# waveygang/wfmash

Hardware: AMD Instinct MI355X
Metric: aligned bases/sec (whole node) + CIGAR-identical rate vs CPU ref (higher is better)
Workload: dtype int32; 1 GPU; C3: 64 synthetic 5%-divergence 50kb segment pairs per GPU, WFA-only (BiWFA gap-affine-2p 5,8,2,24,1; mappings pre-supplied); pairs_per_gpu=64, pairs_total=64, parallelism=records sharded over 1 GPU(s)

## Files before the change

### include/wfmash_hip.h

```cpp
#ifndef WFMASH_HIP_H_
#define WFMASH_HIP_H_

#include <stddef.h>
#include <stdint.h>

#ifdef __cplusplus
extern "C" {
#endif

#define WFM_OK              0
#define WFM_E_NODEVICE     (-1)
#define WFM_E_HIP          (-2)
#define WFM_E_ARG          (-3)
#define WFM_E_NOMEM        (-4)
#define WFM_E_UNSUPPORTED  (-5)
#define WFM_E_ARENA        (-6)

#define WFM_ST_OK            0
#define WFM_ST_UNREACHABLE (-300)
#define WFM_ST_OOM         (-200)
#define WFM_ST_MAX_SCORE   (-100)

#define WFMASH_HIP_VERSION "wfmash-hip-0.3"

// ... 135 lines not shown

#define WFM_CS_SHORT 0
#define WFM_CS_LONG  1
#define WFM_CS_NOT_DONE 1u
#define WFM_CS_SPANS    2u
typedef struct { uint32_t flags, n_runs; uint64_t off, len; } wfm_cs_t;
#define WFM_CS_SLICE 16384
int  wfm_cs_strings(wfm_handle_t* h, const wfm_seqset_t* s, const wfm_result_t* res, const uint32_t* runs, size_t n_runs_total,
                    int form, char** out, size_t* out_bytes, wfm_cs_t* per);
void wfm_free_cs(char* p);

typedef struct { uint32_t problem, kind; uint32_t p, t; uint32_t ref_len, alt_len; uint64_t off; } wfm_variant_t;
typedef struct { uint32_t flags, n_runs; uint64_t first, count; uint32_t end_gaps, pad_; } wfm_varcall_t;
#define WFM_VAR_SNV 0u
#define WFM_VAR_INS 1u
#define WFM_VAR_DEL 2u
#define WFM_VAR_MASKED 256u
#define WFM_VAR_NOT_DONE 1u
#define WFM_VAR_SPANS    2u
#define WFM_VAR_SLICE 16384
int  wfm_call_variants(wfm_handle_t* h, const wfm_seqset_t* s, const wfm_result_t* res, const uint32_t* runs, size_t n_runs_total,
                       wfm_variant_t** vars, size_t* n_vars, char** alleles, size_t* allele_bytes, wfm_varcall_t* per);
void wfm_free_variants(wfm_variant_t* vars, char* alleles);

typedef struct wfm_coverage wfm_coverage_t;
typedef struct { uint64_t base, runs_off; uint32_t n_runs, pad_; } wfm_cov_prob_t;
typedef struct { uint64_t pos; int32_t delta; uint32_t pad_; } wfm_cov_entry_t;
typedef struct { uint64_t start; uint32_t depth, pad_; } wfm_cov_interval_t;
#define WFM_COV_SPANS 2u
#define WFM_COV_TILE 4096
#define WFM_COV_SCAN_BLOCK 1024
int  wfm_coverage_create(wfm_handle_t* h, uint64_t n_bases, wfm_coverage_t** cov);
void wfm_coverage_free(wfm_coverage_t* cov);
int  wfm_coverage_add(wfm_handle_t* h, wfm_coverage_t* cov, const wfm_cov_prob_t* probs, size_t n, const uint32_t* runs, size_t n_runs_total,
                      uint32_t* flags_out);
int  wfm_coverage_export(wfm_handle_t* h, wfm_coverage_t* cov, wfm_cov_entry_t** entries, size_t* n);
int  wfm_coverage_import(wfm_handle_t* h, wfm_coverage_t* cov, const wfm_cov_entry_t* entries, size_t n);
int  wfm_coverage_intervals(wfm_handle_t* h, wfm_coverage_t* cov, wfm_cov_interval_t** iv, size_t* n, uint64_t totals[3]);
void wfm_coverage_free_list(void* p);

#define WFM_OPT_NOT_CHECKED 1u
#define WFM_OPT_SKIPPED     2u
#define WFM_OPT_CHEAPER     4u
#define WFM_OPT_UNREACHED   8u
typedef struct {
  uint32_t flags; int32_t dp_score;
  int32_t  band_lo, band_hi;
  uint64_t cells;
} wfm_optcheck_t;
#define WFM_OPT_BAND_C1   256
#define WFM_OPT_BAND_C4   1024
#define WFM_OPT_REG_MAX   4096
#define WFM_OPT_ROWS_MB   256
int wfm_check_optimal(wfm_handle_t* h, const wfm_penalties_t* pen, const wfm_seqset_t* s,
                      const wfm_result_t* res, uint64_t max_cells , wfm_optcheck_t* out);

void wfm_set_concurrent_calls(wfm_handle_t* h, int other_calls);

#define WFM_PF_ROOT_AGAIN   1u
#define WFM_PF_JOB_AGAIN    2u
#define WFM_PF_BASE_RETRY   4u
#define WFM_PF_BASE_RETRY2  8u
#define WFM_PF_BYTE_KERNEL 16u
#define WFM_PF_P2_ROUNDS   32u
#define WFM_PF_RING_KERNEL 64u
#define WFM_PF_BASE_TILES 128u
#define WFM_PF_RING_GROWN 256u
size_t wfm_get_problem_flags(const wfm_handle_t* h, uint32_t* out, size_t n);

enum {
  WFM_TC_JOBS = 0,
  WFM_TC_EXACT_ENDS = 1,
  WFM_TC_FINE_RERUNS = 2,
  WFM_TC_GAP_RERUNS = 3,
  WFM_TC_RING3 = 4,
  WFM_TC_BLOCKS_COARSE = 5,
  WFM_TC_BLOCKS_FINE = 6,
  WFM_TC_LEFT_BAND = 7,
  WFM_TC_REUSE_RESUMED = 8,
  WFM_TC_REUSE_FALLBACKS = 9,
  WFM_TC_REUSE_KEEPS = 10,
  WFM_TC_REUSE_TOUCHED = 11,
  WFM_TC_REUSE_FELL_OTHER = 12,
  WFM_TILE_COUNTERS = 13
};
size_t wfm_get_tile_counters(const wfm_handle_t* h, uint64_t* out, size_t n);

size_t wfm_trim_device_cache(void);

int  wfm_get_stats(const wfm_handle_t* h, wfm_stats_t* out);
size_t wfm_get_busy_intervals(const wfm_handle_t* h, double* start_end_ms, size_t cap);


int  wfm_hash_kmers(wfm_handle_t* h, const char* seq, int64_t len, int k,
                    uint64_t* hash, int8_t* strand);

typedef struct {
  uint64_t hash;
  int64_t  wpos;
  int64_t  wpos_end;
  int32_t  seqId;
  int16_t  strand;
  int16_t  pad_;
} wfm_minmer_t;

int  wfm_sketch_fragments(wfm_handle_t* h, const char* seq, int64_t seq_len,
                          const int64_t* frag_off, const int32_t* frag_len, size_t n,
                          int k, int s, int32_t seq_id,
                          wfm_minmer_t* out, int32_t* out_count);

typedef struct {
  int64_t  pos;
  uint64_t hash;
  int32_t  seqId;
  int8_t   side;
  int8_t   pad_[3];
} wfm_interval_point_t;

typedef struct wfm_index wfm_index_t;
typedef struct {
  int64_t  n_windows;
  int64_t  n_kept;
  int64_t  n_unique;
  int64_t  n_points;
  uint64_t threshold;
  int64_t  filtered;
  int32_t  adjusted;
  int32_t  pad_;
} wfm_index_info_t;
int  wfm_index_build(wfm_handle_t* h, const wfm_minmer_t* minmers, int64_t n, double max_kmer_freq, wfm_index_t** out);
void wfm_index_free(wfm_handle_t* h, wfm_index_t* ix);
int  wfm_index_info(const wfm_index_t* ix, wfm_index_info_t* out);
int  wfm_index_download(wfm_handle_t* h, const wfm_index_t* ix, uint64_t* uhash, int64_t* poff,
                        wfm_interval_point_t* points, wfm_minmer_t* minmers);

int  wfm_index_replicate(wfm_handle_t* src, const wfm_index_t* ix, wfm_handle_t* dst, wfm_index_t** out);

int  wfm_index_upload(wfm_handle_t* h, const uint64_t* uhash, const int64_t* poff, int64_t n_unique,
                      const wfm_interval_point_t* points, const wfm_minmer_t* minmers, int64_t n_kept,
                      wfm_index_t** out);

int64_t wfm_add_minmers(wfm_handle_t* h, const char* seq, int64_t len, int k, int w, int s, int32_t seq_id,
                        wfm_minmer_t* out, int64_t cap);

int64_t wfm_add_minmers_multi(wfm_handle_t* h, const char* const* seqs, const int64_t* lens, const int32_t* seq_ids,
                              int64_t nseq, int k, int w, int s, int threads, wfm_minmer_t* out, int64_t cap, int64_t* counts);

int wfm_index_build_sequences(wfm_handle_t* h, const char* const* seqs, const int64_t* lens, const int32_t* seq_ids,
                              int64_t nseq, int k, int w, int s, int threads, double max_kmer_freq,
                              wfm_index_t** out, int64_t* n_windows);

typedef struct wfm_minmer_part wfm_minmer_part_t;
int  wfm_sketch_part(wfm_handle_t* h, const char* const* seqs, const int64_t* lens, const int32_t* seq_ids, int64_t nseq,
                     int k, int w, int s, int threads, wfm_minmer_part_t** out);
int64_t wfm_minmer_part_info(const wfm_minmer_part_t* part, int64_t* n_records, int64_t* counts, int64_t cap);
int64_t wfm_minmer_part_download(wfm_handle_t* h, const wfm_minmer_part_t* part, wfm_minmer_t* out, int64_t cap);
void wfm_minmer_part_free(wfm_minmer_part_t* part);

typedef struct { int32_t part; int32_t seq; } wfm_part_seq_t;
#define WFM_GATHER_TILE 2048
int  wfm_index_build_parts(wfm_handle_t* h, const wfm_minmer_part_t* const* parts, int nparts, const wfm_part_seq_t* order,
                           int64_t norder, double max_kmer_freq, wfm_index_t** out, int64_t* n_windows);

int64_t wfm_prefilter_kmers(wfm_handle_t* h, const char* seq, int64_t len, int k, int w, int s, double c_factor,
                            uint32_t* pos, uint64_t* hash, int8_t* strand, int64_t cap);

int64_t wfm_finish_records(wfm_handle_t* h, const wfm_minmer_t* raw, int64_t n, int w, wfm_minmer_t* out, int64_t cap,
// ... 90 lines not shown
```

### include/wfmash_host.h

```cpp
#ifndef WFMASH_HOST_H_
#define WFMASH_HOST_H_

#include <stdint.h>
#include "wfmash_hip.h"

#ifdef __cplusplus
extern "C" {
#endif

typedef struct {
  int32_t  mismatch, gap_open1, gap_ext1, gap_open2, gap_ext2;
  float    min_identity;
  uint64_t min_alignment_length;
  float    min_block_identity;
  uint64_t target_padding;
  uint64_t query_padding;
  uint64_t wflign_max_len_minor;
  int32_t  disable_chain_patching;
  int32_t  sam_format;
  int32_t  emit_md_tag;
  int32_t  no_seq_in_sam;
  int32_t  threads;
  int32_t  resident_sequences;
} wfmh_align_params_t;

typedef struct {
  uint64_t records;
  uint64_t aligned_bp;
  uint64_t written;
  uint64_t skipped;
  uint64_t cells;
  double   ms_gpu;
  double   ms_total;
  double   ms_rows;
  double   ms_fetch;
  double   ms_wflign;
  double   ms_text;
  uint64_t batches;
  uint64_t cells_tile;
  uint64_t tile_launches;
  double   ms_tile;
  double   ms_tags;
  uint64_t records_resident;
  uint64_t lazy_fetches;
} wfmh_align_summary_t;

void wfmh_align_default_params(wfmh_align_params_t* p);

int wfmh_align_paf(wfm_handle_t* h, const char* target_fasta, const char* query_fasta,
                   const char* mapping_paf, const char* out_paf,
                   const wfmh_align_params_t* params, wfmh_align_summary_t* summary);

int wfmh_align_paf_multi(wfm_handle_t* const* handles, int n, const char* target_fasta, const char* query_fasta,
                         const char* mapping_paf, const char* out_paf,
                         const wfmh_align_params_t* params, wfmh_align_summary_t* summary);

void wfmh_set_verify(int on);
int  wfmh_verify_counts(uint64_t out[4]);
int  wfmh_verify_paf(wfm_handle_t* h, const char* target_fasta, const char* query_fasta, const char* aligned_paf, uint64_t out[4]);
char* wfmh_test_verify_parse(const char* line);

void wfmh_set_verify_optimal(int on, uint64_t max_cells);
int  wfmh_verify_optimal_counts(uint64_t out[4]);

void wfmh_set_left_align(int on);
int  wfmh_left_align_counts(uint64_t out[4]);

void wfmh_set_cs(int form);
int  wfmh_cs_counts(uint64_t out[4]);

void wfmh_set_variants(const char* path_or_null);
int  wfmh_variants_counts(uint64_t out[4]);

void wfmh_set_coverage(const char* path_or_null);
int  wfmh_coverage_counts(uint64_t out[4]);
int  wfmh_coverage_paf(wfm_handle_t* h, const char* target_fasta, const char* aligned_paf, const char* out_path, uint64_t out[4]);
char* wfmh_test_coverage_bedgraph(const char* const* names, const uint64_t* lengths, int n_seq, const uint64_t* starts, const uint32_t* depths,
                                  int64_t n_iv);

char* wfmh_test_cigar(const char* fn, const char* a, const char* b, const char* query, const char* target,
                      long long i0, long long i1);
void  wfmh_free(char* p);
void  wfmh_test_subwindow(int64_t win_start, int64_t win_end, int rev, int64_t a, int64_t b, int64_t* out_start, int64_t* out_end);
int wfmh_test_rows(const int32_t* q, int64_t n, int64_t* out);
int wfmh_test_tile_plan(const int32_t* jobs, int64_t n, const int32_t* rules, int32_t* per_block, int32_t* tasks, int64_t tasks_cap, int64_t* scalars);
int wfmh_test_p2_plan(const int32_t* cand, int64_t n, int64_t i0, int rows, int rows_bm, unsigned long long budget, int threads, int core, int64_t* geo,
                      int32_t* tasks, int64_t tasks_cap, int64_t* scalars);
int wfmh_test_base_plan(int op, const int32_t* in, int64_t n, int32_t* out);
int wfmh_test_reuse_plan(int op, const int64_t* in, int64_t n, int64_t* out);
int wfmh_test_tile_plan_dirs(const int32_t* jobs, int64_t n, const int32_t* rules, const uint8_t* dirs, int32_t* per_block, int32_t* tasks, int64_t tasks_cap,
                             int64_t* scalars);
int wfmh_test_tile_interior(const int32_t* q, int64_t n, int32_t* out);
int wfmh_test_tile_lean_waves(const int32_t* in, int64_t* out);
int wfmh_test_opt_band(const int64_t* in, int64_t* out);
int64_t wfmh_test_winnow(const char* seq, int64_t len, int k, int w, int s, int32_t seq_id,
                         const uint64_t* hash, const int8_t* strand, wfm_minmer_t* out, int64_t cap);

int64_t wfmh_test_winnow_chunked(const char* seq, int64_t len, int k, int w, int s, int32_t seq_id,
                                 const uint64_t* hash, const int8_t* strand, int64_t chunk_len,
                                 wfm_minmer_t* out, int64_t cap, int* replays);

int64_t wfmh_test_winnow_thinned(const char* seq, int64_t len, int k, int w, int s, int32_t seq_id,
                                 const uint64_t* hash, const int8_t* strand, double c_factor, int64_t chunk_len,
                                 wfm_minmer_t* out, int64_t cap, uint32_t* kept_pos, int64_t cap_kept,
                                 int64_t* n_kept, int* replays);

void wfmh_test_sort_records(wfm_minmer_t* recs, int64_t n, int threads);
int wfmh_test_packed_lce(const uint8_t* buf_p, int64_t n_p, int64_t start_p, const uint8_t* buf_t, int64_t n_t, int64_t start_t, int v, int h, int maxn);
int wfmh_test_is_acgt(const uint8_t* seq, int64_t n);

int64_t wfmh_test_winnow_model(const char* seq, int64_t len, int k, int w, int s, int32_t seq_id, const uint64_t* hash,
                               const int8_t* strand, double c_factor, int64_t chunk_len, wfm_minmer_t* out, int64_t cap,
                               uint32_t* why);

void wfmh_test_sortlike_model(wfm_minmer_t* recs, int64_t n);

int64_t wfmh_test_finish_records(const wfm_minmer_t* raw, int64_t n, int w, wfm_minmer_t* out, int64_t cap);


typedef struct {
  int32_t  kmer_size;
  int64_t  window_length;
  int64_t  block_length;
  int64_t  chain_gap;
  uint64_t max_mapping_length;
  float    percentage_identity;
  int32_t  sketch_size;
  int32_t  filter_mode;
  uint32_t num_mappings_for_segment;
  uint32_t num_mappings_for_scaffold;
  int32_t  drop_rand;
  int32_t  split;
  int32_t  merge_mappings;
  int32_t  skip_self;
  int32_t  skip_prefix;
  int32_t  lower_triangular;
  char     prefix_delim;
  int32_t  filter_length_mismatches;
  uint64_t sparsity_hash_threshold;
  double   overlap_threshold;
  double   scaffold_overlap_threshold;
  int64_t  scaffold_max_deviation;
  int64_t  scaffold_gap;
  int64_t  scaffold_min_length;
  int32_t  legacy_output;
  int32_t  minimum_hits;
  double   max_kmer_freq;
  int64_t  index_by_size;
  float    kmer_complexity_threshold;
  int32_t  stage1_topani_filter;
  int32_t  stage2_full_scan;
  float    ani_diff, ani_diff_conf;
  double   hg_numerator;
  int32_t  threads;
  int32_t  auto_pct_identity;
  int32_t  ani_percentile;
  float    ani_adjustment;
  const char* target_prefix;
  const char* target_list;
  const char* query_prefix;
  const char* query_list;
  const char* index_file;
  int32_t  write_index;
  int32_t  pad_;
  const char* scaffold_out;
  int32_t  streaming_minhash;
} wfmh_map_params_t;

void wfmh_map_default_params(wfmh_map_params_t* p);

typedef struct {
  uint64_t targets, queries, subsets;
// ... 63 lines not shown
```

### wfmash_amd/capi.py

```python
import ctypes as C
import os

import numpy as np

_HERE = os.path.dirname(os.path.abspath(__file__))
LIB_PATH = os.environ.get("WFM_LIB_PATH") or os.path.join(_HERE, "libwfmash_hip.so")

WFM_MODE_END2END_BIWFA = 0
WFM_MODE_ENDSFREE = 1
WFM_MODE_END2END_UNI = 2
WFM_MODE_MASK = 0xff
WFM_MODE_SCORE_ONLY = 0x100
WFM_MODE_SCORE_LIMIT = 0x200
WFM_ST_MAX_SCORE = -100

DEFAULT_PEN = (5, 8, 2, 24, 1)
WFM_PF_ROOT_AGAIN, WFM_PF_JOB_AGAIN, WFM_PF_BASE_RETRY, WFM_PF_BASE_RETRY2, WFM_PF_BYTE_KERNEL, WFM_PF_P2_ROUNDS, WFM_PF_RING_KERNEL, WFM_PF_BASE_TILES = 1, 2, 4, 8, 16, 32, 64, 128
WFM_PF_RING_GROWN = 256
TILE_COUNTERS = ("jobs", "exact_ends", "fine_reruns", "gap_reruns", "ring3", "blocks_coarse", "blocks_fine", "left_band",
                 "reuse_resumed", "reuse_fallbacks", "reuse_keeps", "reuse_touched", "reuse_fell_other")

EXPORTS = [
    "wfm_create", "wfm_destroy", "wfm_last_error", "wfm_device_name",
    "wfm_align_arena_bytes", "wfm_align_batch", "wfm_upload_sequences",
    "wfm_free_sequences", "wfm_align_resident", "wfm_get_stats",
    "wfm_hash_kmers", "wfm_sketch_fragments", "wfm_add_minmers",
    "wfm_index_build", "wfm_index_free", "wfm_index_info", "wfm_index_download",
    "wfm_map_l1", "wfm_map_l2", "wfm_map_fragments", "wfm_minhash_sketch", "wfm_add_minmers_multi",
    "wfm_prefilter_kmers", "wfm_index_build_sequences", "wfm_index_upload",
    "wfm_index_replicate", "wfm_device_count", "wfm_finish_records",
    "wfm_align_batch_rle", "wfm_align_resident_rle", "wfm_free_runs", "wfm_score_bounds", "wfm_get_busy_intervals", "wfm_trim_device_cache", "wfm_map_fragments_ordered", "wfm_map_sequence_cache", "wfm_selftest_dpp", "wfm_selftest_arena_growth", "wfm_set_concurrent_calls", "wfm_get_problem_flags",
    "wfm_get_tile_counters",
    "wfm_streaming_minmers", "wfm_index_build_streaming",
    "wfm_sketch_part", "wfm_minmer_part_info", "wfm_minmer_part_download", "wfm_minmer_part_free", "wfm_index_build_parts",
    "wfm_seqstore_create", "wfm_seqstore_free", "wfm_seqstore_add", "wfm_seqstore_info",
    "wfm_upload_sequence_refs", "wfm_align_refs_rle", "wfm_download_sequences",
    "wfm_check_runs", "wfm_check_optimal", "wfm_left_align_runs", "wfm_cs_strings", "wfm_free_cs",
    "wfm_call_variants", "wfm_free_variants",
    "wfm_coverage_create", "wfm_coverage_free", "wfm_coverage_add", "wfm_coverage_export", "wfm_coverage_import", "wfm_coverage_intervals",
    "wfm_coverage_free_list",
    "wfm_sketch_intersections",
]
ISECT_LDS_MAX = 4096
WFM_CK_NOT_CHECKED, WFM_CK_BAD_RUN, WFM_CK_SPANS, WFM_CK_M_DIFFERS, WFM_CK_X_EQUAL, WFM_CK_SCORE, WFM_CK_COUNTS = 1, 2, 4, 8, 16, 32, 64
CK_NAMES = ("NOT_CHECKED", "BAD_RUN", "SPANS", "M_DIFFERS", "X_EQUAL", "SCORE", "COUNTS")
CHECK_SLICE = 16384
WFM_LA_NOT_DONE, WFM_LA_SPANS = 1, 2
WFM_CS_SHORT, WFM_CS_LONG = 0, 1
WFM_CS_NOT_DONE, WFM_CS_SPANS = 1, 2
WFM_CS_SLICE = 16384
WFM_VAR_SNV, WFM_VAR_INS, WFM_VAR_DEL = 0, 1, 2
WFM_VAR_MASKED = 256
WFM_VAR_NOT_DONE, WFM_VAR_SPANS = 1, 2
WFM_VAR_SLICE = 16384
WFM_COV_SPANS = 2
WFM_COV_TILE = 4096
WFM_COV_SCAN_BLOCK = 1024
WFM_OPT_NOT_CHECKED, WFM_OPT_SKIPPED, WFM_OPT_CHEAPER, WFM_OPT_UNREACHED = 1, 2, 4, 8
OPT_NAMES = ("NOT_CHECKED", "SKIPPED", "CHEAPER", "UNREACHED")
OPT_BAND_C1, OPT_BAND_C4, OPT_REG_MAX = 256, 1024, 4096
OPT_ROWS_MB = 256
SEQ_GATHER_CHUNK = 16384


class Penalties(C.Structure):
    _fields_ = [("x", C.c_int32), ("o1", C.c_int32), ("e1", C.c_int32),
                ("o2", C.c_int32), ("e2", C.c_int32)]


class Problem(C.Structure):
    _fields_ = [("pattern", C.c_char_p), ("plen", C.c_int32),
                ("text", C.c_char_p), ("tlen", C.c_int32),
                ("mode", C.c_int32),
                ("pattern_begin_free", C.c_int32), ("pattern_end_free", C.c_int32),
                ("text_begin_free", C.c_int32), ("text_end_free", C.c_int32),
                ("score_hint", C.c_int32), ("pad_", C.c_int32)]


class ProblemRef(C.Structure):
    _fields_ = [("pattern", C.c_char_p), ("text", C.c_char_p),
                ("pattern_off", C.c_int64), ("text_off", C.c_int64),
                ("pattern_seq", C.c_int32), ("text_seq", C.c_int32),
                ("plen", C.c_int32), ("tlen", C.c_int32),
                ("mode", C.c_int32),
                ("pattern_revcomp", C.c_int32), ("text_revcomp", C.c_int32),
                ("pattern_begin_free", C.c_int32), ("pattern_end_free", C.c_int32),
                ("text_begin_free", C.c_int32), ("text_end_free", C.c_int32),
                ("score_hint", C.c_int32)]


class Result(C.Structure):
    _fields_ = [("status", C.c_int32), ("score", C.c_int32),
                ("ops_off", C.c_uint64), ("ops_len", C.c_uint32),
                ("n_runs", C.c_uint32), ("cells", C.c_uint64)]


class Check(C.Structure):
    _fields_ = [("flags", C.c_uint32), ("score", C.c_int32), ("bad_p", C.c_int32), ("bad_t", C.c_int32),
                ("bad_run", C.c_uint32), ("n_runs", C.c_uint32),
                ("matches", C.c_uint32), ("mismatches", C.c_uint32), ("ins_runs", C.c_uint32), ("ins_bases", C.c_uint32),
                ("del_runs", C.c_uint32), ("del_bases", C.c_uint32)]


# ... 984 lines not shown
                     ident.ctypes.data, cut.ctypes.data)
        f = self._L.wfm_map_l2
        f.restype = C.c_int64
        f.argtypes = [C.c_void_p, C.c_void_p, C.c_void_p, C.c_void_p, C.c_void_p, C.c_void_p, C.c_int64, C.c_int, C.c_void_p,
                      C.c_int64, C.POINTER(L2Params), C.c_void_p, C.c_void_p, C.c_int64]
        cap = 1 << 16
        while True:
            out = np.zeros(cap, dtype=MAPPING_DTYPE)
            frag = np.zeros(cap, dtype=np.int32)
            n = f(self._p, index._p, q.ctypes.data, qc.ctypes.data, ql.ctypes.data, kc.ctypes.data, nfrag, s, cd.ctypes.data, len(cd),
                  C.byref(P), out.ctypes.data, frag.ctypes.data, cap)
            if n < 0:
                raise WfmError(f"wfm_map_l2 failed ({n}): {self.last_error()}")
            if n <= cap:
                return out[:n], frag[:n]
            cap = int(n)

    def add_minmers_multi(self, seqs, k: int, w: int, s: int, seq_ids=None, threads: int = 1, cap=None):
        n = len(seqs)
        ids = np.ascontiguousarray(seq_ids if seq_ids is not None else range(n), dtype=np.int32)
        bufs = [np.frombuffer(x, dtype=np.uint8) for x in seqs]
        ptrs = (C.c_void_p * n)(*[b.ctypes.data for b in bufs])
        lens = np.array([len(x) for x in seqs], dtype=np.int64)
        cap = int(cap) if cap else 4 * int(lens.sum()) + 64
        out = np.zeros(cap, dtype=MINMER_DTYPE)
        counts = np.zeros(n, dtype=np.int64)
        f = self._L.wfm_add_minmers_multi
        f.restype = C.c_int64
        f.argtypes = [C.c_void_p, C.c_void_p, C.c_void_p, C.c_void_p, C.c_int64, C.c_int, C.c_int, C.c_int, C.c_int, C.c_void_p, C.c_int64,
                      C.c_void_p]
        tot = f(self._p, ptrs, lens.ctypes.data, ids.ctypes.data, n, k, w, s, threads, out.ctypes.data, cap, counts.ctypes.data)
        if tot < 0:
            raise WfmError(f"wfm_add_minmers_multi failed ({tot}): {self.last_error()}")
        offs = np.concatenate([[0], np.cumsum(counts)])
        return [out[offs[i]:offs[i + 1]] for i in range(n)]

    def finish_records(self, raw, w: int):
        raw = np.ascontiguousarray(raw, dtype=MINMER_DTYPE)
        f = self._L.wfm_finish_records
        f.restype = C.c_int64
        f.argtypes = [C.c_void_p, C.c_void_p, C.c_int64, C.c_int, C.c_void_p, C.c_int64, C.POINTER(C.c_int32), C.POINTER(C.c_int32)]
        cap = 4 * len(raw) + 64
        lv, hp = C.c_int32(0), C.c_int32(0)
        while True:
            out = np.zeros(cap, dtype=MINMER_DTYPE)
            n = f(self._p, raw.ctypes.data, len(raw), w, out.ctypes.data, cap, C.byref(lv), C.byref(hp))
            if n < 0:
                raise WfmError(f"wfm_finish_records failed ({n}): {self.last_error()}")
            if n <= cap:
                return out[:n], lv.value, hp.value
            cap = int(n)

    def prefilter_kmers(self, seq: bytes, k: int, w: int, s: int, c_factor: float = 4.0):
        cap = len(seq) + 1
        pos = np.zeros(cap, dtype=np.uint32)
        hsh = np.zeros(cap, dtype=np.uint64)
        st = np.zeros(cap, dtype=np.int8)
        buf = np.frombuffer(seq, dtype=np.uint8)
        f = self._L.wfm_prefilter_kmers
        f.restype = C.c_int64
        f.argtypes = [C.c_void_p, C.c_void_p, C.c_int64, C.c_int, C.c_int, C.c_int, C.c_double, C.c_void_p, C.c_void_p, C.c_void_p, C.c_int64]
        n = f(self._p, buf.ctypes.data, len(seq), k, w, s, c_factor, pos.ctypes.data, hsh.ctypes.data, st.ctypes.data, cap)
        if n < 0:
            raise WfmError(f"wfm_prefilter_kmers failed ({n}): {self.last_error()}")
        return pos[:n], hsh[:n], st[:n]

    def add_minmers(self, seq: bytes, k: int, w: int, s: int, seq_id: int = 0):
        cap = 4 * len(seq) + 64
        out = np.zeros(cap, dtype=MINMER_DTYPE)
        buf = np.frombuffer(seq, dtype=np.uint8)
        self._L.wfm_add_minmers.restype = C.c_int64
        self._L.wfm_add_minmers.argtypes = [C.c_void_p, C.c_void_p, C.c_int64, C.c_int, C.c_int, C.c_int, C.c_int32, C.c_void_p, C.c_int64]
        n = self._L.wfm_add_minmers(self._p, buf.ctypes.data, len(seq), k, w, s, seq_id, out.ctypes.data, cap)
        if n < 0:
            raise WfmError(f"wfm_add_minmers failed ({n}): {self.last_error()}")
        return out[:n]


HOST_EXPORTS = ["wfmh_test_packed_lce", "wfmh_test_is_acgt", "wfmh_align_default_params", "wfmh_align_paf", "wfmh_test_cigar", "wfmh_free", "wfmh_test_winnow",
                "wfmh_map_default_params", "wfmh_test_filter", "wfmh_map", "wfmh_test_winnow_chunked", "wfmh_test_fasta", "wfmh_test_winnow_thinned", "wfmh_test_sort_records", "wfmh_test_index_file",
                "wfmh_map_multi", "wfmh_align_paf_multi", "wfmh_test_winnow_model", "wfmh_test_sortlike_model", "wfmh_test_finish_records",
                "wfmh_release_sequences", "wfmh_test_fasta_shared", "wfmh_seed_paf", "wfmh_test_deal", "wfmh_test_subwindow",
                "wfmh_test_rows", "wfmh_test_tile_plan", "wfmh_test_p2_plan", "wfmh_test_base_plan", "wfmh_test_map_plan", "wfmh_test_filter_ordered",
                "wfmh_test_reuse_plan", "wfmh_test_tile_plan_dirs", "wfmh_test_tile_interior", "wfmh_test_tile_lean_waves", "wfmh_set_verify", "wfmh_verify_counts", "wfmh_verify_paf", "wfmh_test_verify_parse",
                "wfmh_set_verify_optimal", "wfmh_verify_optimal_counts", "wfmh_test_opt_band", "wfmh_set_left_align", "wfmh_left_align_counts", "wfmh_set_cs", "wfmh_cs_counts", "wfmh_set_variants", "wfmh_variants_counts",
                "wfmh_set_coverage", "wfmh_coverage_counts", "wfmh_coverage_paf", "wfmh_test_coverage_bedgraph",
                "wfmh_ani_matrix", "wfmh_ani_matrix_rows", "wfmh_free_ani_rows", "wfmh_set_ani_matrix", "wfmh_test_ani_tsv"]


class MapSummary(C.Structure):
    _fields_ = [("targets", C.c_uint64), ("queries", C.c_uint64), ("subsets", C.c_uint64), ("target_bp", C.c_uint64),
                ("query_bp", C.c_uint64), ("index_windows", C.c_uint64), ("fragments", C.c_uint64), ("l2_mappings", C.c_uint64),
                ("written", C.c_uint64), ("percentage_identity", C.c_float), ("sketch_size", C.c_int32), ("ms_index", C.c_double), ("ms_map", C.c_double), ("ms_filter", C.c_double),
                ("ms_total", C.c_double), ("ms_replicate", C.c_double), ("ms_identity", C.c_double), ("ms_wall", C.c_double),
                ("index_parts", C.c_int32), ("pad_", C.c_int32), ("ms_index_sketch", C.c_double), ("ms_index_merge", C.c_double)]


def _handle_array(handles):
    arr = (C.c_void_p * len(handles))(*[h._p for h in handles])
    return arr


def map_paf_multi(handles, target_fasta: str, out_paf: str, query_fasta: str = None, params=None) -> "MapSummary":
    L = load()
    L.wfmh_map_multi.restype = C.c_int
    L.wfmh_map_multi.argtypes = [C.c_void_p, C.c_int, C.c_char_p, C.c_char_p, C.c_char_p, C.c_void_p, C.POINTER(MapSummary)]
    s = MapSummary()
    rc = L.wfmh_map_multi(_handle_array(handles), len(handles), target_fasta.encode(), query_fasta.encode() if query_fasta else None,
                          out_paf.encode(), C.byref(params) if params is not None else None, C.byref(s))
    if rc != 0:
        raise WfmError(f"wfmh_map_multi failed ({rc}): {handles[0].last_error()}")
    return s


def seed_paf(target_fasta: str, seeds_paf: str, out_paf: str, query_fasta: str = None, params=None) -> "MapSummary":
    L = load()
    L.wfmh_seed_paf.restype = C.c_int
    L.wfmh_seed_paf.argtypes = [C.c_char_p, C.c_char_p, C.c_char_p, C.c_char_p, C.c_void_p, C.POINTER(MapSummary)]
    s = MapSummary()
    rc = L.wfmh_seed_paf(target_fasta.encode(), query_fasta.encode() if query_fasta else None, seeds_paf.encode(), out_paf.encode(),
                         C.byref(params) if params is not None else None, C.byref(s))
    if rc != 0:
        raise WfmError(f"wfmh_seed_paf failed ({rc})")
    return s


def map_paf(handle, target_fasta: str, out_paf: str, query_fasta: str = None, params=None) -> "MapSummary":
    L = load()
    L.wfmh_map.restype = C.c_int
    L.wfmh_map.argtypes = [C.c_void_p, C.c_char_p, C.c_char_p, C.c_char_p, C.c_void_p, C.POINTER(MapSummary)]
    s = MapSummary()
    rc = L.wfmh_map(handle._p, target_fasta.encode(), query_fasta.encode() if query_fasta else None, out_paf.encode(),
                    C.byref(params) if params is not None else None, C.byref(s))
    if rc != 0:
        raise WfmError(f"wfmh_map failed ({rc}): {handle.last_error()}")
    return s


class AniRowC(C.Structure):
    _fields_ = [("query_group", C.c_void_p), ("target_group", C.c_void_p), ("query_hashes", C.c_uint64), ("target_hashes", C.c_uint64),
                ("shared", C.c_uint64), ("jaccard", C.c_double), ("ani", C.c_double)]


def ani_matrix(handles_or_handle, target_fasta: str, query_fasta: str = None, params=None):
    L = load()
    handles = list(handles_or_handle) if isinstance(handles_or_handle, (list, tuple)) else [handles_or_handle]
    f = L.wfmh_ani_matrix_rows
    f.restype = C.c_int
    f.argtypes = [C.c_void_p, C.c_int, C.c_char_p, C.c_char_p, C.c_void_p, C.POINTER(C.POINTER(AniRowC)), C.POINTER(C.c_int64)]
    L.wfmh_free_ani_rows.restype = None
    L.wfmh_free_ani_rows.argtypes = [C.POINTER(AniRowC), C.c_int64]
    rows, n = C.POINTER(AniRowC)(), C.c_int64(0)
    rc = f(_handle_array(handles), len(handles), os.fsencode(target_fasta), os.fsencode(query_fasta) if query_fasta else None,
           C.byref(params) if params is not None else None, C.byref(rows), C.byref(n))
    if rc != 0:
        raise WfmError(f"wfmh_ani_matrix_rows failed ({rc}): {handles[0].last_error()}")
    try:
        return [(C.string_at(r.query_group).decode(), C.string_at(r.target_group).decode(), int(r.query_hashes), int(r.target_hashes),
                 int(r.shared), float(r.jaccard), float(r.ani)) for r in (rows[i] for i in range(n.value))]
    finally:
        L.wfmh_free_ani_rows(rows, n)


def ani_matrix_tsv(handles_or_handle, target_fasta: str, out_tsv: str, query_fasta: str = None, params=None) -> None:
    L = load()
    handles = list(handles_or_handle) if isinstance(handles_or_handle, (list, tuple)) else [handles_or_handle]
    f = L.wfmh_ani_matrix
# ... 638 lines not shown
```

### wfmash_amd/csrc/wfa_device.h

```cpp
#ifndef WFM_WFA_DEVICE_H_
#define WFM_WFA_DEVICE_H_

#include <hip/hip_runtime.h>
#include <stdint.h>

#include "wfa_rows.h"

namespace wfm {

constexpr int WF_NULL = -(1 << 30);
constexpr int RING = 32;
constexpr int RMASK = RING - 1;
constexpr int RING_BIG = 128;

enum { C_M = 0, C_I1 = 1, C_I2 = 2, C_D1 = 3, C_D2 = 4 };
enum { OP_M = 0, OP_X = 1, OP_I = 2, OP_D = 3 };
enum { BT_I1_EXT = 8, BT_I2_EXT = 16, BT_D1_EXT = 32, BT_D2_EXT = 64 };

constexpr int WFM_DEV_UNREACHABLE = -300;
constexpr int WFM_DEV_OVERFLOW = -2;
constexpr int WFM_DEV_BAND = -4;
constexpr int WFM_DEV_P2_NOTHING = -6;
constexpr int WFM_DEV_LIMIT = -7;
constexpr int WFM_DEV_P2_MORE = -5;

struct DevPen { int x, o1, e1, o2, e2; };

struct BpJob {
  int64_t p_fwd, t_fwd, p_rev, t_rev;
  int64_t ring_off;
  int32_t pl, tl;
  int32_t comp_begin, comp_end;
  int32_t width;
  int32_t koff;
  int32_t resume_s;
  int32_t fmax0, rmax0;
  int32_t band;
  int32_t resume_sr;
  int32_t last_fwd;
  int32_t sub;
  int32_t best0;
  int32_t packed;
  int32_t limit;
};
static_assert(sizeof(BpJob) == 104, "BpJob::limit fills the struct's tail padding: the job arrays keep their stride");

struct TileJob {
  int64_t p_fwd, t_fwd, p_rev, t_rev;
  int64_t ring_in, ring_out;
  int32_t pl, tl;
  int32_t comp_begin, comp_end;
  int32_t width, koff;
  int32_t s0;
  int32_t active;
  int32_t fmax, rmax;
  int32_t nblocks;
  int32_t mode;
  int32_t tf, tr;
  int32_t last_fwd;
  int32_t packed;
  int64_t p2_off;
  int32_t w2, koff2;
  int32_t sub;
  int32_t fine_s;
  int64_t ring_prev;
  int32_t prev_ok;
  int32_t reran;
};

struct KeepTask {
  int32_t* dst;
  int32_t job, dir;
  int32_t expect_s;
  int32_t kmin, n;
  int32_t pad_;
};
struct RestoreTask {
  const int32_t* src;
  int32_t job, dir;
  int32_t s_k, kmin, n;
  int32_t slack;
};
void launch_keep(const int32_t* ring, const TileJob* jobs, const KeepTask* tasks, int ntasks, int max_n, hipStream_t st);
void launch_restore(int32_t* ring, const TileJob* jobs, const RestoreTask* tasks, int32_t* out, int ntasks, int max_n, hipStream_t st);

constexpr int P2K = 32;
constexpr int P2ROWS = SNAP_ROWS + P2K;
constexpr int P2TESTS = 2 * P2K;
constexpr int P2ENT = RING * 5;
struct P2Job {
  int64_t ring_in;
  int64_t p2_off;
  int32_t width, koff;
  int32_t w2, koff2;
  int32_t pl, tl;
  int32_t sf, sr, last_fwd;
  int32_t sub, best0;
  int32_t nblk;
  int64_t bm_off;
};

struct BpResult {
  int32_t status;
  int32_t score, score_fwd, score_rev, k_fwd, off_fwd, comp;
  int32_t steps;
  uint64_t cells;
  int32_t steps_p1;
  uint32_t ticks_p1, ticks_p2;
  int32_t pad_;
  uint32_t ticks_list, ticks_pick;
  uint32_t work_items, pad2_;
};

struct BaseJob {
  int64_t p_off, t_off;
  int64_t pre_off;
  int64_t bt_off;
  int64_t ring_off;
  int64_t rle_end;
  int32_t pl, tl;
  int32_t comp_begin, comp_end;
  int32_t endsfree, pbf, pef, tbf, tef;
  int32_t smax, kmin, width;
  int32_t type;
  int32_t pad_;
  int32_t score_only;
};
static_assert(sizeof(BaseJob) == 112, "BaseJob::score_only fills the struct's tail padding: the job arrays keep their stride");

struct BaseResult {
  int32_t status;
  int32_t score;
  int32_t nruns;
  int32_t pad_;
  uint64_t cells;
};

struct Base2TJob {
  BaseJob b;
  int64_t snap_in, snap_out;
  int32_t ntiles, core;
  int32_t task0;
  int32_t s0;
  int32_t done;
  int32_t end_s, end_k, end_off;
};
struct Base2TTask { int32_t job, tile; };
constexpr int B2T_ROWS = 32;
constexpr int B2T_THREADS = 512;
void launch_base2t_block(const uint32_t* pk, int32_t* a32, uint8_t* a8, const Base2TJob* jobs, const Base2TTask* tasks, unsigned long long* tile_key,
                         int32_t* tile_off, int ntasks, int T, hipStream_t st);
// ... 113 lines not shown
```

### wfmash_amd/csrc/wfa_generic_inc.h

```cpp

struct BpCtx {
  const uint8_t* P[2];
  const uint8_t* T[2];
  int32_t* ring;
  int64_t width;
  int pl, tl, koff;
  int kb_lo, kb_hi;
  DevPen pen;
};

__device__ __forceinline__ int32_t* bp_row(const BpCtx& c, int dir, int comp, int s) {
  return c.ring + ((int64_t)((dir * 5 + comp) * RING + (s & RMASK))) * c.width;
}

__device__ __forceinline__ Src bp_src(const BpCtx& c, int dir, int comp, int s, const int (*s_lo)[RING], const int (*s_hi)[RING]) {
  Src r;
  if (s < 0) {
    r.p = c.ring; r.lo = 1; r.hi = 0;
  } else {
    r.p = bp_row(c, dir, comp, s);
    r.lo = s_lo[dir][s & RMASK];
    r.hi = s_hi[dir][s & RMASK];
  }
  return r;
// ... 271 lines not shown
  }
  if (first) bp_row(c, d, C_M, 0)[0] = m0;
  return (c.pl == c.tl && ce == C_M && m0 >= c.tl) ? 1 : 0;
}

__global__ __launch_bounds__(1024) void wfa_bp_kernel(const uint8_t* __restrict__ seq, int32_t* __restrict__ ring_arena,
                                                      const BpJob* __restrict__ jobs, BpResult* __restrict__ results,
                                                      DevPen pen, int scope) {
  const BpJob J = jobs[blockIdx.x];
  __shared__ int s_lo[2][RING];
  __shared__ int s_hi[2][RING];
  __shared__ int s_mak[3][2];
  __shared__ int s_mink[RING * 5];
  __shared__ unsigned char s_bits[RING];
  __shared__ int s_bp[8];
  __shared__ int s_rmax[2][RING][5];

  if (J.resume_s == -3) {
    if (threadIdx.x == 0) {
      BpResult r; r.status = WFM_DEV_BAND; r.score = 0; r.score_fwd = 0; r.score_rev = 0; r.k_fwd = 0; r.off_fwd = 0; r.comp = 0; r.steps = 0; r.cells = 0;
      r.steps_p1 = 0; r.ticks_p1 = 0; r.ticks_p2 = 0; r.pad_ = 0;
      results[blockIdx.x] = r;
    }
    return;
  }
  const int band = J.band;
  BpCtx c;
  c.P[0] = seq + J.p_fwd; c.T[0] = seq + J.t_fwd;
  c.P[1] = seq + J.p_rev; c.T[1] = seq + J.t_rev;
  c.width = J.width;
  c.koff = J.koff;
  c.ring = ring_arena + J.ring_off + c.koff;
  c.pl = J.pl; c.tl = J.tl;
  c.kb_lo = (J.tl - J.pl) - J.sub; c.kb_hi = (J.tl - J.pl) + J.sub;
  c.pen = pen;
  const int tid = threadIdx.x;
  const int A = J.pl + J.tl - 1;
  uint64_t cells = 0;

  if (tid < 2 * RING) { s_lo[tid / RING][tid % RING] = 1; s_hi[tid / RING][tid % RING] = 0; }
  if (tid < 6) ((int*)s_mak)[tid] = 0;
  for (int i = tid; i < 2 * RING * 5; i += blockDim.x) ((int*)s_rmax)[i] = 0;
  __syncthreads();
  int end_reached = 0;
  const bool exact = J.resume_s >= 0 && J.resume_sr >= 0;
  const int rs_f = J.resume_s, rs_r = exact ? J.resume_sr : J.resume_s;
  if (J.resume_s >= 0) {
    if (tid < 2 * RING) {
      const int d = tid / RING, sc = (d == 0 ? rs_f : rs_r) - (tid % RING);
      if (sc >= 0) { const Rng RG = make_rng(J.pl, J.tl, J.sub); s_lo[d][sc & RMASK] = rng_lo(RG, sc); s_hi[d][sc & RMASK] = rng_hi(RG, sc); }
    }
    if (tid == 0) { s_mak[0][0] = J.fmax0; s_mak[0][1] = J.rmax0; s_bp[6] = 0; s_bp[7] = 0; }
  } else if (tid < 128) {
    const int d = tid >> 6;
    int mak = 0;
    const int ended = bp_init_row0(c, d, d == 0 ? J.comp_begin : J.comp_end, d == 0 ? J.comp_end : J.comp_begin, mak);
    if ((tid & 63) == 0) {
      s_bp[6 + d] = ended;
      s_lo[d][0] = 0; s_hi[d][0] = 0;
      s_mak[0][d] = mak;
    }
  }
  __syncthreads();
  int fmax = s_mak[0][0], rmax = s_mak[0][1];
  end_reached = s_bp[6] | s_bp[7];
  if (end_reached) {
    if (tid == 0) {
      BpResult r; r.status = 1; r.score = 0; r.score_fwd = 0; r.score_rev = 0; r.k_fwd = 0; r.off_fwd = 0; r.comp = 0; r.steps = 0; r.cells = 2;
      r.steps_p1 = 0; r.ticks_p1 = 0; r.ticks_p2 = 0; r.pad_ = 0;
      results[blockIdx.x] = r;
    }
    return;
  }
  cells = J.resume_s >= 0 ? 0 : 2;
  const int64_t max_steps = (int64_t)(pen.o1 + pen.o2) * 4 + (int64_t)(J.pl + J.tl + 2) * max(pen.x, max(pen.e1, pen.e2)) * 2 + 256;
  int sf = max(rs_f, 0), sr = max(rs_r, 0);
  int last_fwd = exact ? J.last_fwd : 0;
  int status = 0;
  int buf = 0;
  const long long t_begin = wall_clock64();
  long long sec[8] = {0, 0, 0, 0, 0, 0, 0, 0};
  (void)sec;

  for (;;) {
    if (fmax + rmax >= A) break;
    if (J.limit > 0 && sf >= J.limit) { status = WFM_DEV_LIMIT; break; }
    if (band > 0 && max(sf, sr) + 2 > band) { status = WFM_DEV_BAND; break; }
    buf = (buf + 1) % 3;
    if (tid == 0) { s_mak[(buf + 1) % 3][0] = 0; s_mak[(buf + 1) % 3][1] = 0; }
    if (tid < 10) s_rmax[tid / 5][((tid < 5 ? sf : sr) + 2) & RMASK][tid % 5] = 0;
    int makf = 0, makr = 0;
    int cmf[5] = {0, 0, 0, 0, 0}, cmr[5] = {0, 0, 0, 0, 0};
    SEC_T(ta);
    const int nf = bp_compute_row<true>(c, 0, sf + 1, s_lo, s_hi, makf, sec, cmf);
    const int nr = bp_compute_row<true>(c, 1, sr + 1, s_lo, s_hi, makr, sec, cmr);
    SEC_T(tb);
    makf = wave_max(makf);
    makr = wave_max(makr);
    if ((tid & 63) == 0) {
      if (makf > 0) atomicMax(&s_mak[buf][0], makf);
      if (makr > 0) atomicMax(&s_mak[buf][1], makr);
    }
#pragma unroll
    for (int cc = 0; cc < 5; ++cc) {
      const int vf = wave_max_dpp63(cmf[cc]), vr = wave_max_dpp63(cmr[cc]);
      if ((tid & 63) == 63) {
        if (vf > 0) atomicMax(&s_rmax[0][(sf + 1) & RMASK][cc], vf);
        if (vr > 0) atomicMax(&s_rmax[1][(sr + 1) & RMASK][cc], vr);
      }
    }
    SEC_T(tc);
    __syncthreads();
    SEC_T(td);
    SEC_ADD(3, ta, tb); SEC_ADD(4, tb, tc); SEC_ADD(5, tc, td);
    ++sf; cells += (uint64_t)nf;
    fmax = max(fmax, s_mak[buf][0]);
    last_fwd = 1;
    if (fmax + rmax >= A) break;
    ++sr; cells += (uint64_t)nr;
    rmax = max(rmax, s_mak[buf][1]);
    last_fwd = 0;
    if ((int64_t)sf + sr > max_steps) { status = WFM_DEV_UNREACHABLE; break; }
  }

  const int best0 = min(J.sub < SUB_NONE ? J.sub + 1 : INT32_MAX, J.best0 > 0 ? J.best0 : INT32_MAX);
  int best = best0;
  if (tid == 0) s_bp[7] = 0;
  const long long t_mid = wall_clock64();
#ifdef WFM_PROFILE_SECTIONS
  if (tid == 0 && blockIdx.x == 0) { for (int q = 0; q < 6; ++q) g_sec[q] = sec[q]; g_sec[6] = sf + sr; }
#endif
  const int steps_p1 = sf + sr;
  if (status == 0) {
    const int gopen = max(pen.o1, pen.o2);
    const int own_f = max(rs_f, 0) + 1, own_r = max(rs_r, 0) + 1;
    for (int i = 0; i < scope; ++i) {
      if (sf - i >= 0 && sf - i < own_f) bp_row_maxima(c, 0, sf - i, s_lo, s_hi, s_rmax);
      if (sr - i >= 0 && sr - i < own_r) bp_row_maxima(c, 1, sr - i, s_lo, s_hi, s_rmax);
    }
    __syncthreads();
    for (;;) {
      int d0;
      if (last_fwd) {
        const int min_sr = (sr > scope - 1) ? sr - (scope - 1) : 0;
        if (sf + min_sr - gopen >= best) break;
        d0 = 0;
      } else {
        const int min_sf = (sf > scope - 1) ? sf - (scope - 1) : 0;
        if (min_sf + sr - gopen >= best) break;
        d0 = 1;
      }
      const int s0 = d0 == 0 ? sf : sr;
      const int s1 = d0 == 0 ? sr : sf;
      const bool m0_valid = s_lo[d0][s0 & RMASK] <= s_hi[d0][s0 & RMASK];
      if (m0_valid) {
        for (int i = tid; i < RING * 5; i += blockDim.x) s_mink[i] = INT32_MAX;
        if (tid < scope) s_bits[tid] = (unsigned char)bp_pair_bits(c, d0, s0, s1, tid, best, s_lo, s_hi, s_rmax);
        __syncthreads();
        bp_overlap_scan(c, d0, s0, s1, best, s_lo, s_hi, s_mink, scope, s_rmax, s_bits);
        __syncthreads();
        if (tid == 0) {
          int b = best;
          const int order[5] = {C_D2, C_I2, C_D1, C_I1, C_M};
          for (int i = 0; i < scope; ++i) {
            const int si = s1 - i;
            if (si < 0) break;
            for (int oi = 0; oi < 5; ++oi) {
// ... 408 lines not shown
```

### wfmash_amd/csrc/wfa_host.hip

```cpp
#include <hip/hip_runtime.h>

#include <algorithm>
#include <chrono>
#include <climits>
#include <cstdio>
#include <cstring>
#include <atomic>
#include <mutex>
#include <string>
#include <thread>
#include <vector>

#include "../../include/wfmash_hip.h"
#include "wfa_device.h"
#include "dev_cache.h"
#include "wfa_plan.h"
#include "wfa_optband.h"

#ifdef WFM_PROFILE_SECTIONS
namespace wfm { void read_sections(long long* out); }
#endif
namespace wfm { void p2_counters(unsigned long long* out); }
namespace {

// ... 517 lines not shown
}


struct TileCfg {
  bool exact = true;
  int T_refine = 0;
  int chunk = 2;
  int T = 100, Wt = 1024, threads = 512;
  int min_len = 128, min_score = 64;
  bool enabled = true;
  bool reg = false;
  int C = 2;
  bool fine = true;
  int debug = 0;
  bool p2_dump_on = false;
  int p2_dump = 0;
};

TileCfg tile_cfg(const wfm_penalties_t& pen, int scope) {
  TileCfg c;
  if (const char* e = getenv("WFM_TILE")) c.enabled = atoi(e) != 0;
  if (const char* e = getenv("WFM_TILE_T")) c.T = atoi(e);
  if (const char* e = getenv("WFM_TILE_T_REFINE")) c.T_refine = atoi(e);
  if (const char* e = getenv("WFM_TILE_EXACT")) c.exact = atoi(e) != 0;
  if (const char* e = getenv("WFM_TILE_W")) c.Wt = atoi(e);
  if (const char* e = getenv("WFM_TILE_THREADS")) c.threads = atoi(e);
  if (const char* e = getenv("WFM_TILE_MIN_LEN")) c.min_len = atoi(e);
  if (const char* e = getenv("WFM_TILE_MIN_SCORE")) c.min_score = atoi(e);
  c.fine = env_num("WFM_TILE_FINE", 1) != 0;
  c.debug = env_debug();
  if (const char* e = getenv("WFM_P2_DUMP")) { c.p2_dump_on = true; c.p2_dump = atoi(e); }
  const int RR = ring_rows_for(scope);
  c.T = std::max(c.T, RR);
  if (c.T_refine > 0) c.T_refine = std::max(c.T_refine, RR);
  const bool dflt = pen.x == 5 && pen.o1 + pen.e1 == 10 && pen.o2 + pen.e2 == 25 && pen.e1 == 2 && pen.e2 == 1;
  c.reg = dflt && !(getenv("WFM_TILE_REG") && atoi(getenv("WFM_TILE_REG")) == 0);
  if (c.reg) {
    if (!getenv("WFM_TILE_THREADS")) c.threads = 512;
    c.T = std::min(c.T, (int)((40 * 1024) / (4 * TILE_SLOTS_WIDE)) - 1);
    while (c.threads * c.C <= 2 * c.T && c.threads < 1024) c.threads += 64;
    if (const char* e = getenv("WFM_TILE_CHUNK")) c.chunk = std::max(1, atoi(e));
    c.Wt = c.threads * c.C;
    return c;
  }
  const size_t rows = (size_t)scope + 2 * (pen.e1 + 1) + 2 * (pen.e2 + 1);
  while ((rows * c.Wt + c.T + 1) * 4 > 160 * 1024 && c.Wt > 4 * c.T) c.Wt -= 64;
  if (c.Wt < 4 * c.T || (rows * c.Wt + c.T + 1) * 4 > 160 * 1024) c.enabled = false;
  return c;
}


inline TileJob tile_job_from(const BpJob& j) {
  TileJob t{};
  t.p_fwd = j.p_fwd; t.t_fwd = j.t_fwd; t.p_rev = j.p_rev; t.t_rev = j.t_rev;
  t.ring_in = j.ring_off;
  t.pl = j.pl; t.tl = j.tl; t.comp_begin = j.comp_begin; t.comp_end = j.comp_end;
  t.width = j.width; t.koff = j.koff; t.active = 1; t.packed = j.packed; t.sub = j.sub;
  return t;
}

struct ReuseUse { int32_t keep = 0, dir = 0, s_k = 0; };
struct ReuseCtl {
  KeepStore* store = nullptr;
  int cadence = 0;
  int slack = 0;
  int min_blocks = 1;
  std::vector<ReuseUse> use;
  std::vector<int32_t> upto;
  std::vector<int32_t> meet;
  std::vector<char> bad;
  std::vector<std::vector<int32_t>> kept[2];
  uint64_t keep_bytes = 0, restore_bytes = 0;
};

struct TilePhase {
  wfm_handle* h; wfm_seqset* S; const DevPen& dp; int scope; const TileCfg& cfg; int T; bool refine;
  std::vector<BpJob>& jobs; const std::vector<int>& tiled; std::vector<int64_t>& ring2; double& tile_ms; uint64_t& tile_cells;
  size_t n;
  std::vector<TileJob> tj, got;
  std::vector<int> fmax, rmax, s_begin;
  std::vector<char> active;
  size_t n_active = 0;
  bool any_cut = false;
  int chunk = 1;
  TilePlanRules rules;
  std::vector<TilePlanJob> pjobs;
  TileChunkPlan plan;
  uint32_t blocks = 0;
  double lane_cells = 0;
  ReuseCtl* ru = nullptr;
  std::vector<uint8_t> dirs, own;
  std::vector<int32_t> resumed_at;
  std::vector<KeepTask> ktasks;
  std::vector<int32_t> kids;
  std::vector<RestoreTask> rtasks;
  std::vector<int32_t> rres;
};

void reuse_fall_back(TilePhase& p, size_t i, bool touched = false) {
  if (p.active[i]) { p.active[i] = 0; --p.n_active; }
  p.tj[i].active = 0; p.tj[i].mode = 3;
  p.dirs[i] = 3; p.resumed_at[i] = -1;
  p.ru->bad[i] = 1;
  p.ru->store->drop(p.ru->use[i].keep);
  p.h->tile_ctr[WFM_TC_REUSE_FALLBACKS] += 1;
  p.h->tile_ctr[touched ? WFM_TC_REUSE_TOUCHED : WFM_TC_REUSE_FELL_OTHER] += 1;
}

int init_tile_jobs(TilePhase& p, const std::vector<int32_t>* fine_from, const std::vector<int64_t>* ring3) {
  wfm_handle* h = p.h;
  const TileCfg& cfg = p.cfg;
  const size_t n = p.n;
  const int T = p.T;
  p.tj.resize(n); p.fmax.assign(n, 0); p.rmax.assign(n, 0); p.active.assign(n, 1); p.s_begin.assign(n, 0);
  p.dirs.assign(n, 3); p.own.assign(n, 3); p.resumed_at.assign(n, 0);
  if (p.ru) { p.ru->bad.assign(n, 0); p.ru->kept[0].assign(n, {}); p.ru->kept[1].assign(n, {}); }
  for (size_t i = 0; i < n; ++i) {
    const BpJob& j = p.jobs[(size_t)p.tiled[i]];
    TileJob& t = p.tj[i];
    t = tile_job_from(j);
    t.ring_out = p.ring2[i];
    t.fine_s = (fine_from && i < fine_from->size()) ? (*fine_from)[i] : INT_MAX;
    t.ring_prev = (ring3 && i < ring3->size() && (*ring3)[i] >= 0 && (j.packed & 1) && cfg.reg && cfg.exact && !p.refine) ? (*ring3)[i] : -1;
    h->tile_ctr[WFM_TC_RING3] += t.ring_prev >= 0;
  }
  if (!p.refine || T == cfg.T) h->tile_ctr[WFM_TC_JOBS] += n;
  for (size_t i = 0; i < n; ++i) p.any_cut |= p.tj[i].sub != SUB_NONE;
  if (h->tilejobs.ensure(n) || h->tilemak.ensure(n * 2 * (size_t)std::max(T, 2))) { h->err = "out of device memory (tiles)"; return WFM_E_NOMEM; }
  if (!p.refine) {
    HIPCHK(h, hipMemcpyAsync(h->tilejobs.p, p.tj.data(), n * sizeof(TileJob), hipMemcpyHostToDevice, h->stream));
    launch_tile_init(p.S->d_seq, h->ring.p, h->tilejobs.p, h->tilemak.p, (int)n, ring_rows_for(p.scope), h->stream);
    HIPCHK(h, hipGetLastError());
    std::vector<int32_t> mak(n * 4);
    HIPCHK(h, hipMemcpyAsync(mak.data(), h->tilemak.p, n * 4 * sizeof(int32_t), hipMemcpyDeviceToHost, h->stream));
    HIPCHK(h, hipStreamSynchronize(h->stream));
    for (size_t i = 0; i < n; ++i) {
      p.fmax[i] = mak[(i * 2 + 0) * 2]; p.rmax[i] = mak[(i * 2 + 1) * 2];
      const bool ended = mak[(i * 2 + 0) * 2 + 1] || mak[(i * 2 + 1) * 2 + 1];
      const int A = p.tj[i].pl + p.tj[i].tl - 1;
      if (ended || p.fmax[i] + p.rmax[i] >= A) p.active[i] = 0;
      p.n_active += p.active[i];
      p.tj[i].active = p.active[i]; p.tj[i].fmax = p.fmax[i]; p.tj[i].rmax = p.rmax[i]; p.tj[i].nblocks = 0;
    }
    for (size_t i = 0; p.ru && i < n; ++i) {
      ReuseUse& u = p.ru->use[i];
      if (u.keep <= 0) continue;
      const int A = p.tj[i].pl + p.tj[i].tl - 1;
      const int kept_max = p.ru->store->v[(size_t)u.keep - 1].mx;
      if (!p.active[i] || kept_max + (u.dir == 0 ? p.rmax[i] : p.fmax[i]) >= A) {
        p.ru->store->drop(u.keep); u.keep = 0;
        h->tile_ctr[WFM_TC_REUSE_FALLBACKS] += 1;
        h->tile_ctr[WFM_TC_REUSE_FELL_OTHER] += 1;
        continue;
      }
      (u.dir == 0 ? p.fmax[i] : p.rmax[i]) = kept_max;
      p.tj[i].fmax = p.fmax[i]; p.tj[i].rmax = p.rmax[i];
      p.dirs[i] = (uint8_t)(1 << (1 - u.dir)); p.own[i] = p.dirs[i];
    }
  } else {
    for (size_t i = 0; i < n; ++i) {
      const BpJob& j = p.jobs[(size_t)p.tiled[i]];
      const int A = p.tj[i].pl + p.tj[i].tl - 1;
      p.fmax[i] = j.fmax0; p.rmax[i] = j.rmax0;
      p.s_begin[i] = j.resume_s;
      p.active[i] = (char)(p.fmax[i] + p.rmax[i] < A);
      p.n_active += p.active[i];
      p.tj[i].s0 = j.resume_s; p.tj[i].active = p.active[i]; p.tj[i].fmax = p.fmax[i]; p.tj[i].rmax = p.rmax[i]; p.tj[i].nblocks = 0;
    }
  }
  return WFM_OK;
}

int drop_leavers(TilePhase& p) {
  wfm_handle* h = p.h;
  bool left = false;
  for (size_t i = 0; i < p.n; ++i) {
    const TileJob& t = p.tj[i];
    const BpJob& bj = p.jobs[(size_t)p.tiled[i]];
    if (!p.active[i] || !(tile_job_leaves(t.pl, t.tl, t.sub, t.s0, bj.band, p.chunk, p.T) || tile_job_beyond_limit(t.pl, t.tl, t.sub, bj.limit, t.s0, p.T))) continue;
    p.active[i] = 0; p.tj[i].active = 0; p.tj[i].mode = 3; left = true; --p.n_active;
  }
  if (left) HIPCHK(h, hipMemcpyAsync(h->tilejobs.p, p.tj.data(), p.n * sizeof(TileJob), hipMemcpyHostToDevice, h->stream));
  return WFM_OK;
}

int plan_tile_tasks(TilePhase& p) {
  wfm_handle* h = p.h;
  for (size_t i = 0; i < p.n; ++i) {
    const TileJob& t = p.tj[i];
    p.pjobs[i] = TilePlanJob{t.pl, t.tl, t.sub, t.s0, t.mode, t.fine_s, t.packed, p.active[i]};
  }
  plan_tile_chunk(p.pjobs.data(), p.n, p.rules, p.plan, p.dirs.data());
  const std::vector<TileTask>& tasks = p.plan.tasks;
  if (tasks.empty()) { h->err = "tile phase: active jobs without a tile"; return WFM_E_HIP; }
  if (h->tiletasks.ensure(tasks.size())) { h->err = "out of device memory (tile tasks)"; return WFM_E_NOMEM; }
  HIPCHK(h, hipMemcpyAsync(h->tiletasks.p, tasks.data(), tasks.size() * sizeof(TileTask), hipMemcpyHostToDevice, h->stream));
  return WFM_OK;
}

int launch_keeps(TilePhase& p) {
  wfm_handle* h = p.h;
  p.ktasks.clear(); p.kids.clear();
  if (!p.ru || p.ru->cadence <= 0) return WFM_OK;
  ReuseCtl& ru = *p.ru;
  int max_n = 0;
  for (size_t i = 0; i < p.n && ru.cadence > 0; ++i) {
    const TileJob& t = p.tj[i];
    const int64_t es = (int64_t)t.s0 + (int64_t)p.chunk * p.T;
    if (!p.active[i] || t.mode != 0 || es > ru.upto[i] || es < (int64_t)ru.min_blocks * p.T || es % ((int64_t)ru.cadence * p.T) != 0) continue;
    if (!reuse_keep_wanted((int)es, ru.meet[i] > 0 ? ru.meet[i] : reuse_meet_estimate(t.s0, (int64_t)p.fmax[i] + p.rmax[i], t.pl + t.tl - 1), ru.cadence, p.T)) continue;
    for (int d = 0; d < 2; ++d) {
      if (!((p.own[i] >> d) & 1)) continue;
      KeptRows kr;
      kr.s0 = (int32_t)es; kr.kmin = reuse_keep_kmin(t.pl, (int)es); kr.n = reuse_keep_cols(t.pl, t.tl, (int)es);
      kr.pl = t.pl; kr.tl = t.tl; kr.sub = t.sub;
      kr.d = ru.store->take(reuse_keep_elems(t.pl, t.tl, (int)es), &kr.slab);
      if (!kr.d) {
        ru.cadence = ru.cadence * 2 <= (1 << 20) ? ru.cadence * 2 : 0;
        break;
      }
      ru.store->v.push_back(kr);
      p.kids.push_back((int32_t)ru.store->v.size());
      p.ktasks.push_back(KeepTask{kr.d, (int32_t)i, d, kr.s0, kr.kmin, kr.n, 0});
      max_n = std::max(max_n, kr.n);
      ru.keep_bytes += 2ull * 4ull * (uint64_t)KEEP_ROWS * (uint64_t)kr.n;
    }
  }
  if (p.ktasks.empty()) return WFM_OK;
  if (h->keeptasks.ensure(p.ktasks.size())) { h->err = "out of device memory (keeps)"; return WFM_E_NOMEM; }
  HIPCHK(h, hipMemcpyAsync(h->keeptasks.p, p.ktasks.data(), p.ktasks.size() * sizeof(KeepTask), hipMemcpyHostToDevice, h->stream));
  launch_keep(h->ring.p, h->tilejobs.p, h->keeptasks.p, (int)p.ktasks.size(), max_n, h->stream);
  HIPCHK(h, hipGetLastError());
  return WFM_OK;
}

void settle_keeps(TilePhase& p) {
  for (size_t q = 0; q < p.ktasks.size(); ++q) {
    const KeepTask& kt = p.ktasks[q];
    const TileJob& t = p.tj[(size_t)kt.job];
    if (t.active && t.mode == 0 && t.s0 == kt.expect_s) {
      p.ru->store->v[(size_t)p.kids[q] - 1].mx = kt.dir == 0 ? t.fmax : t.rmax;
      p.ru->kept[kt.dir][(size_t)kt.job].push_back(p.kids[q]);
      p.h->tile_ctr[WFM_TC_REUSE_KEEPS] += 1;
    } else p.ru->store->drop(p.kids[q]);
  }
  p.ktasks.clear(); p.kids.clear();
}

int restore_kept(TilePhase& p) {
  wfm_handle* h = p.h;
  if (!p.ru) return WFM_OK;
  ReuseCtl& ru = *p.ru;
  bool changed = false;
  p.rtasks.clear();
  int max_n = 0;
  for (size_t i = 0; i < p.n; ++i) {
    const TileJob& t = p.tj[i];
    if (p.resumed_at[i] > 0) {
      if (t.s0 > p.resumed_at[i]) p.resumed_at[i] = -1;
      else if (!t.active || t.mode != 0) { reuse_fall_back(p, i); changed = true; }
      continue;
    }
    if (p.dirs[i] == 3 || ru.bad[i]) continue;
    const ReuseUse& u = ru.use[i];
    if (!t.active || t.mode != 0 || t.s0 > u.s_k || (u.s_k - t.s0) % (p.chunk * p.T) != 0) { reuse_fall_back(p, i); changed = true; continue; }
    if (t.s0 < u.s_k) continue;
    const KeptRows& kr = ru.store->v[(size_t)u.keep - 1];
    p.rtasks.push_back(RestoreTask{kr.d, (int32_t)i, u.dir, u.s_k, kr.kmin, kr.n, ru.slack});
    max_n = std::max(max_n, kr.n);
    ru.restore_bytes += 2ull * 4ull * (uint64_t)KEEP_ROWS * (uint64_t)kr.n;
  }
  if (!p.rtasks.empty()) {
    p.rres.assign(p.rtasks.size() * 2, 0);
    if (h->restoretasks.ensure(p.rtasks.size()) || h->restoreres.ensure(p.rres.size())) { h->err = "out of device memory (keeps)"; return WFM_E_NOMEM; }
    HIPCHK(h, hipMemcpyAsync(h->restoretasks.p, p.rtasks.data(), p.rtasks.size() * sizeof(RestoreTask), hipMemcpyHostToDevice, h->stream));
    HIPCHK(h, hipMemsetAsync(h->restoreres.p, 0, p.rres.size() * sizeof(int32_t), h->stream));
    launch_restore(h->ring.p, h->tilejobs.p, h->restoretasks.p, h->restoreres.p, (int)p.rtasks.size(), max_n, h->stream);
    HIPCHK(h, hipGetLastError());
    HIPCHK(h, hipMemcpyAsync(p.rres.data(), h->restoreres.p, p.rres.size() * sizeof(int32_t), hipMemcpyDeviceToHost, h->stream));
    HIPCHK(h, hipStreamSynchronize(h->stream));
    for (size_t q = 0; q < p.rtasks.size(); ++q) {
      const size_t i = (size_t)p.rtasks[q].job;
      changed = true;
      if (p.rres[2 * q]) { reuse_fall_back(p, i, true); continue; }
      const ReuseUse& u = ru.use[i];
      (u.dir == 0 ? p.fmax[i] : p.rmax[i]) = p.rres[2 * q + 1];
      p.tj[i].fmax = p.fmax[i]; p.tj[i].rmax = p.rmax[i];
      p.tj[i].prev_ok = 0;
      p.dirs[i] = 3; p.resumed_at[i] = u.s_k;
      ru.store->drop(u.keep);
      h->tile_ctr[WFM_TC_REUSE_RESUMED] += 1;
    }
  }
  if (changed) HIPCHK(h, hipMemcpyAsync(h->tilejobs.p, p.tj.data(), p.n * sizeof(TileJob), hipMemcpyHostToDevice, h->stream));
  return WFM_OK;
}

int launch_chunk(TilePhase& p) {
  wfm_handle* h = p.h;
  wfm_seqset* S = p.S;
  const TileCfg& cfg = p.cfg;
  const int T = p.T;
  const std::vector<TileTask>& tasks = p.plan.tasks;
  const size_t n_pk = p.plan.n_pk;
  const std::vector<int>&threads_b = p.plan.threads_b, &variants_b = p.plan.variants_b;
  const size_t lds = ((size_t)(p.scope + 2 * (p.dp.e1 + 1) + 2 * (p.dp.e2 + 1)) * cfg.Wt + T + 1) * 4;
  for (int b = 0; b < p.chunk; ++b) {
    HIPCHK(h, hipEventRecord(h->tile_ev[2 * b], h->stream));
    if (cfg.reg) {
      if (n_pk) {
        launch_tile2(S->d_pk, h->ring.p, h->tilejobs.p, h->tiletasks.p, h->tilemak.p, (int)n_pk, threads_b[(size_t)b], T, variants_b[(size_t)b], h->stream);
        h->tile_ctr[WFM_TC_BLOCKS_COARSE] += (variants_b[(size_t)b] & 1) != 0;
        h->tile_ctr[WFM_TC_BLOCKS_FINE] += (variants_b[(size_t)b] & 2) != 0;
      }
      if (tasks.size() > n_pk)
        launch_tile_reg(S->d_seq, h->ring.p, h->tilejobs.p, h->tiletasks.p + n_pk, h->tilemak.p, (int)(tasks.size() - n_pk), threads_b[(size_t)b], T, cfg.C, p.any_cut, h->stream);
    } else launch_tile(S->d_seq, h->ring.p, h->tilejobs.p, h->tiletasks.p, h->tilemak.p, (int)tasks.size(), cfg.threads, T, cfg.Wt, lds, p.dp, p.scope, ring_rows_for(p.scope), h->stream);
    HIPCHK(h, hipEventRecord(h->tile_ev[2 * b + 1], h->stream));
    launch_tile_advance(h->tilejobs.p, h->tilemak.p, (int)p.n, T, p.dp, (cfg.reg && cfg.exact) ? 1 : 0, p.rules.coarse_on ? 1 : 0, variants_b[(size_t)b], h->stream);
  }
  HIPCHK(h, hipGetLastError());
  const int rc = launch_keeps(p);
  if (rc != WFM_OK) return rc;
  HIPCHK(h, hipMemcpyAsync(p.got.data(), h->tilejobs.p, p.n * sizeof(TileJob), hipMemcpyDeviceToHost, h->stream));
  return WFM_OK;
}

int time_chunk(TilePhase& p) {
  wfm_handle* h = p.h;
  const size_t ntasks = p.plan.tasks.size();
  for (int b = 0; b < p.chunk; ++b) {
    float ms = 0;
    HIPCHK(h, hipEventElapsedTime(&ms, h->tile_ev[2 * b], h->tile_ev[2 * b + 1]));
    p.tile_ms += ms;
    if (h->call_base) {
      float t0 = 0;
      HIPCHK(h, hipEventElapsedTime(&t0, h->call_base, h->tile_ev[2 * b]));
      h->tile_iv.emplace_back(t0, t0 + ms);
    }
  }
  p.blocks += (uint32_t)p.chunk;
  for (int b = 0; b < p.chunk; ++b) p.lane_cells += (double)ntasks * p.plan.threads_b[(size_t)b] * p.cfg.C * p.T;
  h->stats.tile_launches += (uint32_t)p.chunk;
  h->stats.tile_tasks += (uint32_t)(ntasks * (size_t)p.chunk);
  return WFM_OK;
}

void account_chunk(TilePhase& p) {
  wfm_handle* h = p.h;
  const int T = p.T;
  p.n_active = 0;
  for (size_t i = 0; i < p.n; ++i) {
    const TileJob& was = p.tj[i];
    const TileJob& got = p.got[i];
    for (int bl = was.nblocks; bl < got.nblocks; ++bl) {
      const bool last_exact = got.mode == 2 && bl == got.nblocks - 1;
      const int base = p.s_begin[i] + (last_exact ? bl - 1 : bl) * T;
      for (int d = 0; d < 2; ++d) {
        if (!((p.dirs[i] >> d) & 1)) continue;
        const int steps = last_exact ? (d == 0 ? got.tf : got.tr) : T;
        p.tile_cells += (uint64_t)cells_sum(was.pl, was.tl, was.sub, base + 1, base + steps);
      }
    }
    if (got.fine_s == -1 && was.fine_s != -1) {
      for (int d = 0; d < 2; ++d) if ((p.dirs[i] >> d) & 1) p.tile_cells += (uint64_t)cells_sum(was.pl, was.tl, was.sub, got.s0 + 1, got.s0 + T);
      h->tile_ctr[WFM_TC_FINE_RERUNS] += 1;
    }
    if (got.reran > was.reran) {
      for (int d = 0; d < 2; ++d) if ((p.dirs[i] >> d) & 1) p.tile_cells += (uint64_t)cells_sum(was.pl, was.tl, was.sub, got.s0 - T + 1, got.s0);
      h->tile_ctr[WFM_TC_GAP_RERUNS] += (uint64_t)(got.reran - was.reran);
    }
    p.tj[i] = got;
    p.active[i] = (char)(got.active != 0);
    p.fmax[i] = got.fmax; p.rmax[i] = got.rmax;
    p.n_active += p.active[i];
  }
}

void hand_back(TilePhase& p, uint32_t level, double cells_before) {
  wfm_handle* h = p.h;
  uint64_t unique_level = 0;
  for (size_t i = 0; i < p.n; ++i) {
    const TileJob& t = p.tj[i];
    const int sf_end = t.mode == 2 ? t.s0 + t.tf : t.s0, sr_end = t.mode == 2 ? t.s0 + t.tr : t.s0;
    if (p.ru && p.ru->bad[i]) continue;
    unique_level += (uint64_t)cells_sum(t.pl, t.tl, t.sub, p.s_begin[i] + 1, sf_end) + (uint64_t)cells_sum(t.pl, t.tl, t.sub, p.s_begin[i] + 1, sr_end);
  }
  h->stats.cells_tile_unique += unique_level;
  for (size_t i = 0; i < p.n; ++i) {
    const TileJob& t = p.tj[i];
    BpJob& j = p.jobs[(size_t)p.tiled[i]];
    j.ring_off = t.ring_in;
    p.ring2[i] = t.ring_out;
    j.resume_s = t.s0;
    j.resume_sr = -1; j.last_fwd = 0;
    h->tile_ctr[WFM_TC_EXACT_ENDS] += t.mode == 2;
    h->tile_ctr[WFM_TC_LEFT_BAND] += t.mode == 3 && !(p.ru && p.ru->bad[i]);
    if (t.mode == 3) {
      j.resume_s = -3; j.resume_sr = t.s0; j.fmax0 = p.fmax[i]; j.rmax0 = p.rmax[i];
      continue;
    }
    if (t.mode == 2) {
      j.resume_s = t.s0 + t.tf;
      j.resume_sr = t.s0 + t.tr;
      j.last_fwd = t.last_fwd;
    }
    j.fmax0 = p.fmax[i]; j.rmax0 = p.rmax[i];
  }
  if (p.cfg.debug) fprintf(stderr, "[wfm] level %u: tiled %zu jobs, %u blocks of %d scores (Wt %d), %.3f ms; %.3e cells computed on %.3e lane-steps (%.0f %% of the lanes hold a cell), %.3e of them in the result (the block in which a job's wavefronts meet runs twice)\n", level, p.n, p.blocks, p.T, p.cfg.Wt, p.tile_ms,
                           (double)p.tile_cells - cells_before, p.lane_cells, p.lane_cells > 0 ? 100.0 * ((double)p.tile_cells - cells_before) / p.lane_cells : 0.0, (double)unique_level);
}

int run_tiled_phase(wfm_handle* h, wfm_seqset* S, const DevPen& dp, int scope, const TileCfg& cfg, int T, bool refine,
                    std::vector<BpJob>& jobs, const std::vector<int>& tiled, std::vector<int64_t>& ring2,
                    double& tile_ms, uint64_t& tile_cells, uint32_t level, const std::vector<int32_t>* fine_from = nullptr,
                    const std::vector<int64_t>* ring3 = nullptr, ReuseCtl* reuse = nullptr) {
  const size_t n = tiled.size();
  if (n == 0) return WFM_OK;
  const double cells_before = (double)tile_cells;
  TilePhase p{h, S, dp, scope, cfg, T, refine, jobs, tiled, ring2, tile_ms, tile_cells, n};
  p.ru = refine ? nullptr : reuse;
  int rc = init_tile_jobs(p, fine_from, ring3);
  if (rc != WFM_OK) return rc;
  if (p.n_active) {
    HIPCHK(h, hipMemcpyAsync(h->tilejobs.p, p.tj.data(), n * sizeof(TileJob), hipMemcpyHostToDevice, h->stream));
    HIPCHK(h, hipMemsetAsync(h->tilemak.p, 0, n * 2 * (size_t)T * sizeof(int32_t), h->stream));
    p.chunk = std::max(1, std::min(cfg.chunk, (int)h->tile_ev.size() / 2));
    p.got.resize(n); p.pjobs.resize(n);
    p.rules = TilePlanRules{cfg.threads, cfg.C, T, p.chunk, cfg.Wt - 2 * T, cfg.reg, cfg.fine, cfg.reg && cfg.exact && tile2_coarse_maxima()};
    auto clk = [] { return std::chrono::steady_clock::now(); };
    auto msd = [](std::chrono::steady_clock::time_point a, std::chrono::steady_clock::time_point b) { return std::chrono::duration<double, std::milli>(b - a).count(); };
    double ms_prep = 0, ms_launch = 0, ms_wait = 0, ms_post = 0;
    while (p.n_active) {
      const auto tq0 = clk();
      if ((rc = drop_leavers(p)) != WFM_OK) return rc;
      if (!p.n_active) break;
      if ((rc = plan_tile_tasks(p)) != WFM_OK) return rc;
      const auto tq1 = clk();
      if ((rc = launch_chunk(p)) != WFM_OK) return rc;
      const auto tq2 = clk();
      HIPCHK(h, hipStreamSynchronize(h->stream));
      const auto tq3 = clk();
      if ((rc = time_chunk(p)) != WFM_OK) return rc;
      account_chunk(p);
      settle_keeps(p);
      if ((rc = restore_kept(p)) != WFM_OK) return rc;
      ms_prep += msd(tq0, tq1); ms_launch += msd(tq1, tq2); ms_wait += msd(tq2, tq3); ms_post += msd(tq3, clk());
    }
    if (cfg.debug > 1)
      fprintf(stderr, "[wfm] level %u tile phase, host side: task lists %.2f ms, launches %.2f ms, waiting for the device %.2f ms, bookkeeping %.2f ms\n", level, ms_prep, ms_launch, ms_wait, ms_post);
  }
  hand_back(p, level, cells_before);
  return WFM_OK;
}


struct P2Chunk {
  wfm_handle* h; wfm_seqset* S; const DevPen& dp; int scope; const TileCfg& cfg; std::vector<BpJob>& jobs;
  const std::vector<int>& cand; const std::vector<int64_t>& ring_other; std::vector<BpResult>& res; double& ms_out;
  std::vector<BpResult>& carry; std::vector<char>& has_carry; bool may_continue; std::vector<int>& again;
  std::vector<P2PlanJob> pcand;
  P2ChunkPlan plan;
  size_t i0 = 0, n = 0;
  std::vector<TileJob> tj;
  std::vector<P2Job> pj;
  std::vector<BpResult> got;
  float ms = 0;
};

void fill_p2_chunk(P2Chunk& c, size_t i0) {
  const size_t budget = std::max<size_t>(c.h->mem_budget / 4, (size_t)64 << 20);
  plan_p2_chunk(c.pcand.data(), c.pcand.size(), i0, P2K, P2ROWS, budget, c.cfg.threads, c.cfg.Wt - 2 * P2K, c.plan);
  c.i0 = i0; c.n = c.plan.geo.size();
  c.tj.clear(); c.pj.clear();
  for (size_t q = 0; q < c.n; ++q) {
    const BpJob& j = c.jobs[(size_t)c.cand[i0 + q]];
    const P2Geometry& g = c.plan.geo[q];
    TileJob t = tile_job_from(j);
    t.ring_out = c.ring_other[i0 + q];
    t.mode = 4; t.tf = j.resume_s; t.tr = j.resume_sr; t.last_fwd = j.last_fwd;
    t.p2_off = (int64_t)g.p2_off; t.w2 = (int32_t)g.w2; t.koff2 = g.koff2;
    P2Job pq{};
    pq.ring_in = j.ring_off; pq.p2_off = (int64_t)g.p2_off; pq.width = j.width; pq.koff = j.koff; pq.w2 = (int32_t)g.w2; pq.koff2 = g.koff2;
    pq.pl = j.pl; pq.tl = j.tl; pq.sf = j.resume_s; pq.sr = j.resume_sr; pq.last_fwd = j.last_fwd; pq.sub = j.sub; pq.best0 = j.best0;
    pq.nblk = (int32_t)g.nblk; pq.bm_off = (int64_t)g.bm_off;
    c.tj.push_back(t); c.pj.push_back(pq);
  }
}

int launch_p2_chunk(P2Chunk& c) {
  wfm_handle* h = c.h;
  wfm_seqset* S = c.S;
  const size_t n = c.n, elems = c.plan.elems, bm_elems = c.plan.bm_elems, n_pk = c.plan.tiles.n_pk;
  const std::vector<TileTask>& tasks = c.plan.tiles.tasks;
  const int threads_c = c.plan.threads_c;
  if (h->p2rows.ensure(elems + 16) || h->p2max.ensure(n * 2 * P2ROWS * 5) || h->p2bmax.ensure(bm_elems + 16) || h->p2pbmax.ensure(bm_elems + 16) ||
      h->p2jobs.ensure(n) || h->tilejobs.ensure(n) || h->tiletasks.ensure(tasks.size()) || h->bpres.ensure(std::max(n, c.jobs.size()))) {
    h->err = "out of device memory (phase-2 rows)"; return WFM_E_NOMEM;
  }
  HIPCHK(h, hipMemcpyAsync(h->tilejobs.p, c.tj.data(), n * sizeof(TileJob), hipMemcpyHostToDevice, h->stream));
  HIPCHK(h, hipMemcpyAsync(h->p2jobs.p, c.pj.data(), n * sizeof(P2Job), hipMemcpyHostToDevice, h->stream));
  HIPCHK(h, hipMemcpyAsync(h->tiletasks.p, tasks.data(), tasks.size() * sizeof(TileTask), hipMemcpyHostToDevice, h->stream));
  HIPCHK(h, hipEventRecord(h->ev0, h->stream));
  bool any_cut = false;
  for (const TileJob& t : c.tj) any_cut |= t.sub != SUB_NONE;
  if (n_pk) launch_tile2_p2(S->d_pk, h->ring.p, h->tilejobs.p, h->tiletasks.p, (int)n_pk, threads_c, h->p2rows.p, h->stream);
  if (tasks.size() > n_pk) launch_tile_p2(S->d_seq, h->ring.p, h->tilejobs.p, h->tiletasks.p + n_pk, (int)(tasks.size() - n_pk), threads_c, h->p2rows.p, any_cut, h->stream);
  launch_p2_blockmax(h->ring.p, h->p2rows.p, h->p2jobs.p, h->p2bmax.p, h->p2max.p, (int)n, h->stream);
  static const int p2_threads = getenv("WFM_P2_THREADS") ? atoi(getenv("WFM_P2_THREADS")) : 0;
  launch_p2_overlap(h->ring.p, h->p2rows.p, h->p2jobs.p, h->p2max.p, h->p2bmax.p, h->p2pbmax.p, h->bpres.p, (int)n,
                    p2_threads > 0 ? p2_threads : 1024, (int)(c.plan.maxw2 >> 6) + 1, c.dp, c.scope, h->stream);
  HIPCHK(h, hipGetLastError());
// ... 24 lines not shown
    for (int r = 0; r < P2ROWS; r += 3) {
      const int32_t* m = rm.data() + ((size_t)d * P2ROWS + r) * 5;
      fprintf(stderr, "[wfm]   dir %d row %d (s = %d): max M %d I1 %d I2 %d D1 %d D2 %d\n", d, r, (d == 0 ? pjq.sf : pjq.sr) - RNG_BACK + r, m[0], m[1], m[2], m[3], m[4]);
    }
  return WFM_OK;
}

void print_p2_chunk(const P2Chunk& c) {
  const std::vector<BpResult>& got = c.got;
  const std::vector<P2Job>& pj = c.pj;
  const size_t n = c.n;
  int more = 0;
  double tk = 0, tc = 0, rd = 0; uint32_t tkmax = 0; int rdmax = 0;
  for (const BpResult& r : got) { more += r.status == WFM_DEV_P2_MORE; tk += r.ticks_p2; tc += r.ticks_p1; rd += r.pad_; tkmax = std::max(tkmax, r.ticks_p2); rdmax = std::max(rdmax, r.pad_); }
  fprintf(stderr, "[wfm] phase 2 from rows computed ahead: %zu jobs, widest %zu columns, %zu tiles of %d threads, %.3f ms, %d left to the step kernel; walk per job: %.1f rounds (max %d), %.0f us (max %.0f), of which cells stage %.0f us\n",
          n, c.plan.maxw2, c.plan.tiles.tasks.size(), c.plan.threads_c, c.ms, more, rd / n, rdmax, tk / n / 100.0, tkmax / 100.0, tc / n / 100.0);
  size_t qs = 0;
  for (size_t q = 0; q < n; ++q) if (got[q].ticks_p2 > got[qs].ticks_p2) qs = q;
  fprintf(stderr, "[wfm]   slowest walk: pl %d tl %d sub %d w2 %d nblk %d: %d rounds, %.0f us = listing %.0f + cells %.0f (incl. listing) + pick %.0f, %u blocks listed, status %d\n", pj[qs].pl, pj[qs].tl,
          pj[qs].sub == SUB_NONE ? -1 : pj[qs].sub, pj[qs].w2, pj[qs].nblk, got[qs].pad_, got[qs].ticks_p2 / 100.0, got[qs].ticks_list / 100.0, got[qs].ticks_p1 / 100.0, got[qs].ticks_pick / 100.0,
          got[qs].work_items, got[qs].status);
}

int continue_p2_chunk(P2Chunk& c) {
  wfm_handle* h = c.h;
  std::vector<BpResult>& got = c.got;
  std::vector<P2Job> mj;
  for (size_t q = 0; q < c.n; ++q) {
    const size_t jq = (size_t)c.cand[c.i0 + q];
    BpJob& j = c.jobs[jq];
    if (got[q].status == WFM_DEV_P2_NOTHING) { got[q] = c.carry[jq]; continue; }
    if (got[q].status != WFM_DEV_P2_MORE) continue;
    if (got[q].comp >= 0) {
      c.carry[jq] = got[q]; c.carry[jq].status = 0; c.has_carry[jq] = 1;
      j.best0 = got[q].score;
    }
    if (!c.may_continue || (j.band > 0 && std::max(j.resume_s, j.resume_sr) + 2 * P2K + 2 > j.band)) continue;
    mj.push_back(c.pj[q]);
    j.resume_s += P2K; j.resume_sr += P2K;
    c.again.push_back((int)(c.i0 + q));
  }
  if (!mj.empty()) {
    HIPCHK(h, hipMemcpyAsync(h->p2jobs.p, mj.data(), mj.size() * sizeof(P2Job), hipMemcpyHostToDevice, h->stream));
    launch_p2_to_ring(h->ring.p, h->p2rows.p, h->p2jobs.p, (int)mj.size(), h->stream);
    HIPCHK(h, hipGetLastError());
    HIPCHK(h, hipStreamSynchronize(h->stream));
  }
  for (size_t q = 0; q < c.n; ++q) c.res[(size_t)c.cand[c.i0 + q]] = got[q];
  return WFM_OK;
}

int run_p2_phase(wfm_handle* h, wfm_seqset* S, const DevPen& dp, int scope, const TileCfg& cfg, std::vector<BpJob>& jobs,
                 const std::vector<int>& cand, const std::vector<int64_t>& ring_other, std::vector<BpResult>& res, double& ms_out,
                 std::vector<BpResult>& carry, std::vector<char>& has_carry, bool may_continue, std::vector<int>& again) {
  if (cand.empty()) return WFM_OK;
  P2Chunk c{h, S, dp, scope, cfg, jobs, cand, ring_other, res, ms_out, carry, has_carry, may_continue, again};
  for (int q : cand) {
    const BpJob& j = jobs[(size_t)q];
    c.pcand.push_back(P2PlanJob{j.pl, j.tl, j.sub, j.resume_s, j.resume_sr, j.packed});
  }
  for (size_t i0 = 0; i0 < cand.size(); i0 += c.n) {
    fill_p2_chunk(c, i0);
    int rc = launch_p2_chunk(c);
    if (rc != WFM_OK) return rc;
    if (cfg.p2_dump_on && (rc = dump_p2_job(c)) != WFM_OK) return rc;
    h->stats.p2_launches++;
    h->stats.p2_jobs += (uint32_t)c.n;
    if (cfg.debug) print_p2_chunk(c);
    if ((rc = continue_p2_chunk(c)) != WFM_OK) return rc;
  }
  return WFM_OK;
}


struct Knobs {
  static int num(const char* name, int dflt) { const char* e = getenv(name); return e ? atoi(e) : dflt; }
  bool use_hints = num("WFM_SCORE_HINT", 1) != 0;
  bool use_bound = use_hints && num("WFM_BOUND", 1) != 0;
  int slack_env = num("WFM_SUB_SLACK", -1);
  bool ring3_on = num("WFM_TILE_RING3", 1) != 0, p2_on = num("WFM_P2", 1) != 0;
  int p2_rounds = std::max(1, num("WFM_P2_ROUNDS", 64));
  int fine_margin = num("WFM_TILE_FINE_MARGIN", 48);
  int coarse_min_blocks = num("WFM_TILE_COARSE_MIN_BLOCKS", 32), coarse_max_jobs = num("WFM_TILE_COARSE_MAX_JOBS", 128);
  bool tile_v2 = num("WFM_TILE_V2", 1) != 0;
  bool band_on = num("WFM_BAND", 1) != 0;
  int band_root = std::max(64, num("WFM_BAND_ROOT", 4096));
  int resume_margin = num("WFM_RESUME_MARGIN", SNAP_ROWS);
  bool reuse = num("WFM_REUSE", 1) != 0 && slack_env < (1 << 28);
  int reuse_min_blocks = std::max(1, num("WFM_REUSE_MIN_BLOCKS", 8));
  int reuse_every = std::max(1, num("WFM_REUSE_EVERY", 2)), reuse_slack = std::max(0, num("WFM_REUSE_TOUCH_SLACK", 0));
  int reuse_levels = num("WFM_REUSE_LEVELS", 8);
  int debug = env_debug();
};

struct Chunk {
  std::vector<BpJob> jobs;
  std::vector<int32_t> node_of;
  size_t ring_elems = 0, end = 0;
  int maxw = 0;
  std::vector<int> tiled, tiled_r;
  std::vector<int64_t> ring2, ring3, ring2_r;
  std::vector<int32_t> fine_from, fine_r, snap_r;
  std::vector<size_t> ring_third;
  std::vector<char> grown_job, resume_bad, has_carry;
  std::vector<ReuseUse> reuse;
  std::vector<int32_t> keep_upto;
  std::vector<char> reuse_bad;
  std::vector<std::vector<int32_t>> kept[2];
  std::vector<BpResult> res, carry;
  std::vector<int> rest, more_set;
  void clear() {
    jobs.clear(); node_of.clear(); ring_elems = 0; maxw = 0;
    tiled.clear(); ring2.clear(); ring3.clear(); ring_third.clear(); fine_from.clear();
    tiled_r.clear(); ring2_r.clear(); fine_r.clear(); snap_r.clear(); grown_job.clear();
    reuse.clear(); keep_upto.clear();
  }
};

struct AlignCall {
  wfm_handle* h;
  const wfm_penalties_t* pen;
  wfm_seqset* S;
  size_t first, last;
  wfm_result_t* out;
  char* ops_arena;
  size_t arena_bytes, arena_base;
  std::vector<uint32_t>* runs_out;
  uint32_t* pflags;
  int scope;
  DevPen dp;
  const Knobs knobs;
  TileCfg tcfg;
  BaseCfg bcfg;
  int RR;
  RingRules rules;
  std::vector<int32_t> prob_status;
  std::vector<uint64_t> prob_cells;
  std::vector<int32_t> prob_score;
  std::vector<Node> bp_nodes, base_nodes, next_bp;
  uint32_t level = 0;
  Chunk ck;
  LevelTimer tm;
  double wall_tile = 0, wall_base = 0;
  uint64_t band_retries = 0, band_jobs = 0, roots_banded = 0, roots_out = 0, hint_retries = 0, limit_out = 0;
  uint64_t grown_jobs = 0, grown_widened = 0, grown_restarts = 0;
  int64_t grown_maxband = 0;
  size_t ring_peak = 0;
  GrownSnaps snaps;
  KeepStore keeps;
  uint64_t reuse_children = 0, reuse_found = 0, reuse_taken = 0;
  uint64_t keep_bytes = 0, restore_bytes = 0;
  uint64_t reuse_full_rings = 0;
};

void make_roots(AlignCall& c) {
  for (size_t i = c.first; i < c.last; ++i) {
    const ProbMeta& pm = c.S->meta[i];
    Node nd{};
    nd.prob = (int32_t)i; nd.pb = 0; nd.pl = pm.plen; nd.tb = 0; nd.tl = pm.tlen;
    nd.cb = C_M; nd.ce = C_M; nd.score_rem = INT_MAX; nd.endsfree = 0;
    nd.sub = SUB_NONE; nd.hinted = 0;
    if (c.pflags && (pm.mode == WFM_MODE_END2END_BIWFA || pm.mode == WFM_MODE_ENDSFREE) && !((size_t)i < c.S->acgt.size() && c.S->acgt[i])) c.pflags[i] |= WFM_PF_BYTE_KERNEL;
    if (c.knobs.use_hints && pm.hint > 0 && pm.mode == WFM_MODE_END2END_BIWFA) { nd.sub = pm.hint; nd.hinted = 1; }
    if (pm.limit > 0) { nd.limit = pm.limit; nd.sub = pm.limit; nd.hinted = 1; }
    int64_t bound = (int64_t)gapcost(*c.pen, pm.plen) + gapcost(*c.pen, pm.tlen) + 8;
    if (pm.limit > 0 && (pm.plen == 0 || pm.tlen == 0) && bound - 8 > pm.limit) { c.prob_status[i] = WFM_ST_MAX_SCORE; continue; }
    if (pm.limit > 0) bound = std::min<int64_t>(bound, pm.limit);
    if (pm.mode == WFM_MODE_ENDSFREE) {
      nd.endsfree = 1;
      nd.smax = (int32_t)std::min<int64_t>(bound, 256);
      c.base_nodes.push_back(nd);
    } else if (pm.mode == WFM_MODE_END2END_UNI || std::max(pm.plen, pm.tlen) <= BIALIGN_FALLBACK_MIN_LENGTH ||
               pm.plen == 0 || pm.tlen == 0) {
      nd.smax = (int32_t)std::min<int64_t>(bound, 256);
      c.base_nodes.push_back(nd);
    } else {
      c.bp_nodes.push_back(nd);
    }
  }
}

int bound_roots(AlignCall& c) {
  wfm_handle* h = c.h;
  std::vector<BoundJob> bj;
  std::vector<size_t> owner;
  if (c.knobs.use_bound)
    for (size_t q = 0; q < c.bp_nodes.size(); ++q) {
      const Node& nd = c.bp_nodes[q];
      const ProbMeta& pm = c.S->meta[nd.prob];
      if (pm.mode != WFM_MODE_END2END_BIWFA || std::min(nd.pl, nd.tl) < 1024 || std::abs(nd.tl - nd.pl) < 64) continue;
      bj.push_back(BoundJob{pm.p_fwd, pm.t_fwd, nd.pl, nd.tl});
      owner.push_back(q);
    }
  if (bj.empty()) return WFM_OK;
  uint64_t bounded_roots = 0, bound_gain = 0;
  const auto tb0 = std::chrono::steady_clock::now();
  if (h->bndjobs.ensure(bj.size()) || h->bndres.ensure(bj.size())) { h->err = "out of device memory (score bounds)"; return WFM_E_NOMEM; }
  HIPCHK(h, hipMemcpyAsync(h->bndjobs.p, bj.data(), bj.size() * sizeof(BoundJob), hipMemcpyHostToDevice, h->stream));
// ... 19 lines not shown
  return WFM_OK;
}

void level_budget(AlignCall& c) {
  size_t total = 0;
  for (const Node& nd : c.bp_nodes) total += ring_elems(ring_full_width(nd.pl, nd.tl), c.RR, 2);
  c.rules.use_band = c.knobs.band_on && total * 4 > std::min<size_t>(c.h->mem_budget, (size_t)2 << 30);
  c.rules.over_budget = total * 4 > c.h->mem_budget;
}

void plan_chunk(AlignCall& c, size_t i0) {
  wfm_handle* h = c.h;
  Chunk& k = c.ck;
  const TileCfg& tcfg = c.tcfg;
  static const size_t ring_chunk_bytes = (size_t)(getenv("WFM_RING_CHUNK_GB") ? std::max(1, atoi(getenv("WFM_RING_CHUNK_GB"))) : 4) << 30;
  k.clear();
  size_t i = i0;
  int64_t fine_min_blocks_r = INT64_MAX;
  int64_t fine_min_blocks = INT64_MAX;
  for (; i < c.bp_nodes.size(); ++i) {
    const Node& nd = c.bp_nodes[i];
    const ProbMeta& pm = c.S->meta[nd.prob];
    RingPlan rp = plan_ring(nd, c.rules);
    const int32_t job_sub = (nd.sub != SUB_NONE && (nd.limit > 0 || (int64_t)std::abs(nd.tl - nd.pl) * 8 >= (int64_t)nd.sub)) ? nd.sub : SUB_NONE;
    const bool reuse_on = c.knobs.reuse && tcfg.reg && tcfg.exact && c.RR == RING;
    if (nd.keep > 0 && reuse_on && rp.fits && rp.band > 0 && !rp.grown) {
      RingRules full = c.rules;
      full.use_band = false;
      const RingPlan fp = plan_ring(nd, full);
      const KeptRows& kr = c.keeps.v[(size_t)nd.keep - 1];
      if (kr.d && kr.s0 % (tcfg.chunk * tcfg.T) == 0 && reuse_eligible(nd, fp, kr.pl, kr.tl, kr.sub, job_sub, kr.s0, tcfg.T)) { rp = fp; ++c.reuse_full_rings; }
    }
    if (!rp.fits) { c.prob_status[nd.prob] = WFM_ST_OOM; c.snaps.drop(nd.snap); c.keeps.drop(nd.keep); continue; }
    const size_t width = rp.width, need = rp.need; const int band = rp.band; const bool tile_it = rp.tile_it, grown = rp.grown;
    if (!k.jobs.empty() && (k.ring_elems + need) * 4 > std::min<size_t>(h->mem_budget, k.jobs.size() >= 128 ? ring_chunk_bytes : std::max(ring_chunk_bytes, (size_t)8 << 30))) break;
    BpJob j{};
    j.p_fwd = pm.p_fwd + nd.pb;
    j.t_fwd = pm.t_fwd + nd.tb;
    j.p_rev = pm.p_rev + (pm.plen - nd.pb - nd.pl);
    j.t_rev = pm.t_rev + (pm.tlen - nd.tb - nd.tl);
    j.ring_off = (int64_t)k.ring_elems;
    j.pl = nd.pl; j.tl = nd.tl;
    j.comp_begin = nd.cb; j.comp_end = nd.ce;
    j.width = (int32_t)width;
    j.koff = rp.koff;
    j.resume_s = -1; j.resume_sr = -1; j.last_fwd = 0; j.fmax0 = 0; j.rmax0 = 0;
    j.band = band;
    j.sub = job_sub;
    j.limit = nd.limit;
    j.best0 = 0;
    j.packed = (c.knobs.tile_v2 && tcfg.reg && tcfg.C == 2 && (size_t)nd.prob < c.S->acgt.size() && c.S->acgt[(size_t)nd.prob]) ? 1 : 0;
    if (j.packed && nd.sub != SUB_NONE && (int64_t)nd.sub * 16 < (int64_t)nd.pl + nd.tl) j.packed |= 2;
    c.band_jobs += band > 0 && !grown;
    k.grown_job.push_back((char)grown);
    const bool resumes = grown && tile_it && nd.snap > 0;
    if (nd.snap > 0 && !resumes) c.snaps.drop(nd.snap);
    if (grown) {
      ++c.grown_jobs;
      c.grown_maxband = std::max<int64_t>(c.grown_maxband, band);
      if (resumes) ++c.grown_widened; else if (nd.noband || nd.band > 0) ++c.grown_restarts;
      if (c.pflags) c.pflags[nd.prob] |= WFM_PF_RING_GROWN;
      if (c.knobs.debug)
        fprintf(stderr, "[wfm] grown ring: problem %d, %s of %d x %d: band %d, %zu columns on the %s%s\n", nd.prob, nd.score_rem == INT_MAX ? "root" : "child", nd.pl, nd.tl, band, width,
                tile_it ? "tile kernels" : "step kernel alone", resumes ? ", widened from its snapshot" : ((nd.noband || nd.band > 0) ? ", from score 0 again" : ""));
    }
    if (resumes) {
      const GrownSnap& sn = c.snaps.v[(size_t)nd.snap - 1];
      k.tiled_r.push_back((int)k.jobs.size()); k.ring2_r.push_back((int64_t)(k.ring_elems + need / 2)); k.snap_r.push_back(nd.snap);
      const int64_t est = nd.score_rem != INT_MAX ? (int64_t)nd.score_rem : (int64_t)nd.pl + nd.tl;
      fine_min_blocks_r = std::min<int64_t>(fine_min_blocks_r, std::max<int64_t>(0, est / 2 - sn.s0) / tcfg.T);
      k.fine_r.push_back(nd.score_rem != INT_MAX ? std::max(0, nd.score_rem / 2 - c.knobs.fine_margin) : INT_MAX);
    } else if (tile_it) {
      k.tiled.push_back((int)k.jobs.size()); k.ring2.push_back((int64_t)(k.ring_elems + need / 2)); k.ring_third.push_back(need / 2);
      const int64_t est = nd.score_rem != INT_MAX ? (int64_t)nd.score_rem : (nd.sub != SUB_NONE ? (int64_t)nd.sub : (int64_t)nd.pl + nd.tl);
      fine_min_blocks = std::min<int64_t>(fine_min_blocks, est / 2 / tcfg.T);
      k.fine_from.push_back(nd.score_rem != INT_MAX ? std::max(0, nd.score_rem / 2 - c.knobs.fine_margin) : INT_MAX);
      ReuseUse use;
      if (nd.keep > 0 && reuse_on) {
        const KeptRows& kr = c.keeps.v[(size_t)nd.keep - 1];
        if (kr.d && kr.s0 % (tcfg.chunk * tcfg.T) == 0 && reuse_eligible(nd, rp, kr.pl, kr.tl, kr.sub, j.sub, kr.s0, tcfg.T)) { use.keep = nd.keep; use.dir = nd.keep_dir; use.s_k = kr.s0; ++c.reuse_taken; }
      }
      if (nd.keep > 0 && use.keep == 0) c.keeps.drop(nd.keep);
      k.reuse.push_back(use);
      int32_t upto = 0;
      if (reuse_on && band == 0 && !grown && (int)c.level <= c.knobs.reuse_levels && !(nd.score_rem == INT_MAX && pm.score_only())) {
        const int known = nd.score_rem != INT_MAX ? nd.score_rem : (nd.sub != SUB_NONE ? nd.sub : INT_MAX);
        upto = known != INT_MAX ? std::max(0, reuse_resume_limit(known / 2 + 2 * SNAP_ROWS, tcfg.T, c.knobs.fine_margin)) : INT_MAX;
      }
      k.keep_upto.push_back(upto);
    } else c.keeps.drop(nd.keep);
    if (resumes) c.keeps.drop(nd.keep);
    k.node_of.push_back((int32_t)i);
    k.ring_elems += need;
    const int64_t est_w = nd.score_rem == INT_MAX ? (int64_t)width : std::min<int64_t>((int64_t)width, (int64_t)nd.score_rem + 128);
    k.maxw = std::max(k.maxw, (int)est_w);
    k.jobs.push_back(j);
  }
  k.end = i;
  if (k.tiled.size() > (size_t)c.knobs.coarse_max_jobs || fine_min_blocks < (int64_t)c.knobs.coarse_min_blocks) std::fill(k.fine_from.begin(), k.fine_from.end(), 0);
  if (k.tiled_r.size() > (size_t)c.knobs.coarse_max_jobs || fine_min_blocks_r < (int64_t)c.knobs.coarse_min_blocks) std::fill(k.fine_r.begin(), k.fine_r.end(), 0);
  size_t third = 0;
  for (size_t x : k.ring_third) third += x;
  const bool give = c.knobs.ring3_on && tcfg.reg && tcfg.exact && third > 0 && (k.ring_elems + third) * 4 <= std::min<size_t>(h->mem_budget, (size_t)12 << 30);
  k.ring3.assign(k.tiled.size(), -1);
  if (give)
    for (size_t q = 0; q < k.tiled.size(); ++q) { k.ring3[q] = (int64_t)k.ring_elems; k.ring_elems += k.ring_third[q]; }
}

int widen_resumed(AlignCall& c) {
  wfm_handle* h = c.h;
  Chunk& k = c.ck;
  if (h->ring.ensure(k.ring_elems + 16) || h->bpjobs.ensure(k.jobs.size()) || h->bpres.ensure(k.jobs.size())) {
    h->err = "out of device memory (ring arena)"; return WFM_E_NOMEM;
  }
  c.ring_peak = std::max(c.ring_peak, k.ring_elems);
  k.resume_bad.assign(k.jobs.size(), 0);
  if (k.tiled_r.empty()) return WFM_OK;
  std::vector<RingWidenJob> wj;
  int maxw_dst = 0;
  for (size_t q = 0; q < k.tiled_r.size(); ++q) {
    BpJob& j = k.jobs[(size_t)k.tiled_r[q]];
    const GrownSnap& sn = c.snaps.v[(size_t)k.snap_r[q] - 1];
    wj.push_back(RingWidenJob{sn.d, h->ring.p + j.ring_off, sn.w, sn.koff, j.width, j.koff, -(sn.s0 + 8), sn.s0 + 8});
    maxw_dst = std::max(maxw_dst, j.width);
    j.resume_s = sn.s0; j.resume_sr = -1; j.fmax0 = sn.fmax; j.rmax0 = sn.rmax;
  }
  if (h->widenjobs.ensure(wj.size())) { h->err = "out of device memory (ring arena)"; return WFM_E_NOMEM; }
  HIPCHK(h, hipMemcpyAsync(h->widenjobs.p, wj.data(), wj.size() * sizeof(RingWidenJob), hipMemcpyHostToDevice, h->stream));
  launch_ring_widen(h->widenjobs.p, (int)wj.size(), maxw_dst, c.RR, h->stream);
  HIPCHK(h, hipGetLastError());
  HIPCHK(h, hipStreamSynchronize(h->stream));
  for (int32_t id : k.snap_r) c.snaps.drop(id);
  return WFM_OK;
}

int run_chunk_tiles(AlignCall& c) {
  wfm_handle* h = c.h;
  Chunk& k = c.ck;
  const TileCfg& tcfg = c.tcfg;
  double tms = 0; uint64_t tcells = 0;
  const auto tw0 = std::chrono::steady_clock::now();
  ReuseCtl ru;
  ru.store = &c.keeps; ru.slack = c.knobs.reuse_slack; ru.min_blocks = c.knobs.reuse_min_blocks;
  ru.use = k.reuse; ru.upto = k.keep_upto;
  for (size_t q = 0; q < k.tiled.size(); ++q) {
    const Node& nd = c.bp_nodes[(size_t)k.node_of[(size_t)k.tiled[q]]];
    ru.meet.push_back(nd.score_rem != INT_MAX ? nd.score_rem / 2 : 0);
  }
  {
    std::vector<ReuseKeeper> kp;
    for (size_t q = 0; q < k.tiled.size(); ++q) {
      const BpJob& j = k.jobs[(size_t)k.tiled[q]];
      if (k.keep_upto[q] > 0) kp.push_back(ReuseKeeper{j.pl, j.tl, k.keep_upto[q] == INT_MAX ? (j.pl + j.tl) / 16 : k.keep_upto[q]});
    }
    c.keeps.cap_bytes = h->mem_budget / 8;
    const int chunk_blocks = std::max(1, std::min(tcfg.chunk, (int)h->tile_ev.size() / 2));
    ru.cadence = kp.empty() ? 0 : reuse_fit_cadence(kp.data(), kp.size(), reuse_cadence(c.knobs.reuse_every, chunk_blocks), tcfg.T, c.keeps.cap_bytes);
  }
  const bool any_reuse = ru.cadence > 0 || std::any_of(ru.use.begin(), ru.use.end(), [](const ReuseUse& u) { return u.keep > 0; });
  int rc = run_tiled_phase(h, c.S, c.dp, c.scope, tcfg, tcfg.T, false, k.jobs, k.tiled, k.ring2, tms, tcells, c.level, &k.fine_from, &k.ring3, any_reuse ? &ru : nullptr);
  k.reuse_bad.assign(k.jobs.size(), 0);
  k.kept[0].assign(k.jobs.size(), {}); k.kept[1].assign(k.jobs.size(), {});
  if (any_reuse && !ru.bad.empty())
    for (size_t q = 0; q < k.tiled.size(); ++q) {
      k.reuse_bad[(size_t)k.tiled[q]] = ru.bad[q];
      for (int d = 0; d < 2; ++d) k.kept[d][(size_t)k.tiled[q]].swap(ru.kept[d][q]);
    }
  c.keep_bytes += ru.keep_bytes; c.restore_bytes += ru.restore_bytes;
  if (rc == WFM_OK && tcfg.T_refine > 0 && tcfg.T_refine < tcfg.T && !(tcfg.reg && tcfg.exact))
    rc = run_tiled_phase(h, c.S, c.dp, c.scope, tcfg, tcfg.T_refine, true, k.jobs, k.tiled, k.ring2, tms, tcells, c.level);
  if (rc == WFM_OK && !k.tiled_r.empty()) {
    std::vector<int> from_s(k.tiled_r.size());
    for (size_t q = 0; q < k.tiled_r.size(); ++q) from_s[q] = k.jobs[(size_t)k.tiled_r[q]].resume_s;
    rc = run_tiled_phase(h, c.S, c.dp, c.scope, tcfg, tcfg.T, true, k.jobs, k.tiled_r, k.ring2_r, tms, tcells, c.level, &k.fine_r);
    for (size_t q = 0; rc == WFM_OK && q < k.tiled_r.size(); ++q) {
      BpJob& j = k.jobs[(size_t)k.tiled_r[q]];
      const bool exact_end = j.resume_s >= 0 && j.resume_sr >= 0;
      if (tcfg.reg && tcfg.exact && ((exact_end && std::min(j.resume_s, j.resume_sr) - from_s[q] < c.knobs.resume_margin) || (j.resume_s >= 0 && j.resume_sr < 0 && j.resume_s == from_s[q]))) {
        j.resume_s = -3; j.resume_sr = -1;
        k.resume_bad[(size_t)k.tiled_r[q]] = 1;
      }
      k.tiled.push_back(k.tiled_r[q]); k.ring2.push_back(k.ring2_r[q]);
    }
  }
  c.wall_tile += std::chrono::duration<double, std::milli>(std::chrono::steady_clock::now() - tw0).count();
  if (rc != WFM_OK) return rc;
  c.tm.bp_ms += tms; c.tm.tile_ms += tms;
  h->stats.cells_bp += tcells; h->stats.cells_tile += tcells;
  return WFM_OK;
}

int run_chunk_p2(AlignCall& c) {
  wfm_handle* h = c.h;
  Chunk& k = c.ck;
  k.res.assign(k.jobs.size(), BpResult{});
  k.rest.clear(); k.more_set.clear();
  std::vector<int> cand;
  std::vector<int64_t> other;
  std::vector<char> is_cand(k.jobs.size(), 0);
  if (c.knobs.p2_on && c.tcfg.reg && c.tcfg.exact)
    for (size_t q = 0; q < k.tiled.size(); ++q) {
      const BpJob& j = k.jobs[(size_t)k.tiled[q]];
      if (j.resume_s >= 0 && j.resume_sr >= 0) { cand.push_back(k.tiled[q]); other.push_back(k.ring2[q]); is_cand[(size_t)k.tiled[q]] = 1; }
    }
  double pms = 0;
  k.carry.assign(k.jobs.size(), BpResult{});
  k.has_carry.assign(k.jobs.size(), 0);
  std::vector<int> cand_r = cand, again;
  std::vector<int64_t> other_r = other;
  for (int round = 1; !cand_r.empty(); ++round) {
    again.clear();
    const int rc = run_p2_phase(h, c.S, c.dp, c.scope, c.tcfg, k.jobs, cand_r, other_r, k.res, pms, k.carry, k.has_carry, round < c.knobs.p2_rounds, again);
    if (rc != WFM_OK) return rc;
    std::vector<int> c2; std::vector<int64_t> o2;
    for (int a : again) {
      c2.push_back(cand_r[(size_t)a]); o2.push_back(other_r[(size_t)a]);
      if (c.pflags) c.pflags[c.bp_nodes[(size_t)k.node_of[(size_t)cand_r[(size_t)a]]].prob] |= WFM_PF_P2_ROUNDS;
    }
    h->stats.p2_again += (uint32_t)again.size();
    cand_r.swap(c2); other_r.swap(o2);
  }
  c.tm.bp_ms += pms;
  for (size_t q = 0; q < k.jobs.size(); ++q)
    if (!is_cand[q] || k.res[q].status == WFM_DEV_P2_MORE) { k.rest.push_back((int)q); h->stats.p2_more += is_cand[q]; if (is_cand[q]) k.more_set.push_back((int)q); }
  if (c.pflags)
    for (size_t q = 0; q < k.jobs.size(); ++q)
      if (is_cand[q] && k.res[q].status == WFM_DEV_P2_MORE) c.pflags[c.bp_nodes[(size_t)k.node_of[q]].prob] |= WFM_PF_P2_ROUNDS;
  return WFM_OK;
}

int run_chunk_step(AlignCall& c) {
  wfm_handle* h = c.h;
  Chunk& k = c.ck;
  const std::vector<int>& rest = k.rest;
  if (rest.empty()) return WFM_OK;
  auto is_more = [&](int q) { return std::find(k.more_set.begin(), k.more_set.end(), q) != k.more_set.end(); };
  int threads = 1024;
  if (k.maxw <= 1024) threads = 256;
  else if (k.maxw <= 8192) threads = 512;
  std::vector<BpJob> rj(rest.size());
  for (size_t q = 0; q < rest.size(); ++q) rj[q] = k.jobs[(size_t)rest[q]];
  HIPCHK(h, hipMemcpyAsync(h->bpjobs.p, rj.data(), rj.size() * sizeof(BpJob), hipMemcpyHostToDevice, h->stream));
  HIPCHK(h, hipEventRecord(h->ev0, h->stream));
  launch_bp(c.S->d_seq, h->ring.p, h->bpjobs.p, h->bpres.p, (int)rj.size(), threads, c.dp, c.scope, c.RR, h->stream);
  HIPCHK(h, hipGetLastError());
  HIPCHK(h, hipEventRecord(h->ev1, h->stream));
  std::vector<BpResult> rr(rj.size());
  HIPCHK(h, hipMemcpyAsync(rr.data(), h->bpres.p, rr.size() * sizeof(BpResult), hipMemcpyDeviceToHost, h->stream));
  HIPCHK(h, hipStreamSynchronize(h->stream));
  float ms = 0;
  HIPCHK(h, hipEventElapsedTime(&ms, h->ev0, h->ev1));
  c.tm.bp_ms += ms;
  if (h->call_base) {
    float t0 = 0;
    HIPCHK(h, hipEventElapsedTime(&t0, h->call_base, h->ev0));
    h->bp_iv.emplace_back(t0, t0 + ms);
  }
  h->stats.bp_launches++;
  for (size_t q = 0; q < rest.size(); ++q) {
    if (rr[q].status == WFM_DEV_P2_NOTHING) {
      const uint64_t cl = rr[q].cells; const int32_t st = rr[q].steps;
      rr[q] = k.carry[(size_t)rest[q]]; rr[q].cells = cl; rr[q].steps = st;
    }
    k.res[(size_t)rest[q]] = rr[q];
  }
  if (c.knobs.debug) {
    uint64_t cl = 0; double t1 = 0, t2 = 0; int64_t st1 = 0, st = 0; uint32_t m1 = 0, m2 = 0;
    for (const BpResult& r : rr) { cl += r.cells; t1 += r.ticks_p1; t2 += r.ticks_p2; st1 += r.steps_p1; st += r.steps; m1 = std::max(m1, r.ticks_p1); m2 = std::max(m2, r.ticks_p2); }
    fprintf(stderr, "[wfm] level %u: %zu bp jobs (step kernel), %d thr, %.3f ms, cells %.3e, avg steps p1 %.0f p2 %.0f, avg ms p1 %.3f p2 %.3f, max ms p1 %.3f p2 %.3f\n", c.level, rr.size(), threads, ms,
            (double)cl, (double)st1 / rr.size(), (double)(st - st1) / rr.size(), t1 / rr.size() / 1e5, t2 / rr.size() / 1e5, m1 / 1e5, m2 / 1e5);
    if (c.knobs.debug > 1) {
      std::vector<size_t> ord(rr.size());
      for (size_t q = 0; q < ord.size(); ++q) ord[q] = q;
      std::sort(ord.begin(), ord.end(), [&](size_t a, size_t b) { return rr[a].ticks_p1 + rr[a].ticks_p2 > rr[b].ticks_p1 + rr[b].ticks_p2; });
      for (size_t q = 0; q < std::min<size_t>(3, ord.size()); ++q) {
        const BpResult& r = rr[ord[q]];
        const BpJob& j = rj[ord[q]];
        fprintf(stderr, "[wfm]   slow step-kernel job: pl %d tl %d width %d band %d sub %d resume %d/%d (%s), status %d score %d = %d + %d, steps p1 %d p2 %d, ms p1 %.3f p2 %.3f\n", j.pl, j.tl, j.width,
                j.band, j.sub == SUB_NONE ? -1 : j.sub, j.resume_s, j.resume_sr, is_more(rest[ord[q]]) ? "phase-2 walk ran out of rows" : (j.resume_sr >= 0 ? "exact" : "not exact"), r.status,
                r.score, r.score_fwd, r.score_rev, r.steps_p1, r.steps - r.steps_p1, r.ticks_p1 / 1e5, r.ticks_p2 / 1e5);
      }
    }
  }
  return WFM_OK;
}

int keep_snapshot(AlignCall& c, size_t q, Node& again) {
  wfm_handle* h = c.h;
  const BpJob& j = c.ck.jobs[q];
  if (c.ck.resume_bad[q] || c.ck.res[q].status != WFM_DEV_BAND || j.resume_s != -3 || j.resume_sr < 0 || j.sub != SUB_NONE || j.band <= 0) return WFM_OK;
  GrownSnap sn;
  sn.s0 = j.resume_sr; sn.fmax = j.fmax0; sn.rmax = j.rmax0;
  const int reach = sn.s0 + 8;
  sn.koff = reach + 4;
  sn.koff += ((j.koff - sn.koff) % 4 + 4) % 4;
  sn.w = (sn.koff + reach + 5 + 3) & ~3;
  if (wfm_dmalloc((void**)&sn.d, ring_elems((size_t)sn.w, c.RR) * sizeof(int32_t)) != hipSuccess) { (void)hipGetLastError(); sn.d = nullptr; }
  if (!sn.d) return WFM_OK;
  const RingWidenJob wj{h->ring.p + j.ring_off, sn.d, j.width, j.koff, sn.w, sn.koff, -reach, reach};
  c.snaps.v.push_back(sn);
  again.snap = (int32_t)c.snaps.v.size();
  if (h->widenjobs.ensure(1)) { h->err = "out of device memory (ring arena)"; return WFM_E_NOMEM; }
  HIPCHK(h, hipMemcpyAsync(h->widenjobs.p, &wj, sizeof(wj), hipMemcpyHostToDevice, h->stream));
  launch_ring_widen(h->widenjobs.p, 1, sn.w, c.RR, h->stream);
  HIPCHK(h, hipGetLastError());
  HIPCHK(h, hipStreamSynchronize(h->stream));
  return WFM_OK;
}

void push_children(AlignCall& c, const Node& nd, const BpResult& r, int bp_v, int bp_h, size_t q) {
  const wfm_penalties_t* pen = c.pen;
  Node a{}, b{};
  a.prob = nd.prob; a.pb = nd.pb; a.pl = bp_v; a.tb = nd.tb; a.tl = bp_h;
  const int slack = c.knobs.slack_env >= 0 ? c.knobs.slack_env : 2 * std::max(pen->o1, pen->o2) + 8;
  a.sub = (int)std::min<int64_t>((int64_t)r.score_fwd + slack, SUB_NONE);
  b.sub = (int)std::min<int64_t>((int64_t)r.score_rev + slack, SUB_NONE);
  a.hinted = 0; b.hinted = 0;
  a.cb = nd.cb; a.ce = r.comp; a.score_rem = r.score_fwd;
  b.prob = nd.prob; b.pb = nd.pb + bp_v; b.pl = nd.pl - bp_v; b.tb = nd.tb + bp_h; b.tl = nd.tl - bp_h;
  b.cb = r.comp; b.ce = nd.ce; b.score_rem = r.score_rev;
  for (Node* ch : {&a, &b}) {
    if (ch->pl == 0 || ch->tl == 0) { ch->smax = 0; c.base_nodes.push_back(*ch); }
    else if (ch->score_rem <= BIALIGN_FALLBACK_MIN_SCORE) {
      const int open_end = ch->ce == C_M ? 0 : ((ch->ce == C_I1 || ch->ce == C_D1) ? pen->o1 : pen->o2);
      ch->smax = std::max(ch->score_rem, 0) + open_end;
      c.base_nodes.push_back(*ch);
    }
    else {
      const int d = ch == &a ? 0 : 1;
      std::vector<int32_t>& kept = c.ck.kept[d][q];
      if (!kept.empty()) {
        ++c.reuse_children;
        std::vector<int32_t> kept_s(kept.size());
        for (size_t x = 0; x < kept.size(); ++x) kept_s[x] = c.keeps.v[(size_t)kept[x] - 1].s0;
        const int pick = ch->sub != SUB_NONE ? reuse_pick_keep(kept_s.data(), kept_s.size(), ch->score_rem, c.tcfg.T, c.knobs.fine_margin, c.knobs.reuse_min_blocks) : -1;
        if (pick >= 0) { ch->keep = kept[(size_t)pick]; ch->keep_dir = d; kept[(size_t)pick] = 0; ++c.reuse_found; }
      }
      c.next_bp.push_back(*ch);
    }
  }
}

void dump_failed_problem(AlignCall& c, const Node& nd, const char* dd) {
  const ProbMeta& pm = c.S->meta[nd.prob];
  std::vector<char> pb((size_t)pm.plen), tb((size_t)pm.tlen);
  (void)hipMemcpy(pb.data(), c.S->d_seq + pm.p_fwd, pb.size(), hipMemcpyDeviceToHost);
  (void)hipMemcpy(tb.data(), c.S->d_seq + pm.t_fwd, tb.size(), hipMemcpyDeviceToHost);
  static std::atomic<int> nfail{0};
  const std::string fn = std::string(dd) + "/fail_" + std::to_string(nfail.fetch_add(1)) + ".txt";
  if (FILE* f = fopen(fn.c_str(), "w")) {
    fprintf(f, "%d %d %d\n", pm.plen, pm.tlen, pm.hint);
    fwrite(pb.data(), 1, pb.size(), f); fputc('\n', f);
    fwrite(tb.data(), 1, tb.size(), f); fputc('\n', f);
    fclose(f);
  }
}

int settle_chunk(AlignCall& c) {
  wfm_handle* h = c.h;
  Chunk& k = c.ck;
  h->stats.bp_jobs += (uint32_t)k.jobs.size();
  for (size_t q = 0; q < k.jobs.size(); ++q) {
    const Node nd = c.bp_nodes[(size_t)k.node_of[q]];
    const BpResult& r = k.res[q];
    c.prob_cells[nd.prob] += r.cells;
    h->stats.cells_bp += r.cells;
    if (nd.score_rem == INT_MAX && k.jobs[q].band > 0 && !k.grown_job[q]) { ++c.roots_banded; c.roots_out += r.status == WFM_DEV_BAND; }
    c.keeps.drop(nd.keep);
    if (k.reuse_bad[q]) {
      Node again = nd; again.keep = 0; again.keep_dir = 0;
      c.next_bp.push_back(again);
      continue;
    }
    if (nd.limit > 0 && !(r.status == 1 || (r.status == 0 && r.score <= nd.limit))) {
      const BpJob& j = k.jobs[q];
      const bool beyond = r.status == WFM_DEV_LIMIT || r.status == 0 || (r.status == WFM_DEV_BAND && j.band == 0) ||
                          (r.status == WFM_DEV_BAND && j.resume_s == -3 && j.resume_sr >= 0 && !k.resume_bad[q] &&
                           tile_job_beyond_limit(j.pl, j.tl, j.sub, j.limit, j.resume_sr, c.tcfg.T));
      if (beyond) { c.prob_status[nd.prob] = WFM_ST_MAX_SCORE; ++c.limit_out; continue; }
      if (r.status == WFM_DEV_BAND) {
        Node again = nd; again.noband = 1; again.band = j.band; again.snap = 0; again.keep = 0; again.keep_dir = 0;
        if (c.pflags) c.pflags[nd.prob] |= WFM_PF_ROOT_AGAIN;
        const bool full_fits = ring_elems(ring_full_width(nd.pl, nd.tl), c.RR) * 4 <= h->mem_budget;
        if (!full_fits && c.pflags) c.pflags[nd.prob] |= WFM_PF_RING_GROWN;
        c.next_bp.push_back(again);
        c.band_retries += full_fits;
        continue;
      }
    }
    const bool guessed = nd.hinted && k.jobs[q].sub != SUB_NONE;
    if (r.status == WFM_DEV_BAND || (guessed && (r.status < 0 || (r.status == 0 && r.score > nd.sub)))) {
      Node again = nd; again.noband = 1; again.sub = SUB_NONE; again.hinted = 0;
      again.band = k.jobs[q].band; again.snap = 0; again.keep = 0; again.keep_dir = 0;
      if (c.pflags) c.pflags[nd.prob] |= nd.score_rem == INT_MAX ? WFM_PF_ROOT_AGAIN : WFM_PF_JOB_AGAIN;
      const bool full_fits = ring_elems(ring_full_width(nd.pl, nd.tl), c.RR) * 4 <= h->mem_budget;
      if (!full_fits) {
        if (c.pflags) c.pflags[nd.prob] |= WFM_PF_RING_GROWN;
        if (k.resume_bad[q]) again.band = nd.band;
        const int rc = keep_snapshot(c, q, again);
        if (rc != WFM_OK) return rc;
      }
      static const bool same_level = getenv("WFM_RETRY_SAME_LEVEL") && atoi(getenv("WFM_RETRY_SAME_LEVEL")) != 0;
      if (guessed || !same_level) c.next_bp.push_back(again); else c.bp_nodes.push_back(again);
// ... 1719 lines not shown
```

### wfmash_amd/csrc/wfa_kernels.hip

```cpp
#include <hip/hip_runtime.h>
#include <stdint.h>
#include <algorithm>
#include <cstdlib>
#include <type_traits>

#include "wfa_device.h"
#include "wfa_base.h"

namespace wfm {

#ifdef WFM_PROFILE_SECTIONS
__device__ long long g_sec[8];
#define SEC_T(v) const long long v = clock64(); asm volatile("" ::: "memory")
#define SEC_ADD(i, a, b) sec[i] += (b) - (a)
#else
#define SEC_T(v)
#define SEC_ADD(i, a, b)
#endif

__device__ __forceinline__ uint64_t load8(const uint8_t* p) {
  uint64_t v;
  __builtin_memcpy(&v, p, 8);
  return v;
}
// ... 529 lines not shown
      I2h[c] = nI2[c]; D2h[c] = nD2[c];
    }
    mak = wave_max_dpp63(mak);
    if (lane == 63 && mak > 0) atomicMax(&s_makr[t], mak);
  }
  }
  if (P2) return;
  const int s_end = s0 + Tn;
  if (Tn < H) {
#pragma unroll
    for (int c = 0; c < C; ++c) {
      const int k = k0 + c;
      if (k < tk.core_lo || k > tk.core_hi) continue;
      for (int d = Tn; d < H; ++d) {
        const int sc = s_end - d;
        if (sc < 0 || k < rlo(sc) || k > rhi(sc)) continue;
        const int64_t ro = ((int64_t)(sc & RMASK)) * width + k;
        rout[(int64_t)C_I1 * RING * width + ro] = rin[(int64_t)C_I1 * RING * width + ro];
        rout[(int64_t)C_I2 * RING * width + ro] = rin[(int64_t)C_I2 * RING * width + ro];
        rout[(int64_t)C_D1 * RING * width + ro] = rin[(int64_t)C_D1 * RING * width + ro];
        rout[(int64_t)C_D2 * RING * width + ro] = rin[(int64_t)C_D2 * RING * width + ro];
      }
    }
  }
  auto write_rows = [&](auto TR) {
    constexpr int tr = decltype(TR)::value;
#pragma unroll
    for (int c = 0; c < C; ++c) {
      const int k = k0 + c;
      if (k < tk.core_lo || k > tk.core_hi) continue;
#pragma unroll
      for (int d = 0; d < H; ++d) {
        const int r = ((tr - d) % NCL + NCL) % NCL;
        const int back = ((tr - r) % NCL + NCL) % NCL;
        const int e = (d - back) / NCL;
        const int sc = s_end - d;
        if (sc >= 0 && k >= rlo(sc) && k <= rhi(sc)) rout[((int64_t)(C_M * RING + (sc & RMASK))) * width + k] = Mh[c][r][e];
      }
    }
  };
  switch (Tn % NCL) {
    case 0: write_rows(std::integral_constant<int, 0>{}); break;
    case 1: write_rows(std::integral_constant<int, 1>{}); break;
    case 2: write_rows(std::integral_constant<int, 2>{}); break;
    case 3: write_rows(std::integral_constant<int, 3>{}); break;
    default: write_rows(std::integral_constant<int, 4>{}); break;
  }
  __syncthreads();
  int32_t* mk = mak_out + ((int64_t)tk.job * 2 + dir) * T;
  for (int t = 1 + tid; t <= T; t += NT) if (s_makr[t] > 0) atomicMax(&mk[t - 1], s_makr[t]);
}

__global__ __launch_bounds__(64) void wfa_tile_advance_kernel(TileJob* __restrict__ jobs, int32_t* __restrict__ mak, int njobs, int T, DevPen pen,
                                                              int exact, int coarse, int launched) {
  const int i = blockIdx.x, lane = threadIdx.x;
  if (i >= njobs) return;
  TileJob J = jobs[i];
  if (!J.active) return;
  if (coarse && (J.packed & 1)) {
    const bool job_fine = J.mode == 5 || (J.mode == 0 && J.s0 + T >= J.fine_s);
    if (launched != 2 && !(launched & (job_fine ? 2 : 1))) return;
  }
  int32_t* mf = mak + ((int64_t)i * 2 + 0) * T;
  int32_t* mr = mak + ((int64_t)i * 2 + 1) * T;
  if (J.mode == 1) {
    for (int t = lane; t < T; t += 64) { mf[t] = 0; mr[t] = 0; }
    if (lane == 0) {
      const int64_t t = J.ring_in; J.ring_in = J.ring_out; J.ring_out = t;
      J.mode = 2; J.active = 0; J.nblocks += 1;
      jobs[i] = J;
    }
    return;
  }
  if (J.mode == 6) {
    for (int t = lane; t < T; t += 64) { mf[t] = 0; mr[t] = 0; }
    if (lane == 0) {
      const int64_t t = J.ring_in; J.ring_in = J.ring_out; J.ring_out = t;
      J.mode = 1; J.reran += 1;
      jobs[i] = J;
    }
    return;
  }
  const int A = J.pl + J.tl - 1;
  int fm = J.fmax, rm = J.rmax;
  int tf = 0, tr = 0, last_fwd = 0;
  bool term = false;
  for (int base = 0; base < T && !term; base += 64) {
    const int t = base + lane;
    const int vf = t < T ? mf[t] : 0, vr = t < T ? mr[t] : 0;
    int pf = vf, pr = vr;
#pragma unroll
    for (int d = 1; d < 64; d <<= 1) {
      const int uf = __shfl_up(pf, d, 64), ur = __shfl_up(pr, d, 64);
      if (lane >= d) { pf = max(pf, uf); pr = max(pr, ur); }
    }
    int er = __shfl_up(pr, 1, 64);
    if (lane == 0) er = 0;
    const int fm_t = max(fm, pf), rm_t = max(rm, pr), rm_before = max(rm, er);
    const bool hit_f = t < T && fm_t + rm_before >= A, hit_r = t < T && fm_t + rm_t >= A;
    const unsigned long long bf = __ballot(hit_f), br = __ballot(hit_r);
    if (bf | br) {
      const int lf = bf ? __builtin_ctzll(bf) : 64, lr = br ? __builtin_ctzll(br) : 64;
      term = true;
      if (lf <= lr) { last_fwd = 1; tf = base + lf + 1; tr = base + lf; fm = __shfl(fm_t, lf, 64); rm = __shfl(rm_before, lf, 64); }
      else { last_fwd = 0; tf = tr = base + lr + 1; fm = __shfl(fm_t, lr, 64); rm = __shfl(rm_t, lr, 64); }
    } else {
      fm = __shfl(fm_t, 63, 64); rm = __shfl(rm_t, 63, 64);
    }
  }
  for (int t = lane; t < T; t += 64) { mf[t] = 0; mr[t] = 0; }
  if (lane != 0) return;
  const int64_t max_steps = (int64_t)(pen.o1 + pen.o2) * 4 + (int64_t)(J.pl + J.tl + 2) * max(pen.x, max(pen.e1, pen.e2)) * 2 + 256;
  J.nblocks += 1;
  const bool was_coarse = coarse && (launched & 1) && (J.packed & 1) && J.mode == 0 && J.s0 + T < J.fine_s;
  if (term && exact && was_coarse) {
    J.mode = 5; J.fine_s = -1; J.nblocks -= 1;
  } else if (term && exact) {
    J.mode = (J.ring_prev >= 0 && J.prev_ok && min(tf, tr) < 26) ? 6 : 1;
    J.tf = tf; J.tr = tr; J.last_fwd = last_fwd;
    J.fmax = fm; J.rmax = rm;
  } else if (term || 2 * (int64_t)(J.s0 + T) > max_steps) {
    J.active = 0;
  } else {
    J.fmax = fm; J.rmax = rm;
    J.s0 += T;
    J.mode = 0;
    if (J.ring_prev >= 0) {
      const int64_t t = J.ring_prev; J.ring_prev = J.ring_in; J.ring_in = J.ring_out; J.ring_out = t;
      J.prev_ok = 1;
    } else {
      const int64_t t = J.ring_in; J.ring_in = J.ring_out; J.ring_out = t;
    }
  }
  jobs[i] = J;
}

__device__ __forceinline__ void keep_row(int r, int& comp, int& back) {
  if (r < SNAP_ROWS) { comp = C_M; back = r; return; }
  const int q = r - SNAP_ROWS;
  comp = q < 2 ? C_I1 : (q < 4 ? C_D1 : (q == 4 ? C_I2 : C_D2));
  back = q < 4 ? (q & 1) : 0;
}
__global__ __launch_bounds__(256) void wfa_keep_kernel(const int32_t* __restrict__ ring, const TileJob* __restrict__ jobs, const KeepTask* __restrict__ tasks) {
  const KeepTask t = tasks[blockIdx.y];
  const int x = blockIdx.x * 256 + threadIdx.x;
  if (x >= t.n) return;
  const TileJob J = jobs[t.job];
  if (!J.active || J.mode != 0 || J.s0 != t.expect_s) return;
  const int k = t.kmin + x;
  const Rng RG = make_rng(J.pl, J.tl, J.sub);
  const int64_t width = J.width;
  const int32_t* rin = ring + J.ring_in + J.koff + (int64_t)t.dir * 5 * RING * width;
#pragma unroll 4
  for (int r = 0; r < KEEP_ROWS; ++r) {
    int comp, back;
    keep_row(r, comp, back);
    const int sc = J.s0 - back;
    const bool ok = sc >= 0 && k >= rng_lo(RG, sc) && k <= rng_hi(RG, sc);
    t.dst[(int64_t)r * t.n + x] = ok ? rin[((int64_t)(comp * RING + (sc & RMASK))) * width + k] : WF_NULL;
  }
}
__global__ __launch_bounds__(256) void wfa_restore_kernel(int32_t* __restrict__ ring, const TileJob* __restrict__ jobs, const RestoreTask* __restrict__ tasks,
                                                          int32_t* __restrict__ out) {
  const RestoreTask t = tasks[blockIdx.y];
  const int x = blockIdx.x * 256 + threadIdx.x;
  const TileJob J = jobs[t.job];
  int touch = 0, mak = 0;
  if (x < t.n && J.s0 == t.s_k) {
    const int k = t.kmin + x;
    if (k >= -J.pl && k <= J.tl) {
      const Rng RG = make_rng(J.pl, J.tl, J.sub);
      const int64_t width = J.width;
      int32_t* rin = ring + J.ring_in + J.koff + (int64_t)t.dir * 5 * RING * width;
      const int wall = min(J.tl, J.pl + k) - t.slack;
      for (int r = 0; r < KEEP_ROWS; ++r) {
        int comp, back;
        keep_row(r, comp, back);
        const int sc = t.s_k - back;
        if (sc < 0 || k < rng_lo(RG, sc) || k > rng_hi(RG, sc)) continue;
        const int v = t.src[(int64_t)r * t.n + x];
        rin[((int64_t)(comp * RING + (sc & RMASK))) * width + k] = v;
        touch |= v >= wall;
        if (comp == C_M && v >= 0) mak = max(mak, 2 * v - k);
      }
    }
  }
  if (__any(touch) && (threadIdx.x & 63) == 0) atomicOr(&out[2 * blockIdx.y], 1);
  mak = wave_max_dpp63(mak);
  if ((threadIdx.x & 63) == 63 && mak > 0) atomicMax(&out[2 * blockIdx.y + 1], mak);
}
void launch_keep(const int32_t* ring, const TileJob* jobs, const KeepTask* tasks, int ntasks, int max_n, hipStream_t st) {
  if (ntasks <= 0 || max_n <= 0) return;
  for (int t0 = 0; t0 < ntasks; t0 += 32768)
    hipLaunchKernelGGL(wfa_keep_kernel, dim3((max_n + 255) / 256, std::min(32768, ntasks - t0)), dim3(256), 0, st, ring, jobs, tasks + t0);
}
void launch_restore(int32_t* ring, const TileJob* jobs, const RestoreTask* tasks, int32_t* out, int ntasks, int max_n, hipStream_t st) {
  if (ntasks <= 0 || max_n <= 0) return;
  for (int t0 = 0; t0 < ntasks; t0 += 32768)
    hipLaunchKernelGGL(wfa_restore_kernel, dim3((max_n + 255) / 256, std::min(32768, ntasks - t0)), dim3(256), 0, st, ring, jobs, tasks + t0, out + 2 * t0);
}

__device__ __forceinline__ const int32_t* p2_row(const int32_t* ring, const int32_t* p2, const P2Job& J, int d, int cc, int s) {
  const int sd = d == 0 ? J.sf : J.sr;
  if (s <= sd) return ring + J.ring_in + J.koff + ((int64_t)((d * 5 + cc) * RING + (s & RMASK))) * J.width;
  return p2 + J.p2_off + J.koff2 + ((int64_t)((d * 5 + cc) * P2K + (s - sd - 1))) * J.w2;
}
__device__ __forceinline__ const int32_t* p2_maxrow(const int32_t* p2max, int job, const P2Job& J, int d, int s) {
  const int sd = d == 0 ? J.sf : J.sr;
  return p2max + (((int64_t)job * 2 + d) * P2ROWS + (s - (sd - 25))) * 5;
}
__global__ __launch_bounds__(256) void wfa_p2_blockmax_kernel(const int32_t* __restrict__ ring, const int32_t* __restrict__ p2,
                                                             const P2Job* __restrict__ jobs, int32_t* __restrict__ bmax,
                                                             int32_t* __restrict__ p2max) {
  const int job = blockIdx.x / (2 * P2ROWS), r2 = blockIdx.x % (2 * P2ROWS), d = r2 / P2ROWS, r = r2 % P2ROWS;
  const P2Job J = jobs[job];
// ... 671 lines not shown
```

### wfmash_amd/csrc/wfa_plan.h

```cpp
#ifndef WFM_WFA_PLAN_H_
#define WFM_WFA_PLAN_H_
#include <stddef.h>
#include <stdint.h>
#include <string.h>

#include <algorithm>
#include <climits>
#include <vector>

#include "../../include/wfmash_hip.h"
#include "wfa_rows.h"

namespace wfm {

struct Node {
  int32_t prob;
  int32_t pb, pl, tb, tl;
  int32_t cb, ce;
  int32_t score_rem;
  int32_t smax;
  int32_t endsfree;
  int32_t noband;
  int32_t sub;
  int32_t hinted;
  int32_t tries;
  int32_t band;
  int32_t snap;
  int32_t keep;
  int32_t keep_dir;
  int32_t limit;
};

inline size_t ring_full_width(int pl, int tl) { return ((size_t)pl + tl + 9 + 3) & ~(size_t)3; }
inline size_t ring_col_bytes(int RR) { return (size_t)2 * 5 * RR * 4; }
inline size_t ring_elems(size_t w, int RR, int rings = 1) { return w * 2 * 5 * RR * rings; }

struct BandGeometry { int64_t shift; size_t width; int koff; };
inline BandGeometry band_geometry(int pl, int tl, int64_t b) {
  const int64_t shift = std::max<int64_t>(0, ((int64_t)pl - (b + 8)) & ~(int64_t)3);
  const int64_t right = std::min<int64_t>(tl, b + 8);
  return BandGeometry{shift, ((size_t)((int64_t)pl - shift + right + 9) + 3) & ~(size_t)3, (int)(pl + 4 - shift)};
}

struct RingRules {
  bool tiles = true;
  int min_len = 128, min_score = 64, chunk = 2, T = 100;
  int RR = 32;
  size_t mem_budget = 0;
  int band_root = 4096;
  bool use_band = false, over_budget = false, roots_off = false;
};
struct RingPlan {
  bool fits = true;
  size_t width = 0;
  int koff = 0, band = 0;
  bool tile_it = false;
  bool grown = false;
  size_t need = 0;
};

inline RingPlan plan_ring(const Node& nd, const RingRules& r) {
  RingPlan p;
  const size_t full_width = ring_full_width(nd.pl, nd.tl);
  p.width = full_width;
  p.koff = nd.pl + 4;
  p.tile_it = r.tiles && nd.pl + nd.tl >= r.min_len && (nd.score_rem == INT_MAX || nd.score_rem >= r.min_score);
  const bool tiles_take_it = p.tile_it;
  const bool known = nd.score_rem != INT_MAX || nd.sub != SUB_NONE;
  if (r.use_band && (known || r.over_budget) && p.tile_it && !nd.noband && !(r.roots_off && nd.score_rem == INT_MAX)) {
    int64_t dir_scores = nd.score_rem == INT_MAX ? (int64_t)r.band_root : (int64_t)nd.score_rem / 2 + 64;
    if (nd.score_rem == INT_MAX && nd.sub != SUB_NONE) dir_scores = std::min<int64_t>(dir_scores, ((int64_t)nd.sub + 128) / 2 + 64);
    const int64_t b = dir_scores + (int64_t)r.chunk * r.T + 16;
    const BandGeometry g = band_geometry(nd.pl, nd.tl, b);
    if (g.shift > 0 && g.width * 2 <= full_width) { p.band = (int)b; p.width = g.width; p.koff = g.koff; }
  }
  if (p.tile_it && ring_elems(p.width, r.RR, 2) * 4 > r.mem_budget) p.tile_it = false;
  p.need = ring_elems(p.width, r.RR, p.tile_it ? 2 : 1);
  if (p.need * 4 > r.mem_budget) {
    const size_t col_bytes = ring_col_bytes(r.RR);
    const int64_t first = nd.score_rem == INT_MAX ? (int64_t)r.band_root : (int64_t)nd.score_rem / 2 + 64 + (int64_t)r.chunk * r.T + 16;
    int64_t nb = nd.band > 0 ? std::max<int64_t>(4 * (int64_t)nd.band, first) : first;
    BandGeometry g = band_geometry(nd.pl, nd.tl, nb);
    p.fits = g.width < full_width;
    if (p.fits && g.width * col_bytes > r.mem_budget) {
      nb = ((int64_t)(r.mem_budget / col_bytes) - 32) / 2;
      p.fits = nb > (int64_t)nd.band && nb >= 64;
      if (p.fits) { g = band_geometry(nd.pl, nd.tl, nb); p.fits = g.width < full_width && g.width * col_bytes <= r.mem_budget; }
    }
    if (!p.fits) return p;
    p.grown = true;
    p.band = (int)nb; p.width = g.width; p.koff = g.koff;
    p.tile_it = tiles_take_it && ring_elems(p.width, r.RR, 2) * 4 <= r.mem_budget;
    p.need = ring_elems(p.width, r.RR, p.tile_it ? 2 : 1);
  }
  return p;
}

inline int64_t cells_sum(int pl, int tl, int sub, int a, int b) {
  if (b < a) return 0;
  const Rng rg = make_rng(pl, tl, sub);
  const int64_t kinv = (int64_t)tl - pl, khi = kinv + sub, klo = kinv - sub;
  int64_t cand[16];
  int nc = 0;
  auto add = [&](int64_t x) { for (int64_t y : {x, x + 1}) if (y > a && y <= b) cand[nc++] = y; };
  add(tl); add(khi / 2 - (khi < 0 && (khi & 1) ? 1 : 0)); add(khi - tl);
  add(pl); add((-klo) / 2 - (-klo < 0 && ((-klo) & 1) ? 1 : 0)); add(-klo - pl);
  std::sort(cand, cand + nc);
  int64_t total = 0;
  int64_t u = a;
  auto cells = [&](int64_t s) { return (int64_t)rng_hi(rg, (int)s) - rng_lo(rg, (int)s) + 1; };
  auto seg = [&](int64_t x, int64_t y) {
    if (y < x) return;
    const int64_t cx = cells(x), cy = cells(y);
    if (cx <= 0 && cy <= 0) return;
    if (cx > 0 && cy > 0) { total += (cx + cy) * (y - x + 1) / 2; return; }
    if (y == x) { total += std::max<int64_t>(cx, 0); return; }
    const int64_t slope = (cy - cx) / (y - x);
    if (cx > 0) {
      const int64_t last = x + (cx - 1) / (-slope);
      total += (cx + cells(last)) * (last - x + 1) / 2;
    } else {
      const int64_t first = y - (cy - 1) / slope;
      total += (cells(first) + cy) * (y - first + 1) / 2;
    }
  };
  for (int q = 0; q < nc; ++q) {
    if (cand[q] <= u) continue;
    seg(u, cand[q] - 1);
    u = cand[q];
  }
  seg(u, b);
  return total;
}

struct TilePlanJob { int pl, tl, sub, s0, mode, fine_s, packed, active; };
struct TilePlanRules {
  int threads = 512, C = 2, T = 100, chunk = 2;
  int core = 0;
  bool reg = true;
  bool fine = true;
  bool coarse_on = false;
};
struct TileChunkPlan {
  std::vector<int> threads_b, variants_b;
  int core_c = 0;
  std::vector<TileTask> tasks, tasks_by;
  size_t n_pk = 0;
};

inline bool tile_job_leaves(int pl, int tl, int sub, int s0, int band, int chunk, int T) {
  if (band > 0 && s0 + chunk * T + 2 > band) return true;
  if (sub == SUB_NONE) return false;
  int L, R;
  rng_block(make_rng(pl, tl, sub), s0, s0 + T, L, R);
  return 2 * s0 > sub + 128 || R < L;
}
inline bool tile_job_beyond_limit(int pl, int tl, int sub, int limit, int s0, int T) {
  if (limit <= 0) return false;
  if (s0 >= limit) return true;
  int L, R;
  rng_block(make_rng(pl, tl, sub), s0, s0 + T, L, R);
  return 2 * s0 > sub + 128 || R < L;
}

inline bool fits_one_tile(int widest, int threads, int C) { return widest <= threads * C; }
inline int one_tile_threads(int widest, int threads, int C) { return std::min(threads, std::max(64, ((widest + C - 1) / C + 63) / 64 * 64)); }

inline void append_tile_tasks(TileChunkPlan& p, int job, int dir, int ntiles, int core, bool packed, int dirs = 3) {
  if (!((dirs >> dir) & 1)) return;
  std::vector<TileTask>& to = packed ? p.tasks : p.tasks_by;
  for (int t = 0; t < ntiles; ++t) to.push_back(TileTask{(int32_t)job, dir, t, core});
}
inline void close_task_list(TileChunkPlan& p) {
  p.n_pk = p.tasks.size();
  p.tasks.insert(p.tasks.end(), p.tasks_by.begin(), p.tasks_by.end());
}

inline void plan_tile_chunk(const TilePlanJob* jobs, size_t n, const TilePlanRules& r, TileChunkPlan& p, const uint8_t* dirs = nullptr) {
  const int chunk = r.chunk, T = r.T;
  auto block_range = [&](const TilePlanJob& j, int b, int& L, int& R) { rng_block(make_rng(j.pl, j.tl, j.sub), j.s0 + b * T, j.s0 + (b + 1) * T, L, R); };
  p.tasks.clear(); p.tasks_by.clear();
  p.core_c = r.core;
  p.threads_b.assign((size_t)chunk, r.threads);
  if (r.reg && r.C == 2) {
    std::vector<int> wb((size_t)chunk, 0);
    for (size_t i = 0; i < n; ++i) {
      if (!jobs[i].active) continue;
      int wmax = 0;
      for (int b = 0; b < chunk; ++b) {
        int L, R;
        block_range(jobs[i], b, L, R);
        wmax = std::max(wmax, R - L + 1);
        wb[(size_t)b] = std::max(wb[(size_t)b], wmax);
      }
    }
    if (fits_one_tile(wb[(size_t)chunk - 1], r.threads, r.C)) {
      for (int b = 0; b < chunk; ++b) {
        const int wdt = r.fine ? wb[(size_t)b] : wb[(size_t)chunk - 1];
        p.threads_b[(size_t)b] = r.fine ? one_tile_threads(wdt, r.threads, r.C) : std::min(r.threads, wdt <= 256 ? 128 : (wdt <= 512 ? 256 : r.threads));
      }
      p.core_c = p.threads_b[(size_t)chunk - 1] * r.C;
    }
  }
  for (size_t i = 0; i < n; ++i) {
    if (!jobs[i].active) continue;
    int ntiles = 0;
    for (int b = 0; b < chunk; ++b) {
      int L, R;
      block_range(jobs[i], b, L, R);
      ntiles = std::max(ntiles, tiles_for(L, R, p.core_c));
    }
    for (int d = 0; d < 2; ++d) append_tile_tasks(p, (int)i, d, ntiles, p.core_c, jobs[i].packed != 0, dirs ? dirs[i] : 3);
  }
  close_task_list(p);
  p.variants_b.assign((size_t)chunk, r.coarse_on ? 0 : 2);
  if (!r.coarse_on) return;
  for (size_t i = 0; i < n; ++i) {
    const TilePlanJob& j = jobs[i];
    if (!j.active || !(j.packed & 1)) continue;
    for (int b = 0; b < chunk; ++b) {
      const bool reaches = (int64_t)j.s0 + (int64_t)(b + 1) * T >= (int64_t)j.fine_s;
      if ((j.mode == 5 && b == 0) || (j.mode == 0 && reaches)) p.variants_b[(size_t)b] |= 2;
      if (j.mode == 0 && !reaches) p.variants_b[(size_t)b] |= 1;
    }
  }
  for (int b = 0; b < chunk; ++b) if (!p.variants_b[(size_t)b]) p.variants_b[(size_t)b] = 2;
}

inline int reuse_cadence(int every, int chunk) { return (std::max(1, every) + chunk - 1) / chunk * chunk; }
inline int reuse_resume_limit(int score_rem, int T, int fine_margin) {
  const int64_t x = (int64_t)score_rem / 2 - fine_margin;
  return x < 0 ? -1 : (int)(x / T * T - T);
}
inline int reuse_pick_keep(const int32_t* kept_s, size_t n, int score_rem, int T, int fine_margin, int min_blocks = 1) {
  if (score_rem == INT_MAX) return -1;
  const int limit = reuse_resume_limit(score_rem, T, fine_margin);
  const int64_t least = (int64_t)std::max(1, min_blocks) * T;
  int best = -1;
  for (size_t i = 0; i < n; ++i)
    if (kept_s[i] >= least && kept_s[i] <= limit && (best < 0 || kept_s[i] > kept_s[(size_t)best])) best = (int)i;
  return best;
}
inline bool reuse_ranges_contained(int ppl, int ptl, int psub, int cpl, int ctl, int csub, int s_k) {
  const Rng P = make_rng(ppl, ptl, psub), Cc = make_rng(cpl, ctl, csub);
  for (int s = std::max(0, s_k - RNG_BACK); s <= s_k; ++s) {
    const int lo = rng_lo(Cc, s), hi = rng_hi(Cc, s);
    if (hi < lo) continue;
    if (lo < rng_lo(P, s) || hi > rng_hi(P, s)) return false;
  }
  return true;
}
inline bool reuse_eligible(const Node& nd, const RingPlan& rp, int ppl, int ptl, int psub, int child_sub, int s_k, int T) {
  if (nd.keep <= 0 || nd.score_rem == INT_MAX || nd.sub == SUB_NONE || !rp.fits || !rp.tile_it || rp.band != 0 || rp.grown) return false;
  if (s_k < T || s_k % T != 0) return false;
  return reuse_ranges_contained(ppl, ptl, psub, nd.pl, nd.tl, child_sub, s_k);
}
inline bool reuse_keep_wanted(int es, int64_t s_meet, int cadence, int T) {
  if (s_meet <= 0) return false;
  return 100 * (int64_t)es >= 40 * s_meet - 100 * (64 + (int64_t)(2 + cadence) * T) && 100 * (int64_t)es <= 60 * s_meet;
}
inline int64_t reuse_meet_estimate(int s0, int64_t mak, int64_t A) { return s0 <= 0 || mak <= 0 ? 0 : (int64_t)s0 * A / mak; }
inline int reuse_keep_kmin(int pl, int s) { return std::max(-pl, -s); }
inline int reuse_keep_cols(int pl, int tl, int s) { return std::min(tl, s) - std::max(-pl, -s) + 1; }
inline size_t reuse_keep_elems(int pl, int tl, int s) { return (size_t)KEEP_ROWS * (size_t)reuse_keep_cols(pl, tl, s); }
struct ReuseKeeper { int pl, tl, upto; };
inline int reuse_fit_cadence(const ReuseKeeper* jobs, size_t n, int cadence, int T, size_t cap_bytes) {
  int upto_max = 0;
  for (size_t i = 0; i < n; ++i) upto_max = std::max(upto_max, jobs[i].upto);
  for (; (int64_t)cadence * T <= upto_max; cadence *= 2) {
    size_t bytes = 0;
    for (size_t i = 0; i < n && bytes <= cap_bytes; ++i)
      for (int64_t s = (int64_t)cadence * T; s <= jobs[i].upto && bytes <= cap_bytes; s += (int64_t)cadence * T) bytes += 2 * 4 * reuse_keep_elems(jobs[i].pl, jobs[i].tl, (int)s);
    if (bytes <= cap_bytes) return cadence;
  }
  return 0;
}

struct P2PlanJob { int pl, tl, sub, sf, sr, packed; };
struct P2Geometry {
  int koff2; size_t w2, nblk;
  size_t p2_off, bm_off;
};
struct P2ChunkPlan {
  std::vector<P2Geometry> geo;
  size_t elems = 0, bm_elems = 0, maxw2 = 0;
  int threads_c = 0;
  TileChunkPlan tiles;
};
inline void plan_p2_chunk(const P2PlanJob* cand, size_t n_cand, size_t i0, int rows, int rows_bm, size_t budget, int threads, int core, P2ChunkPlan& p) {
  p.geo.clear(); p.elems = 0; p.bm_elems = 0; p.maxw2 = 0;
  p.tiles.tasks.clear(); p.tiles.tasks_by.clear();
  for (size_t i = i0; i < n_cand; ++i) {
    const P2PlanJob& j = cand[i];
    const int reach = std::max(j.sf, j.sr) + rows;
    int L, R;
    rng_block(make_rng(j.pl, j.tl, j.sub), std::max(0, std::min(j.sf, j.sr) - P2_BACK), reach, L, R);
    if (R < L) { L = 0; R = 0; }
    P2Geometry g;
    g.koff2 = ((-L + 4) + 3) & ~3;
    g.w2 = ((size_t)(R + g.koff2 + 8) + 3) & ~(size_t)3;
    g.nblk = (g.w2 >> 6) + 1;
    const size_t need = g.w2 * 2 * 5 * rows, need_bm = g.nblk * 2 * rows_bm * 5;
    if (!p.geo.empty() && (p.elems + need + 2 * (p.bm_elems + need_bm)) * 4 > budget) break;
    p.maxw2 = std::max(p.maxw2, g.w2);
    g.p2_off = p.elems; g.bm_off = p.bm_elems;
    p.bm_elems += need_bm;
    p.elems += need;
    p.geo.push_back(g);
  }
  const size_t n = p.geo.size();
  auto dir_range = [&](const P2PlanJob& j, int d, int& L, int& R) { rng_block(make_rng(j.pl, j.tl, j.sub), d == 0 ? j.sf : j.sr, (d == 0 ? j.sf : j.sr) + rows, L, R); };
  p.threads_c = threads; p.tiles.core_c = core;
  int widest = 0;
  for (size_t q = 0; q < n; ++q)
    for (int d = 0; d < 2; ++d) {
      int L, R;
      dir_range(cand[i0 + q], d, L, R);
      widest = std::max(widest, R - L + 1);
    }
  if (fits_one_tile(widest, threads, 2)) {
    p.threads_c = one_tile_threads(widest, threads, 2);
    p.tiles.core_c = p.threads_c * 2;
  }
  for (size_t q = 0; q < n; ++q)
    for (int d = 0; d < 2; ++d) {
      int L, R;
      dir_range(cand[i0 + q], d, L, R);
      append_tile_tasks(p.tiles, (int)q, d, tiles_for(L, R, p.tiles.core_c), p.tiles.core_c, cand[i0 + q].packed != 0);
    }
  close_task_list(p.tiles);
}

inline void base_columns(const Node& nd, int pbf, int pef, int tbf, int tef, bool corner_band, int64_t* kmin_out, int64_t* kmax_out) {
  int64_t kmin = nd.endsfree ? std::max<int64_t>(-nd.pl, -(int64_t)pbf - nd.smax) : std::max<int64_t>(-nd.pl, -nd.smax);
  int64_t kmax = nd.endsfree ? std::min<int64_t>(nd.tl, (int64_t)tbf + nd.smax) : std::min<int64_t>(nd.tl, nd.smax);
  const bool end_fixed = !nd.endsfree || (pef == 0 && tef == 0);
  if (corner_band && end_fixed) {
    const int64_t k_end = (int64_t)nd.tl - nd.pl;
    const int64_t bmin = std::max(kmin, k_end - nd.smax), bmax = std::min(kmax, k_end + nd.smax);
    const int64_t lo0 = nd.endsfree ? std::max<int64_t>(-(int64_t)pbf, bmin) : 0, hi0 = nd.endsfree ? std::min<int64_t>((int64_t)tbf, bmax) : 0;
    if (bmin <= bmax && lo0 <= hi0 && lo0 >= bmin && hi0 <= bmax) { kmin = bmin; kmax = bmax; }
  }
  *kmin_out = kmin; *kmax_out = kmax;
}

struct BaseRules {
  bool base_v2 = true;
  bool base_tiles = true;
  bool force_tiles = false;
  bool few_jobs = false;
  int wide_from = 2048;
};
inline int base_kind(int64_t width, int pl, int tl, int tries, bool acgt, const BaseRules& r) {
  if (r.base_v2 && (pl == 0 || tl == 0)) return 1;
  if (r.base_v2 && width <= 2048 && acgt)
    return width <= 128 ? 0 : (r.base_tiles && (r.force_tiles || (r.few_jobs && (tries > 0 || width > 640))) ? 5 : (width <= 640 ? 1 : 2));
  if (r.base_v2 && r.base_tiles && acgt) return 5;
  return width > r.wide_from ? 4 : 3;
// ... 67 lines not shown
```

### wfmash_amd/csrc/wfa_tile2.hip

```cpp
#include <hip/hip_runtime.h>
#include <stdint.h>
#include <type_traits>

#include "wfa_device.h"
#include "wfa_base.h"
#include "wfa_pack.h"

#ifdef WFM_TILE_TRACE
__device__ unsigned long long g_tile_trace[48 * 16 * 128 * 4];
extern "C" int wfm_debug_tile_trace(unsigned long long* out, size_t n) {
  return (int)hipMemcpyFromSymbol(out, HIP_SYMBOL(g_tile_trace), n * sizeof(unsigned long long), 0, hipMemcpyDeviceToHost);
}
#if WFM_TILE_TRACE == 1
#define WFM_TRACE_STAMP(slot_) do { if (trace_on) { const unsigned long long ts_ = __builtin_readcyclecounter(); if (lane == 0) g_tile_trace[(((size_t)blockIdx.x * 16 + wv) * 128 + (t & 127)) * 4 + (slot_)] = ts_; } } while (0)
#else
#define WFM_TRACE_STAMP(slot_) do { } while (0)
#endif
#define WFM_TRACE_MARK(idx_) do { if (WFM_TILE_TRACE == 2 && trace_on2) { const unsigned long long ts_ = __builtin_readcyclecounter(); if (lane == 0) g_tile_trace[(((size_t)blockIdx.x * 16 + wv) * 128 + (idx_)) * 4] = ts_; } } while (0)
#else
#define WFM_TRACE_STAMP(slot_) do { } while (0)
#define WFM_TRACE_MARK(idx_) do { } while (0)
#endif

namespace wfm {
// ... 201 lines not shown
  uint32_t v = 0;
  if ((i + 1) * 16 <= nbytes) {
    const uint4 q = *reinterpret_cast<const uint4*>(seq + i * 16);
    const uint32_t w[4] = {q.x, q.y, q.z, q.w};
#pragma unroll
    for (int j = 0; j < 4; ++j) {
      const uint32_t c = (w[j] >> 1) & 0x03030303u;
      v |= ((c & 3u) | ((c >> 6) & 0xcu) | ((c >> 12) & 0x30u) | ((c >> 18) & 0xc0u)) << (8 * j);
    }
  } else {
    for (int j = 0; j < 16; ++j) {
      const int64_t a = i * 16 + j;
      const uint32_t c = a < nbytes ? (uint32_t)seq[a] : 0u;
      v |= pack_code((uint8_t)c) << (2 * j);
    }
  }
  pk[i] = v;
}
__global__ __launch_bounds__(256) void seq_acgt_kernel(const uint8_t* __restrict__ seq, const SeqRev* __restrict__ jobs, int32_t* __restrict__ flag) {
  const SeqRev J = jobs[blockIdx.x >> 1];
  const bool text = blockIdx.x & 1;
  const uint8_t* src = seq + (text ? J.t_fwd : J.p_fwd);
  const int n = text ? J.tlen : J.plen;
  bool bad = false;
  for (int q = threadIdx.x; q < n; q += blockDim.x) {
    const uint8_t c = src[q];
    bad |= !pack_is_acgt(c);
  }
  if (__any(bad) && (threadIdx.x & 63) == 0) flag[blockIdx.x >> 1] = 0;
}
void launch_seq_pack(const uint8_t* seq, uint32_t* pk, int64_t nwords, int64_t nbytes, const SeqRev* jobs, int njobs, int32_t* flag, hipStream_t st) {
  if (nwords > 0) hipLaunchKernelGGL(seq_pack_kernel, dim3((unsigned)((nwords + 255) / 256)), dim3(256), 0, st, seq, pk, nwords, nbytes);
  if (njobs > 0) hipLaunchKernelGGL(seq_acgt_kernel, dim3((unsigned)njobs * 2), dim3(256), 0, st, seq, jobs, flag);
}

template <int NTMAX, bool P2, bool FAST, bool FINE = true, int MS = 0>
__global__ __launch_bounds__(NTMAX) void wfa_tile2_kernel(const uint32_t* __restrict__ pk, int32_t* __restrict__ ring_arena,
                                                        const TileJob* __restrict__ jobs, const TileTask* __restrict__ tasks,
                                                        int32_t* __restrict__ mak_out, int T, int32_t* __restrict__ p2_arena, int coarse) {
  constexpr int C = 2, LB = 25, H = LB + 1, NCL = 5, DEP = 6, E1 = 2;
  constexpr bool WAVE1 = NTMAX == 64;
  constexpr bool PIPE = FAST && !P2;
  constexpr bool SLOTS = FAST && FINE && !P2;
  static_assert(!SLOTS || (MS >= 2 && MS <= 64 && (MS & (MS - 1)) == 0), "slots per score: a power of two within a wave");
  __shared__ __attribute__((aligned(16))) int s_edge[2][WAVE1 ? 1 : 17][2][4];
  __shared__ __attribute__((aligned(16))) uint32_t s_winP[PK_WIN_DW + PK_SLACK_DW], s_winT[PK_WIN_DW + PK_SLACK_DW];
  __shared__ int s_wlo[2];
  extern __shared__ __attribute__((aligned(16))) int s_makr[];
  TileTask tk = tasks[blockIdx.x];
  const TileJob J = jobs[tk.job];
  if (!J.active) return;
  const int sbase = P2 ? (tk.dir == 0 ? J.tf : J.tr) : (J.mode == 6 ? J.s0 - T : J.s0);
  const Rng RG = make_rng(J.pl, J.tl, J.sub);
  const bool lowdiv = (J.packed & 2) != 0;
  int halo = T;
  {
    const int s1 = sbase + T;
    int L, R;
    rng_block(RG, sbase, s1, L, R);
    const int idx = tk.core_lo, core = tk.core_hi;
    tk.core_lo = L + idx * core;
    tk.core_hi = min(R, tk.core_lo + core - 1);
    if (tk.core_lo > R) return;
    if (tk.core_lo == L && tk.core_hi == R) halo = 0;
  }
  const int dir = tk.dir, tid = threadIdx.x, lane = tid & 63, wv = tid >> 6;
  const int kA = tk.core_lo - halo;
  const int nw = min((int)(blockDim.x >> 6), (tk.core_hi + halo - kA) / (64 * C) + 1), NT = nw * 64;
  if (wv >= nw) return;
#ifdef WFM_TILE_TRACE
  const bool trace_on2 = !P2 && FAST && !WAVE1 && gridDim.x >= 512 && blockIdx.x < 48 && sbase == 4000 && J.mode == 0;
#endif
  WFM_TRACE_MARK(120);
  if (tid < 2) s_wlo[tid] = INT32_MAX;
  if (!WAVE1) for (int i = tid; i < (int)(sizeof(s_edge) / sizeof(int)); i += NT) ((int*)s_edge)[i] = WF_NULL;
  const int64_t aP = dir == 0 ? J.p_fwd : J.p_rev, aT = dir == 0 ? J.t_fwd : J.t_rev;
  const int pl = J.pl, tl = J.tl, s0 = sbase;
  const int k0 = kA + tid * C;
  const int64_t width = J.width;
  const int32_t* rin = ring_arena + ((!P2 && J.mode == 6) ? J.ring_prev : J.ring_in) + J.koff + (int64_t)dir * 5 * RING * width;
  int32_t* rout = ring_arena + J.ring_out + J.koff + (int64_t)dir * 5 * RING * width;
  const int kmax = tk.core_hi + halo;
  const int Tn = (!P2 && J.mode == 1) ? (dir == 0 ? J.tf : J.tr) : T;
  const int t_stream = Tn - ((J.mode == 1 || J.mode == 6 || J.ring_prev < 0) ? H : E1);
  if (!P2 && FAST && !(coarse & 2)) {
    const bool fine = !(coarse & 1) || J.mode == 5 || (J.mode == 0 && sbase + T >= J.fine_s);
    if (fine != FINE) return;
  }
  __shared__ int s_run[(!P2 && FAST && !FINE) ? NTMAX : 1];
  if (!P2 && FAST && !FINE) s_run[tid] = 0;

  int Mh[C][NCL][DEP];
  int I1h[C][E1], D1h[C][E1], I2h[C], D2h[C];
  const bool lean_on = (coarse & 4) != 0;
  if (lean_on && tile_wave_lean_load(RG, __builtin_amdgcn_readfirstlane(k0), kmax, s0)) {
    const int32_t* const wrow = rin + __builtin_amdgcn_readfirstlane(k0);
    const unsigned lofs = (unsigned)lane * (unsigned)(C * sizeof(int32_t));
    auto ld_lean = [&](int comp, int sc, int& a, int& b) {
      ld_pair(reinterpret_cast<const int32_t*>(reinterpret_cast<const char*>(wrow + ((int64_t)(comp * RING + (sc & RMASK))) * width) + lofs), a, b);
    };
#pragma unroll
    for (int d = 0; d < H; ++d) ld_lean(C_M, s0 - d, Mh[0][(NCL - d % NCL) % NCL][d / NCL], Mh[1][(NCL - d % NCL) % NCL][d / NCL]);
#pragma unroll
    for (int r = 1; r < NCL; ++r) { Mh[0][r][DEP - 1] = WF_NULL; Mh[1][r][DEP - 1] = WF_NULL; }
#pragma unroll
    for (int d = 0; d < E1; ++d) {
      ld_lean(C_I1, s0 - d, I1h[0][d], I1h[1][d]);
      ld_lean(C_D1, s0 - d, D1h[0][d], D1h[1][d]);
    }
    ld_lean(C_I2, s0, I2h[0], I2h[1]);
    ld_lean(C_D2, s0, D2h[0], D2h[1]);
  } else {
    __builtin_amdgcn_s_waitcnt(0x0F70);
    const bool kin0 = k0 <= kmax, kin1 = k0 + 1 <= kmax;
#pragma unroll
    for (int c = 0; c < C; ++c)
#pragma unroll
      for (int r = 0; r < NCL; ++r)
#pragma unroll
        for (int e = 0; e < DEP; ++e) Mh[c][r][e] = WF_NULL;
    auto ld_row = [&](int comp, int sc, int& a, int& b) {
      const int lo = rng_lo(RG, sc), hi = rng_hi(RG, sc);
      const bool ok0 = kin0 && sc >= 0 && k0 >= lo && k0 <= hi, ok1 = kin1 && sc >= 0 && k0 + 1 >= lo && k0 + 1 <= hi;
      int x = WF_NULL, y = WF_NULL;
      if (ok0 || ok1) ld_pair(rin + ((int64_t)(comp * RING + (sc & RMASK))) * width + k0, x, y);
      a = ok0 ? x : WF_NULL; b = ok1 ? y : WF_NULL;
    };
#pragma unroll
    for (int d = 0; d < H; ++d)
      ld_row(C_M, s0 - d, Mh[0][(NCL - d % NCL) % NCL][d / NCL], Mh[1][(NCL - d % NCL) % NCL][d / NCL]);
#pragma unroll
    for (int d = 0; d < E1; ++d) {
      ld_row(C_I1, s0 - d, I1h[0][d], I1h[1][d]);
      ld_row(C_D1, s0 - d, D1h[0][d], D1h[1][d]);
    }
    ld_row(C_I2, s0, I2h[0], I2h[1]);
    ld_row(C_D2, s0, D2h[0], D2h[1]);
  }
  if (FINE && !P2) for (int t = tid; t < (SLOTS ? (T + 1) * MS : T + 1); t += NT) s_makr[t] = 0;
  unsigned mk_off = (unsigned)(lane & (MS - 1)) * 4u;
  auto slot_max = [&](int j, int mak) {
    (void)__hip_atomic_fetch_max(static_cast<int*>(__builtin_assume_aligned(reinterpret_cast<char*>(s_makr) + mk_off, 4)) + j * MS, mak, __ATOMIC_RELAXED, __HIP_MEMORY_SCOPE_WORKGROUP);
  };
  unsigned hmaxu[C];
  int s_last[C];
  int negk[C];
  bool incore[C];
#pragma unroll
  for (int c = 0; c < C; ++c) {
    const int k = k0 + c;
    const bool colok = (k >= -pl) && (k <= tl);
    hmaxu[c] = colok ? (unsigned)min(tl, pl + k) : 0u;
    s_last[c] = colok ? min(k - RG.kb_lo, RG.kb_hi - k) : -1;
    incore[c] = k >= tk.core_lo && k <= tk.core_hi;
    negk[c] = incore[c] ? -k : -(1 << 29);
  }
  {
    int hlo = INT32_MAX, vlo = INT32_MAX;
#pragma unroll
    for (int c = 0; c < C; ++c) {
      const int k = k0 + c;
      int lo = INT32_MAX;
#pragma unroll
      for (int r = 0; r < NCL; ++r)
#pragma unroll
        for (int e = 0; e < DEP; ++e) lo = min(lo, Mh[c][r][e] >= 0 ? Mh[c][r][e] : INT32_MAX);
#pragma unroll
// ... 1001 lines not shown
```

### wfmash_amd/host/capi_host.cpp

```cpp
#include <algorithm>
#include <exception>
#include <iostream>
#include <string>
#include <thread>
#include <vector>

#include "../../include/wfmash_host.h"
#include "../csrc/wfa_handle.h"
#include "../csrc/wfa_pack.h"
#include "../csrc/wfa_plan.h"
#include "../csrc/wfa_optband.h"
#include "aligner.hpp"
#include "fasta.hpp"
#include "map_stats.hpp"

extern "C" {

int wfmh_test_packed_lce(const uint8_t* buf_p, int64_t n_p, int64_t start_p, const uint8_t* buf_t, int64_t n_t, int64_t start_t, int v, int h, int maxn) {
  if (!buf_p || !buf_t || n_p < 0 || n_t < 0 || start_p < 0 || start_t < 0 || v < 0 || h < 0) return -1;
  std::vector<uint32_t> wp((size_t)(n_p + 15) / 16 + 16, 0u), wt((size_t)(n_t + 15) / 16 + 16, 0u);
  wfm::pack_words_model(buf_p, n_p, wp.data());
  wfm::pack_words_model(buf_t, n_t, wt.data());
  const int64_t ori_p = start_p & ~(int64_t)15, ori_t = start_t & ~(int64_t)15;
  return wfm::pk_lce_model(wp.data() + (ori_p >> 4), wt.data() + (ori_t >> 4), (uint32_t)(v + (start_p - ori_p)), (uint32_t)(h + (start_t - ori_t)), maxn);
// ... 163 lines not shown
  return 0;
}

int wfmh_test_tile_lean_waves(const int32_t* in, int64_t* out) {
  const wfm::Rng r = wfm::make_rng(in[0], in[1], in[2]);
  const int s0 = in[3], T = in[4], Tn = in[5], core = in[6], threads = in[7];
  if (T < 1 || core < 1 || threads < 64) return -1;
  int L, R;
  wfm::rng_block(r, s0, s0 + T, L, R);
  const int nt = wfm::tiles_for(L, R, core);
  out[0] = nt; out[1] = out[2] = out[3] = out[4] = 0;
  for (int idx = 0; idx < nt; ++idx) {
    int lo, hi;
    wfm::tile_span(L, R, idx, core, &lo, &hi);
    const int halo = (lo == L && hi == R) ? 0 : T;
    const int kA = lo - halo, kmax = hi + halo;
    const int nw = std::min(threads / 64, (kmax - kA) / wfm::WAVE_DIAGS + 1);
    int lean_here = 0;
    for (int w = 0; w < nw; ++w) {
      const int kw = kA + w * wfm::WAVE_DIAGS;
      out[1] += 1;
      lean_here += wfm::tile_wave_lean_load(r, kw, kmax, s0) ? 1 : 0;
      out[3] += wfm::tile_wave_lean_store(r, kw, lo, hi, s0 + Tn, Tn) ? 1 : 0;
    }
    out[2] += lean_here;
    out[4] += (lean_here > 0 && lean_here < nw) ? 1 : 0;
  }
  return 0;
}

int wfmh_test_opt_band(const int64_t* in, int64_t* out) {
  if (!in || !out || in[5] < 0 || in[6] < 0 || in[11] < 0) return -1;
  const wfm::OptBand b = wfm::opt_band(wfm::OptPen{in[0], in[1], in[2], in[3], in[4]}, in[5], in[6], in[7], in[8], in[9], in[10], in[11]);
  out[0] = b.lo; out[1] = b.hi; out[2] = (int64_t)b.cells;
  return 0;
}

int wfmh_test_tile_plan(const int32_t* jobs, int64_t n, const int32_t* rules, int32_t* per_block, int32_t* tasks, int64_t tasks_cap, int64_t* scalars) {
  static_assert(sizeof(wfm::TilePlanJob) == 8 * sizeof(int32_t) && sizeof(wfm::TileTask) == 4 * sizeof(int32_t), "the hooks copy these as rows of int32");
  wfm::TilePlanRules r{rules[0], rules[1], rules[2], rules[3], rules[4], rules[5] != 0, rules[6] != 0, rules[7] != 0};
  if (r.chunk < 1 || r.T < 1 || r.threads < 1 || r.C < 1 || r.core < 1) return -1;
  wfm::TileChunkPlan p;
  wfm::plan_tile_chunk(reinterpret_cast<const wfm::TilePlanJob*>(jobs), (size_t)n, r, p);
  std::copy(p.threads_b.begin(), p.threads_b.end(), per_block);
  std::copy(p.variants_b.begin(), p.variants_b.end(), per_block + r.chunk);
  memcpy(tasks, p.tasks.data(), std::min<size_t>(p.tasks.size(), (size_t)tasks_cap) * sizeof(wfm::TileTask));
  scalars[0] = p.core_c; scalars[1] = (int64_t)p.tasks.size(); scalars[2] = (int64_t)p.n_pk;
  return 0;
}

int wfmh_test_reuse_plan(int op, const int64_t* in, int64_t n, int64_t* out) {
  if (op == 0) {
    std::vector<int32_t> kept((size_t)n);
    for (int64_t i = 0; i < n; ++i) kept[(size_t)i] = (int32_t)in[4 + i];
    out[0] = wfm::reuse_pick_keep(kept.data(), kept.size(), (int)in[0], (int)in[1], (int)in[2], (int)in[3]);
    out[1] = in[0] == INT_MAX ? -1 : wfm::reuse_resume_limit((int)in[0], (int)in[1], (int)in[2]);
    return 0;
  }
  if (op == 1) {
    wfm::Node nd{};
    nd.pl = (int32_t)in[0]; nd.tl = (int32_t)in[1]; nd.score_rem = (int32_t)in[2]; nd.keep = (int32_t)in[4];
    nd.sub = nd.score_rem == INT_MAX ? wfm::SUB_NONE : nd.score_rem + 56;
    wfm::RingPlan rp;
    rp.fits = in[5] != 0; rp.tile_it = in[6] != 0; rp.band = (int)in[7]; rp.grown = in[8] != 0;
    out[0] = wfm::reuse_eligible(nd, rp, (int)in[9], (int)in[10], (int)in[11], (int)in[3], (int)in[12], (int)in[13]);
    return 0;
  }
  if (op == 2) {
    if (in[0] < 1 || in[1] < 1 || in[2] < 1) return -1;
    std::vector<wfm::ReuseKeeper> kp((size_t)n);
    for (int64_t i = 0; i < n; ++i) kp[(size_t)i] = wfm::ReuseKeeper{(int)in[4 + 3 * i], (int)in[5 + 3 * i], (int)in[6 + 3 * i]};
    out[0] = wfm::reuse_cadence((int)in[0], (int)in[1]);
    out[1] = wfm::reuse_fit_cadence(kp.data(), kp.size(), (int)out[0], (int)in[2], (size_t)in[3]);
    return 0;
  }
  if (op == 3) {
    out[1] = wfm::reuse_meet_estimate((int)in[0], in[2], in[3]);
    out[0] = wfm::reuse_keep_wanted((int)in[1], out[1], (int)in[4], (int)in[5]);
    return 0;
  }
  return -1;
}

int wfmh_test_tile_plan_dirs(const int32_t* jobs, int64_t n, const int32_t* rules, const uint8_t* dirs, int32_t* per_block, int32_t* tasks, int64_t tasks_cap,
                             int64_t* scalars) {
  wfm::TilePlanRules r{rules[0], rules[1], rules[2], rules[3], rules[4], rules[5] != 0, rules[6] != 0, rules[7] != 0};
  if (r.chunk < 1 || r.T < 1 || r.threads < 1 || r.C < 1 || r.core < 1) return -1;
  wfm::TileChunkPlan p;
  wfm::plan_tile_chunk(reinterpret_cast<const wfm::TilePlanJob*>(jobs), (size_t)n, r, p, dirs);
  std::copy(p.threads_b.begin(), p.threads_b.end(), per_block);
  std::copy(p.variants_b.begin(), p.variants_b.end(), per_block + r.chunk);
  memcpy(tasks, p.tasks.data(), std::min<size_t>(p.tasks.size(), (size_t)tasks_cap) * sizeof(wfm::TileTask));
  scalars[0] = p.core_c; scalars[1] = (int64_t)p.tasks.size(); scalars[2] = (int64_t)p.n_pk;
  return 0;
}

int wfmh_test_p2_plan(const int32_t* cand, int64_t n, int64_t i0, int rows, int rows_bm, unsigned long long budget, int threads, int core, int64_t* geo,
                      int32_t* tasks, int64_t tasks_cap, int64_t* scalars) {
  static_assert(sizeof(wfm::P2PlanJob) == 6 * sizeof(int32_t), "the hook copies these as rows of int32");
  if (i0 < 0 || i0 >= n || rows < 1 || threads < 1 || core < 1) return -1;
  wfm::P2ChunkPlan p;
  wfm::plan_p2_chunk(reinterpret_cast<const wfm::P2PlanJob*>(cand), (size_t)n, (size_t)i0, rows, rows_bm, (size_t)budget, threads, core, p);
  for (size_t q = 0; q < p.geo.size(); ++q) {
    const wfm::P2Geometry& g = p.geo[q];
    const int64_t v[5] = {g.koff2, (int64_t)g.w2, (int64_t)g.nblk, (int64_t)g.p2_off, (int64_t)g.bm_off};
    std::copy(v, v + 5, geo + 5 * q);
  }
  memcpy(tasks, p.tiles.tasks.data(), std::min<size_t>(p.tiles.tasks.size(), (size_t)tasks_cap) * sizeof(wfm::TileTask));
  const int64_t v[8] = {(int64_t)p.geo.size(), (int64_t)p.elems, (int64_t)p.bm_elems, (int64_t)p.maxw2, p.threads_c, p.tiles.core_c,
                        (int64_t)p.tiles.tasks.size(), (int64_t)p.tiles.n_pk};
  std::copy(v, v + 8, scalars);
  return 0;
}

int wfmh_test_base_plan(int op, const int32_t* in, int64_t n, int32_t* out) {
  if (op == 0) {
    for (int64_t i = 0; i < n; ++i, in += 10)
      out[i] = wfm::base_kind(in[0], in[1], in[2], in[3], in[4] != 0, wfm::BaseRules{in[5] != 0, in[6] != 0, in[7] != 0, in[8] != 0, in[9]});
    return 0;
  }
  if (op != 1 || in[0] < 1 || in[1] * 2 <= 2 * in[0]) return -1;
  std::vector<int32_t> width((size_t)n), smax((size_t)n);
  for (int64_t i = 0; i < n; ++i) { width[(size_t)i] = in[2 + 2 * i]; smax[(size_t)i] = in[3 + 2 * i]; }
  const wfm::BaseTilePlan p = wfm::plan_base_tiles(width.data(), smax.data(), (size_t)n, in[0], in[1]);
  out[0] = p.core; out[1] = p.nblocks;
  std::copy(p.ntiles.begin(), p.ntiles.end(), out + 2);
  return 0;
}

char* wfmh_test_cigar(const char* fn, const char* a, const char* b, const char* query, const char* target,
                      long long i0, long long i1) {
  std::string f = fn ? fn : "", sa = a ? a : "", sb = b ? b : "", q = query ? query : "", t = target ? target : "";
  std::string r;
  const wflign::CigarOps o2 = wflign::parse_cigar(sb);
  wflign::CigarOps o = wflign::parse_cigar(sa);
  auto erosion = [](const wflign::Erosion& e, size_t third) { return std::to_string(e.query_eroded) + "," + std::to_string(e.target_eroded) + "," + std::to_string(third); };
  if (f == "erode") { wflign::erode_short_matches_in_cigar(o, (int)i0, i1 != 0); r = wflign::cigar_to_string(o); }
  else if (f == "merge") { wflign::merge_adjacent_ops(o, o2, 0, o2.size()); r = wflign::cigar_to_string(o); }
  else if (f == "compress") r = wflign::compress_ops(sa.data(), sa.size());
  else if (f == "swap_start") { wflign::try_swap_start_pattern(o, q.data(), (int64_t)q.size(), t.data(), (int64_t)t.size()); r = wflign::cigar_to_string(o); }
  else if (f == "swap_end") { wflign::try_swap_end_pattern(o, q.data(), (int64_t)q.size(), t.data(), (int64_t)t.size()); r = wflign::cigar_to_string(o); }
  else if (f == "head_erosion") {
    const wflign::Erosion e = wflign::scan_head_erosion(o);
    r = erosion(e, wflign::cigar_to_string(o, 0, e.erode_end_pos).size());
  } else if (f == "tail_erosion") {
    const wflign::Erosion e = wflign::scan_tail_erosion(o);
    r = erosion(e, e.erode_start_idx);
  } else if (f == "patch_plan") {
    const wflign::PatchPlan pl = wflign::plan_patches(o);
    r = erosion(pl.head, pl.head.erode_end_pos) + "," + erosion(pl.tail, pl.tail.erode_start_idx) + "," + std::to_string((int)pl.head_wanted) + "," +
        std::to_string((int)pl.tail_wanted) + "," + std::to_string((int)pl.tail_independent);
  } else if (f == "runs") {
    std::vector<uint32_t> runs;
    std::stringstream ss(sa);
    std::string item;
    while (std::getline(ss, item, ',')) if (!item.empty()) runs.push_back((uint32_t)std::stoul(item));
    wflign::ops_from_runs(runs.data(), runs.size(), o);
    r = wflign::cigar_to_string(o);
  } else if (f == "paf") {
    std::vector<std::string> p;
    std::stringstream ss(sb);
    std::string item;
    while (std::getline(ss, item, '|')) p.push_back(item);
    if (p.size() == 12) {
      wflign::PafParams pp;
      wflign::write_alignment_paf(r, o, p[0], std::stoull(p[1]), std::stoull(p[2]), std::stoull(p[3]), p[4] == "1", p[5],
// ... 86 lines not shown
```

Before: 56.05 million aligned bases/s.

## Plan BiWFA meet score from parent's known score to skip meet detection and rerun

When a child node's remaining score is known from the parent's breakpoint, the host computes the forward/reverse meet scores up front and passes them to the tile kernels. Jobs then jump directly into the exact final block instead of detecting the meet via per-score maxima and rerunning that block. The planner can also pick the coarse packed kernel variant without per-score maxima, and the fine-from threshold is disabled for planned jobs. This adds TileJob fields, a new env knob and debug counters, and relies on the planned sum exactly matching the true meet score.

```diff
diff --git a/include/wfmash_hip.h b/include/wfmash_hip.h
--- a/include/wfmash_hip.h
+++ b/include/wfmash_hip.h
@@ -241,7 +241,8 @@
   WFM_TC_REUSE_KEEPS = 10,
   WFM_TC_REUSE_TOUCHED = 11,
   WFM_TC_REUSE_FELL_OTHER = 12,
-  WFM_TILE_COUNTERS = 13
+  WFM_TC_PLANNED_ENDS = 13,
+  WFM_TILE_COUNTERS = 14
 };
 size_t wfm_get_tile_counters(const wfm_handle_t* h, uint64_t* out, size_t n);
 
diff --git a/include/wfmash_host.h b/include/wfmash_host.h
--- a/include/wfmash_host.h
+++ b/include/wfmash_host.h
@@ -88,6 +88,7 @@
                       int32_t* tasks, int64_t tasks_cap, int64_t* scalars);
 int wfmh_test_base_plan(int op, const int32_t* in, int64_t n, int32_t* out);
 int wfmh_test_reuse_plan(int op, const int64_t* in, int64_t n, int64_t* out);
+int wfmh_test_planned_meet(const int64_t* in, int64_t n, int64_t* out);
 int wfmh_test_tile_plan_dirs(const int32_t* jobs, int64_t n, const int32_t* rules, const uint8_t* dirs, int32_t* per_block, int32_t* tasks, int64_t tasks_cap,
                              int64_t* scalars);
 int wfmh_test_tile_interior(const int32_t* q, int64_t n, int32_t* out);
diff --git a/wfmash_amd/capi.py b/wfmash_amd/capi.py
--- a/wfmash_amd/capi.py
+++ b/wfmash_amd/capi.py
@@ -18,7 +18,7 @@
 WFM_PF_ROOT_AGAIN, WFM_PF_JOB_AGAIN, WFM_PF_BASE_RETRY, WFM_PF_BASE_RETRY2, WFM_PF_BYTE_KERNEL, WFM_PF_P2_ROUNDS, WFM_PF_RING_KERNEL, WFM_PF_BASE_TILES = 1, 2, 4, 8, 16, 32, 64, 128
 WFM_PF_RING_GROWN = 256
 TILE_COUNTERS = ("jobs", "exact_ends", "fine_reruns", "gap_reruns", "ring3", "blocks_coarse", "blocks_fine", "left_band",
-                 "reuse_resumed", "reuse_fallbacks", "reuse_keeps", "reuse_touched", "reuse_fell_other")
+                 "reuse_resumed", "reuse_fallbacks", "reuse_keeps", "reuse_touched", "reuse_fell_other", "planned_ends")
 
 EXPORTS = [
     "wfm_create", "wfm_destroy", "wfm_last_error", "wfm_device_name",
@@ -1169,7 +1169,7 @@
                 "wfmh_map_multi", "wfmh_align_paf_multi", "wfmh_test_winnow_model", "wfmh_test_sortlike_model", "wfmh_test_finish_records",
                 "wfmh_release_sequences", "wfmh_test_fasta_shared", "wfmh_seed_paf", "wfmh_test_deal", "wfmh_test_subwindow",
                 "wfmh_test_rows", "wfmh_test_tile_plan", "wfmh_test_p2_plan", "wfmh_test_base_plan", "wfmh_test_map_plan", "wfmh_test_filter_ordered",
-                "wfmh_test_reuse_plan", "wfmh_test_tile_plan_dirs", "wfmh_test_tile_interior", "wfmh_test_tile_lean_waves", "wfmh_set_verify", "wfmh_verify_counts", "wfmh_verify_paf", "wfmh_test_verify_parse",
+                "wfmh_test_reuse_plan", "wfmh_test_planned_meet", "wfmh_test_tile_plan_dirs", "wfmh_test_tile_interior", "wfmh_test_tile_lean_waves", "wfmh_set_verify", "wfmh_verify_counts", "wfmh_verify_paf", "wfmh_test_verify_parse",
                 "wfmh_set_verify_optimal", "wfmh_verify_optimal_counts", "wfmh_test_opt_band", "wfmh_set_left_align", "wfmh_left_align_counts", "wfmh_set_cs", "wfmh_cs_counts", "wfmh_set_variants", "wfmh_variants_counts",
                 "wfmh_set_coverage", "wfmh_coverage_counts", "wfmh_coverage_paf", "wfmh_test_coverage_bedgraph",
                 "wfmh_ani_matrix", "wfmh_ani_matrix_rows", "wfmh_free_ani_rows", "wfmh_set_ani_matrix", "wfmh_test_ani_tsv"]
diff --git a/wfmash_amd/csrc/wfa_device.h b/wfmash_amd/csrc/wfa_device.h
--- a/wfmash_amd/csrc/wfa_device.h
+++ b/wfmash_amd/csrc/wfa_device.h
@@ -66,7 +66,23 @@
   int64_t ring_prev;
   int32_t prev_ok;
   int32_t reran;
-};
+  int32_t plan_sum;
+  int32_t plan_deep;
+};
+static_assert(sizeof(TileJob) == 160, "TileJob::plan_sum and its padding behind reran: no field the tile kernels read has moved");
+__host__ __device__ inline bool tile_plan_enter(TileJob& J, int T) {
+  if (J.plan_sum <= 0) return false;
+  const int sf = (J.plan_sum + 1) / 2, sr = J.plan_sum / 2;
+  if ((sf - 1) / T * T != J.s0) return false;
+  J.tf = sf - J.s0; J.tr = sr - J.s0; J.last_fwd = J.plan_sum & 1;
+  J.mode = (J.ring_prev >= 0 && J.prev_ok && !J.plan_deep && (J.tf < J.tr ? J.tf : J.tr) < 26) ? 6 : 1;
+  return true;
+}
+__host__ __device__ inline bool tile_plan_short_next(const TileJob& J, int T) {
+  if (J.plan_sum <= 0 || !J.plan_deep || J.mode != 0) return false;
+  const int sf = (J.plan_sum + 1) / 2, sr = J.plan_sum / 2, b0 = (sf - 1) / T * T;
+  return b0 == J.s0 + T && sr - b0 < 26;
+}
 
 struct KeepTask {
   int32_t* dst;
diff --git a/wfmash_amd/csrc/wfa_generic_inc.h b/wfmash_amd/csrc/wfa_generic_inc.h
--- a/wfmash_amd/csrc/wfa_generic_inc.h
+++ b/wfmash_amd/csrc/wfa_generic_inc.h
@@ -377,7 +377,7 @@
   long long sec[8] = {0, 0, 0, 0, 0, 0, 0, 0};
   (void)sec;
 
-  for (;;) {
+  for (; !exact;) {
     if (fmax + rmax >= A) break;
     if (J.limit > 0 && sf >= J.limit) { status = WFM_DEV_LIMIT; break; }
     if (band > 0 && max(sf, sr) + 2 > band) { status = WFM_DEV_BAND; break; }
diff --git a/wfmash_amd/csrc/wfa_host.hip b/wfmash_amd/csrc/wfa_host.hip
--- a/wfmash_amd/csrc/wfa_host.hip
+++ b/wfmash_amd/csrc/wfa_host.hip
@@ -623,11 +623,14 @@
   std::vector<char> active;
   size_t n_active = 0;
   bool any_cut = false;
+  bool any_planned = false;
+  bool plan_deep = env_num("WFM_TILE_PLANNED_DEEP", 1) != 0;
   int chunk = 1;
   TilePlanRules rules;
   std::vector<TilePlanJob> pjobs;
   TileChunkPlan plan;
   uint32_t blocks = 0;
+  uint32_t launches_coarse = 0, launches_fine = 0, reruns5 = 0, reruns6 = 0;
   double lane_cells = 0;
   ReuseCtl* ru = nullptr;
   std::vector<uint8_t> dirs, own;
@@ -648,7 +651,7 @@
   p.h->tile_ctr[touched ? WFM_TC_REUSE_TOUCHED : WFM_TC_REUSE_FELL_OTHER] += 1;
 }
 
-int init_tile_jobs(TilePhase& p, const std::vector<int32_t>* fine_from, const std::vector<int64_t>* ring3) {
+int init_tile_jobs(TilePhase& p, const std::vector<int32_t>* fine_from, const std::vector<int64_t>* ring3, const std::vector<int32_t>* plan_from) {
   wfm_handle* h = p.h;
   const TileCfg& cfg = p.cfg;
   const size_t n = p.n;
@@ -664,6 +667,9 @@
     t.fine_s = (fine_from && i < fine_from->size()) ? (*fine_from)[i] : INT_MAX;
     t.ring_prev = (ring3 && i < ring3->size() && (*ring3)[i] >= 0 && (j.packed & 1) && cfg.reg && cfg.exact && !p.refine) ? (*ring3)[i] : -1;
     h->tile_ctr[WFM_TC_RING3] += t.ring_prev >= 0;
+    t.plan_sum = (plan_from && i < plan_from->size() && !p.refine && cfg.reg && cfg.exact && (j.packed & 1)) ? (*plan_from)[i] : 0;
+    t.plan_deep = (t.plan_sum > 0 && p.plan_deep) ? 1 : 0;
+    p.any_planned |= t.plan_sum > 0 && t.fine_s == INT_MAX;
   }
   if (!p.refine || T == cfg.T) h->tile_ctr[WFM_TC_JOBS] += n;
   for (size_t i = 0; i < n; ++i) p.any_cut |= p.tj[i].sub != SUB_NONE;
@@ -698,6 +704,7 @@
       p.tj[i].fmax = p.fmax[i]; p.tj[i].rmax = p.rmax[i];
       p.dirs[i] = (uint8_t)(1 << (1 - u.dir)); p.own[i] = p.dirs[i];
     }
+    for (size_t i = 0; i < n; ++i) if (p.active[i]) tile_plan_enter(p.tj[i], T);
   } else {
     for (size_t i = 0; i < n; ++i) {
       const BpJob& j = p.jobs[(size_t)p.tiled[i]];
@@ -853,6 +860,7 @@
         launch_tile2(S->d_pk, h->ring.p, h->tilejobs.p, h->tiletasks.p, h->tilemak.p, (int)n_pk, threads_b[(size_t)b], T, variants_b[(size_t)b], h->stream);
         h->tile_ctr[WFM_TC_BLOCKS_COARSE] += (variants_b[(size_t)b] & 1) != 0;
         h->tile_ctr[WFM_TC_BLOCKS_FINE] += (variants_b[(size_t)b] & 2) != 0;
+        p.launches_coarse += (variants_b[(size_t)b] & 1) != 0; p.launches_fine += (variants_b[(size_t)b] & 2) != 0;
       }
       if (tasks.size() > n_pk)
         launch_tile_reg(S->d_seq, h->ring.p, h->tilejobs.p, h->tiletasks.p + n_pk, h->tilemak.p, (int)(tasks.size() - n_pk), threads_b[(size_t)b], T, cfg.C, p.any_cut, h->stream);
@@ -896,7 +904,7 @@
     const TileJob& got = p.got[i];
     for (int bl = was.nblocks; bl < got.nblocks; ++bl) {
       const bool last_exact = got.mode == 2 && bl == got.nblocks - 1;
-      const int base = p.s_begin[i] + (last_exact ? bl - 1 : bl) * T;
+      const int base = p.s_begin[i] + ((last_exact && got.plan_sum <= 0) ? bl - 1 : bl) * T;
       for (int d = 0; d < 2; ++d) {
         if (!((p.dirs[i] >> d) & 1)) continue;
         const int steps = last_exact ? (d == 0 ? got.tf : got.tr) : T;
@@ -906,10 +914,12 @@
     if (got.fine_s == -1 && was.fine_s != -1) {
       for (int d = 0; d < 2; ++d) if ((p.dirs[i] >> d) & 1) p.tile_cells += (uint64_t)cells_sum(was.pl, was.tl, was.sub, got.s0 + 1, got.s0 + T);
       h->tile_ctr[WFM_TC_FINE_RERUNS] += 1;
+      p.reruns5 += 1;
     }
     if (got.reran > was.reran) {
       for (int d = 0; d < 2; ++d) if ((p.dirs[i] >> d) & 1) p.tile_cells += (uint64_t)cells_sum(was.pl, was.tl, was.sub, got.s0 - T + 1, got.s0);
       h->tile_ctr[WFM_TC_GAP_RERUNS] += (uint64_t)(got.reran - was.reran);
+      p.reruns6 += (uint32_t)(got.reran - was.reran);
     }
     p.tj[i] = got;
     p.active[i] = (char)(got.active != 0);
@@ -936,6 +946,7 @@
     j.resume_s = t.s0;
     j.resume_sr = -1; j.last_fwd = 0;
     h->tile_ctr[WFM_TC_EXACT_ENDS] += t.mode == 2;
+    h->tile_ctr[WFM_TC_PLANNED_ENDS] += t.mode == 2 && t.plan_sum > 0;
     h->tile_ctr[WFM_TC_LEFT_BAND] += t.mode == 3 && !(p.ru && p.ru->bad[i]);
     if (t.mode == 3) {
       j.resume_s = -3; j.resume_sr = t.s0; j.fmax0 = p.fmax[i]; j.rmax0 = p.rmax[i];
@@ -948,27 +959,28 @@
     }
     j.fmax0 = p.fmax[i]; j.rmax0 = p.rmax[i];
   }
-  if (p.cfg.debug) fprintf(stderr, "[wfm] level %u: tiled %zu jobs, %u blocks of %d scores (Wt %d), %.3f ms; %.3e cells computed on %.3e lane-steps (%.0f %% of the lanes hold a cell), %.3e of them in the result (the block in which a job's wavefronts meet runs twice)\n", level, p.n, p.blocks, p.T, p.cfg.Wt, p.tile_ms,
-                           (double)p.tile_cells - cells_before, p.lane_cells, p.lane_cells > 0 ? 100.0 * ((double)p.tile_cells - cells_before) / p.lane_cells : 0.0, (double)unique_level);
+  if (p.cfg.debug) fprintf(stderr, "[wfm] level %u: tiled %zu jobs, %u blocks of %d scores (Wt %d), %.3f ms; %.3e cells computed on %.3e lane-steps (%.0f %% of the lanes hold a cell), %.3e of them in the result (the block in which a job's wavefronts meet runs twice); launches of the packed kernel without / with per-score maxima %u / %u, mode-5 reruns %u, mode-6 reruns %u\n", level, p.n, p.blocks, p.T, p.cfg.Wt, p.tile_ms,
+                           (double)p.tile_cells - cells_before, p.lane_cells, p.lane_cells > 0 ? 100.0 * ((double)p.tile_cells - cells_before) / p.lane_cells : 0.0, (double)unique_level,
+                           p.launches_coarse, p.launches_fine, p.reruns5, p.reruns6);
 }
 
 int run_tiled_phase(wfm_handle* h, wfm_seqset* S, const DevPen& dp, int scope, const TileCfg& cfg, int T, bool refine,
                     std::vector<BpJob>& jobs, const std::vector<int>& tiled, std::vector<int64_t>& ring2,
                     double& tile_ms, uint64_t& tile_cells, uint32_t level, const std::vector<int32_t>* fine_from = nullptr,
-                    const std::vector<int64_t>* ring3 = nullptr, ReuseCtl* reuse = nullptr) {
+                    const std::vector<int64_t>* ring3 = nullptr, ReuseCtl* reuse = nullptr, const std::vector<int32_t>* plan_from = nullptr) {
   const size_t n = tiled.size();
   if (n == 0) return WFM_OK;
   const double cells_before = (double)tile_cells;
   TilePhase p{h, S, dp, scope, cfg, T, refine, jobs, tiled, ring2, tile_ms, tile_cells, n};
   p.ru = refine ? nullptr : reuse;
-  int rc = init_tile_jobs(p, fine_from, ring3);
+  int rc = init_tile_jobs(p, fine_from, ring3, plan_from);
   if (rc != WFM_OK) return rc;
   if (p.n_active) {
     HIPCHK(h, hipMemcpyAsync(h->tilejobs.p, p.tj.data(), n * sizeof(TileJob), hipMemcpyHostToDevice, h->stream));
     HIPCHK(h, hipMemsetAsync(h->tilemak.p, 0, n * 2 * (size_t)T * sizeof(int32_t), h->stream));
     p.chunk = std::max(1, std::min(cfg.chunk, (int)h->tile_ev.size() / 2));
     p.got.resize(n); p.pjobs.resize(n);
-    p.rules = TilePlanRules{cfg.threads, cfg.C, T, p.chunk, cfg.Wt - 2 * T, cfg.reg, cfg.fine, cfg.reg && cfg.exact && tile2_coarse_maxima()};
+    p.rules = TilePlanRules{cfg.threads, cfg.C, T, p.chunk, cfg.Wt - 2 * T, cfg.reg, cfg.fine, cfg.reg && cfg.exact && tile2_coarse_maxima(), p.any_planned};
     auto clk = [] { return std::chrono::steady_clock::now(); };
     auto msd = [](std::chrono::steady_clock::time_point a, std::chrono::steady_clock::time_point b) { return std::chrono::duration<double, std::milli>(b - a).count(); };
     double ms_prep = 0, ms_launch = 0, ms_wait = 0, ms_post = 0;
@@ -1159,6 +1171,7 @@
   int p2_rounds = std::max(1, num("WFM_P2_ROUNDS", 64));
   int fine_margin = num("WFM_TILE_FINE_MARGIN", 48);
   int coarse_min_blocks = num("WFM_TILE_COARSE_MIN_BLOCKS", 32), coarse_max_jobs = num("WFM_TILE_COARSE_MAX_JOBS", 128);
+  bool planned_end = num("WFM_TILE_PLANNED_END", 1) != 0 && slack_env < (1 << 28);
   bool tile_v2 = num("WFM_TILE_V2", 1) != 0;
   bool band_on = num("WFM_BAND", 1) != 0;
   int band_root = std::max(64, num("WFM_BAND_ROOT", 4096));
@@ -1178,6 +1191,7 @@
   std::vector<int> tiled, tiled_r;
   std::vector<int64_t> ring2, ring3, ring2_r;
   std::vector<int32_t> fine_from, fine_r, snap_r;
+  std::vector<int32_t> plan_from;
   std::vector<size_t> ring_third;
   std::vector<char> grown_job, resume_bad, has_carry;
   std::vector<ReuseUse> reuse;
@@ -1190,7 +1204,7 @@
     jobs.clear(); node_of.clear(); ring_elems = 0; maxw = 0;
     tiled.clear(); ring2.clear(); ring3.clear(); ring_third.clear(); fine_from.clear();
     tiled_r.clear(); ring2_r.clear(); fine_r.clear(); snap_r.clear(); grown_job.clear();
-    reuse.clear(); keep_upto.clear();
+    reuse.clear(); keep_upto.clear(); plan_from.clear();
   }
 };
 
@@ -1376,6 +1390,9 @@
       }
       if (nd.keep > 0 && use.keep == 0) c.keeps.drop(nd.keep);
       k.reuse.push_back(use);
+      const bool planned = c.knobs.planned_end && tcfg.reg && tcfg.exact && c.RR == RING &&
+                           planned_meet_eligible(nd, rp, (j.packed & 1) != 0, use.keep > 0 ? use.s_k : 0, tcfg.T);
+      k.plan_from.push_back(planned ? nd.meet : 0);
       int32_t upto = 0;
       if (reuse_on && band == 0 && !grown && (int)c.level <= c.knobs.reuse_levels && !(nd.score_rem == INT_MAX && pm.score_only())) {
         const int known = nd.score_rem != INT_MAX ? nd.score_rem : (nd.sub != SUB_NONE ? nd.sub : INT_MAX);
@@ -1393,6 +1410,7 @@
   k.end = i;
   if (k.tiled.size() > (size_t)c.knobs.coarse_max_jobs || fine_min_blocks < (int64_t)c.knobs.coarse_min_blocks) std::fill(k.fine_from.begin(), k.fine_from.end(), 0);
   if (k.tiled_r.size() > (size_t)c.knobs.coarse_max_jobs || fine_min_blocks_r < (int64_t)c.knobs.coarse_min_blocks) std::fill(k.fine_r.begin(), k.fine_r.end(), 0);
+  for (size_t q = 0; q < k.tiled.size(); ++q) if (k.plan_from[q] > 0 && k.fine_from[q] > 0) k.fine_from[q] = INT_MAX;
   size_t third = 0;
   for (size_t x : k.ring_third) third += x;
   const bool give = c.knobs.ring3_on && tcfg.reg && tcfg.exact && third > 0 && (k.ring_elems + third) * 4 <= std::min<size_t>(h->mem_budget, (size_t)12 << 30);
@@ -1452,7 +1470,7 @@
     ru.cadence = kp.empty() ? 0 : reuse_fit_cadence(kp.data(), kp.size(), reuse_cadence(c.knobs.reuse_every, chunk_blocks), tcfg.T, c.keeps.cap_bytes);
   }
   const bool any_reuse = ru.cadence > 0 || std::any_of(ru.use.begin(), ru.use.end(), [](const ReuseUse& u) { return u.keep > 0; });
-  int rc = run_tiled_phase(h, c.S, c.dp, c.scope, tcfg, tcfg.T, false, k.jobs, k.tiled, k.ring2, tms, tcells, c.level, &k.fine_from, &k.ring3, any_reuse ? &ru : nullptr);
+  int rc = run_tiled_phase(h, c.S, c.dp, c.scope, tcfg, tcfg.T, false, k.jobs, k.tiled, k.ring2, tms, tcells, c.level, &k.fine_from, &k.ring3, any_reuse ? &ru : nullptr, &k.plan_from);
   k.reuse_bad.assign(k.jobs.size(), 0);
   k.kept[0].assign(k.jobs.size(), {}); k.kept[1].assign(k.jobs.size(), {});
   if (any_reuse && !ru.bad.empty())
@@ -1613,6 +1631,8 @@
   a.cb = nd.cb; a.ce = r.comp; a.score_rem = r.score_fwd;
   b.prob = nd.prob; b.pb = nd.pb + bp_v; b.pl = nd.pl - bp_v; b.tb = nd.tb + bp_h; b.tl = nd.tl - bp_h;
   b.cb = r.comp; b.ce = nd.ce; b.score_rem = r.score_rev;
+  a.meet = planned_meet_sum(a.score_rem, *pen, a.cb, a.ce, false);
+  b.meet = planned_meet_sum(b.score_rem, *pen, b.cb, b.ce, true);
   for (Node* ch : {&a, &b}) {
     if (ch->pl == 0 || ch->tl == 0) { ch->smax = 0; c.base_nodes.push_back(*ch); }
     else if (ch->score_rem <= BIALIGN_FALLBACK_MIN_SCORE) {
diff --git a/wfmash_amd/csrc/wfa_kernels.hip b/wfmash_amd/csrc/wfa_kernels.hip
--- a/wfmash_amd/csrc/wfa_kernels.hip
+++ b/wfmash_amd/csrc/wfa_kernels.hip
@@ -635,6 +635,7 @@
     return;
   }
   const int A = J.pl + J.tl - 1;
+  const bool planned = J.plan_sum > 0;
   int fm = J.fmax, rm = J.rmax;
   int tf = 0, tr = 0, last_fwd = 0;
   bool term = false;
@@ -652,7 +653,7 @@
     const int fm_t = max(fm, pf), rm_t = max(rm, pr), rm_before = max(rm, er);
     const bool hit_f = t < T && fm_t + rm_before >= A, hit_r = t < T && fm_t + rm_t >= A;
     const unsigned long long bf = __ballot(hit_f), br = __ballot(hit_r);
-    if (bf | br) {
+    if ((bf | br) && !planned) {
       const int lf = bf ? __builtin_ctzll(bf) : 64, lr = br ? __builtin_ctzll(br) : 64;
       term = true;
       if (lf <= lr) { last_fwd = 1; tf = base + lf + 1; tr = base + lf; fm = __shfl(fm_t, lf, 64); rm = __shfl(rm_before, lf, 64); }
@@ -684,6 +685,7 @@
     } else {
       const int64_t t = J.ring_in; J.ring_in = J.ring_out; J.ring_out = t;
     }
+    tile_plan_enter(J, T);
   }
   jobs[i] = J;
 }
diff --git a/wfmash_amd/csrc/wfa_plan.h b/wfmash_amd/csrc/wfa_plan.h
--- a/wfmash_amd/csrc/wfa_plan.h
+++ b/wfmash_amd/csrc/wfa_plan.h
@@ -29,6 +29,7 @@
   int32_t keep;
   int32_t keep_dir;
   int32_t limit;
+  int32_t meet;
 };
 
 inline size_t ring_full_width(int pl, int tl) { return ((size_t)pl + tl + 9 + 3) & ~(size_t)3; }
@@ -140,6 +141,7 @@
   bool reg = true;
   bool fine = true;
   bool coarse_on = false;
+  bool planned = false;
 };
 struct TileChunkPlan {
   std::vector<int> threads_b, variants_b;
@@ -224,7 +226,7 @@
       if (j.mode == 0 && !reaches) p.variants_b[(size_t)b] |= 1;
     }
   }
-  for (int b = 0; b < chunk; ++b) if (!p.variants_b[(size_t)b]) p.variants_b[(size_t)b] = 2;
+  for (int b = 0; b < chunk; ++b) if (!p.variants_b[(size_t)b]) p.variants_b[(size_t)b] = r.planned ? 1 : 2;
 }
 
 inline int reuse_cadence(int every, int chunk) { return (std::max(1, every) + chunk - 1) / chunk * chunk; }
@@ -274,6 +276,24 @@
     if (bytes <= cap_bytes) return cadence;
   }
   return 0;
+}
+
+inline int planned_meet_sum(int score_rem, const wfm_penalties_t& pen, int comp_begin, int comp_end, bool second) {
+  if (score_rem == INT_MAX || score_rem <= 0) return 0;
+  const int cut = second ? comp_begin : comp_end;
+  const int D = cut == 0 ? 0 : ((cut == 1 || cut == 3) ? pen.o1 : pen.o2);
+  return std::max(0, score_rem - D);
+}
+struct PlannedMeet { int sf, sr, last_fwd; };
+inline PlannedMeet planned_meet_state(int sum) { return PlannedMeet{(sum + 1) / 2, sum / 2, sum & 1}; }
+inline PlannedMeet planned_meet(int score_rem, const wfm_penalties_t& pen, int comp_begin, int comp_end, bool second) {
+  return planned_meet_state(planned_meet_sum(score_rem, pen, comp_begin, comp_end, second));
+}
+inline int planned_meet_block(int sum, int T) { return ((sum + 1) / 2 - 1) / T * T; }
+inline bool planned_meet_eligible(const Node& nd, const RingPlan& rp, bool packed, int s_keep, int T) {
+  if (nd.meet <= 0 || nd.score_rem == INT_MAX || nd.sub == SUB_NONE || !rp.fits || !rp.tile_it || rp.grown || !packed) return false;
+  if (planned_meet_state(nd.meet).sf < 1) return false;
+  return s_keep <= 0 || planned_meet_block(nd.meet, T) >= s_keep + T;
 }
 
 struct P2PlanJob { int pl, tl, sub, sf, sr, packed; };
diff --git a/wfmash_amd/csrc/wfa_tile2.hip b/wfmash_amd/csrc/wfa_tile2.hip
--- a/wfmash_amd/csrc/wfa_tile2.hip
+++ b/wfmash_amd/csrc/wfa_tile2.hip
@@ -307,7 +307,7 @@
   int32_t* rout = ring_arena + J.ring_out + J.koff + (int64_t)dir * 5 * RING * width;
   const int kmax = tk.core_hi + halo;
   const int Tn = (!P2 && J.mode == 1) ? (dir == 0 ? J.tf : J.tr) : T;
-  const int t_stream = Tn - ((J.mode == 1 || J.mode == 6 || J.ring_prev < 0) ? H : E1);
+  const int t_stream = Tn - ((J.mode == 1 || J.mode == 6 || J.ring_prev < 0 || (!P2 && tile_plan_short_next(J, T))) ? H : E1);
   if (!P2 && FAST && !(coarse & 2)) {
     const bool fine = !(coarse & 1) || J.mode == 5 || (J.mode == 0 && sbase + T >= J.fine_s);
     if (fine != FINE) return;
diff --git a/wfmash_amd/host/capi_host.cpp b/wfmash_amd/host/capi_host.cpp
--- a/wfmash_amd/host/capi_host.cpp
+++ b/wfmash_amd/host/capi_host.cpp
@@ -269,6 +269,25 @@
   return -1;
 }
 
+int wfmh_test_planned_meet(const int64_t* in, int64_t n, int64_t* out) {
+  for (int64_t i = 0; i < n; ++i, in += 16, out += 8) {
+    wfm_penalties_t pen{};
+    pen.x = (int)in[0]; pen.o1 = (int)in[1]; pen.e1 = (int)in[2]; pen.o2 = (int)in[3]; pen.e2 = (int)in[4];
+    const int T = (int)in[15];
+    if (T < 1) return -1;
+    const int sum = wfm::planned_meet_sum((int)in[5], pen, (int)in[6], (int)in[7], in[8] != 0);
+    const wfm::PlannedMeet m = wfm::planned_meet((int)in[5], pen, (int)in[6], (int)in[7], in[8] != 0);
+    const int b0 = wfm::planned_meet_block(sum, T);
+    wfm::Node nd{};
+    nd.score_rem = (int32_t)in[5]; nd.cb = (int32_t)in[6]; nd.ce = (int32_t)in[7]; nd.sub = (int32_t)in[9]; nd.meet = sum;
+    wfm::RingPlan rp;
+    rp.fits = in[10] != 0; rp.tile_it = in[11] != 0; rp.grown = in[12] != 0;
+    out[0] = sum; out[1] = m.sf; out[2] = m.sr; out[3] = m.last_fwd; out[4] = b0; out[5] = m.sf - b0; out[6] = m.sr - b0;
+    out[7] = wfm::planned_meet_eligible(nd, rp, in[13] != 0, (int)in[14], T) ? 1 : 0;
+  }
+  return 0;
+}
+
 int wfmh_test_tile_plan_dirs(const int32_t* jobs, int64_t n, const int32_t* rules, const uint8_t* dirs, int32_t* per_block, int32_t* tasks, int64_t tasks_cap,
                              int64_t* scalars) {
   wfm::TilePlanRules r{rules[0], rules[1], rules[2], rules[3], rules[4], rules[5] != 0, rules[6] != 0, rules[7] != 0};
```

Result: faster. 60.19 million aligned bases/s, median of 6 (+7.4%).
